# carltonyfakhry/geneticsCRE

Hardware: AMD Instinct MI355X
Metric: path_x_permutation_scores_per_sec (higher is better)
Workload: dtype u32

## Files before the change

geneticscre_amd/csrc/gcre_ie.hip:

```cpp
#include "gcre_ie_common.h"

namespace gcre {

#ifdef GCRE_IE_TIMING
#define GCRE_TM_MARK(var) __builtin_amdgcn_s_waitcnt(0); const u64 var = __builtin_amdgcn_s_memtime()
#define GCRE_TM_ADD(i, t1, t0) tm[i] += (t1) - (t0)
#else
#define GCRE_TM_MARK(var)
#define GCRE_TM_ADD(i, t1, t0)
#endif

template <int M, int L>
__global__ __launch_bounds__(64 * kIeWaves) __attribute__((amdgpu_waves_per_eu(M == 1 ? 4 : 2))) void k_null_ie(const IeArgs a) {
  static_assert(L % 4 == 0 && L >= 8 && L <= 16, "planes come in groups of 4");
  const int lane = threadIdx.x & 63;
  const int wave = __builtin_amdgcn_readfirstlane(threadIdx.x >> 6);
  const int xcd = blockIdx.x & 7;
  const i64 bi = (i64)(blockIdx.x >> 3);
  const i64 bx = a.waves_per_xcd / kIeWaves;
  const i64 cpt = (a.seg_end - a.seg_begin + kIeWaves - 1) / kIeWaves;
  const i64 chunks = cpt * a.nkt;
  const u32 lane4 = (u32)lane * 4u;
  __shared__ u32 gmax_lds[kIeWaves][32 * 64];
  u32* scr = gmax_lds[wave] + lane;
#pragma unroll
  for (int q = 0; q < 32; q++) scr[q * 64] = 0u;

  const SparseSeg GCRE_CONSTANT* segs = (const SparseSeg GCRE_CONSTANT*)a.segs;
  const u64 GCRE_CONSTANT* loff0 = (const u64 GCRE_CONSTANT*)a.loff0;
  const u32 GCRE_CONSTANT* lidx0 = (const u32 GCRE_CONSTANT*)a.lidx0;

  int cur_kt = -1;
  __amdgpu_buffer_rsrc_t mt = __builtin_amdgcn_make_buffer_rsrc((void*)a.mt, 0, 0x7fffffff, 0x00020000);
#ifdef GCRE_IE_TIMING
  u64 tm[6] = {0, 0, 0, 0, 0, 0};
  const u64 tm_begin = __builtin_amdgcn_s_memtime();
#endif

  auto flush = [&]() {
    if (cur_kt < 0) return;
    GCRE_TM_MARK(tf0);
    __syncthreads();
    const u32 slot0 = (u32)wave * 512u + (u32)lane * 8u;
    __amdgpu_buffer_rsrc_t nb = __builtin_amdgcn_make_buffer_rsrc((void*)(a.null_bits + (size_t)cur_kt * 2048), 0, 8192, 0x00020000);
    const u32x4 g0 = __builtin_amdgcn_raw_buffer_load_b128(nb, slot0 * 4u, 0, 16 );
    const u32x4 g1 = __builtin_amdgcn_raw_buffer_load_b128(nb, slot0 * 4u + 16u, 0, 16 );
    u32* out = a.null_bits + (size_t)cur_kt * 2048 + slot0;
    u32* cell = &gmax_lds[0][0] + (slot0 & 31u) * 64u + (slot0 >> 5);
    u32 own[8];
#pragma unroll
    for (int j = 0; j < 8; j++) {
      u32 m = 0u;
#pragma unroll
      for (int w = 0; w < kIeWaves; w++) {
        const u32 v = cell[w * 32 * 64 + j * 64];
        m = v > m ? v : m;
        cell[w * 32 * 64 + j * 64] = 0u;
      }
      own[j] = m;
    }
#pragma unroll
    for (int j = 0; j < 8; j++) {
      const u32 g = j < 4 ? g0[j & 3] : g1[j & 3];
      if (own[j] > g) atomicMax(out + j, own[j]);
    }
    __syncthreads();
    GCRE_TM_MARK(tf1);
    GCRE_TM_ADD(3, tf1, tf0);
#ifdef GCRE_IE_TIMING
    tm[4] += 1;
#endif
  };

  auto to_counts = [&](const u32 (&C)[L], u32 (&R)[16]) {
#pragma unroll
    for (int l = 0; l < 16; l++) R[l] = (l < L) ? C[l] : 0u;
    transpose16(R);
  };
  auto finish_m1 = [&](const u32 (&C)[L], u32 total) {
    u32 R[16];
    to_counts(C, R);
    const u32* diag_g = (const u32*)a.t32 + sp_diag_offset(total);
    u32 v[32], o[32];
#pragma unroll
    for (int j = 0; j < 16; j++) {
      v[j] = diag_g[R[j] & 0xffffu];
      v[j + 16] = diag_g[R[j] >> 16];
    }
#pragma unroll
    for (int q = 0; q < 32; q++) o[q] = scr[q * 64];
#pragma unroll
    for (int q = 0; q < 32; q++)
      if (v[q] > o[q]) scr[q * 64] = v[q];
  };

  auto finish_m2 = [&](const u32 (&Cp)[L], const u32 (&Cn)[L], u32 tp, u32 tn) {
    u32 Rp[16], Rn[16];
    to_counts(Cp, Rp);
    to_counts(Cn, Rn);
    const double* dp = a.d64 + sp_diag_offset(tp);
    const double* dn = a.d64 + sp_diag_offset(tn);
#pragma unroll
    for (int g0 = 0; g0 < 16; g0 += 4) {
      double sp[8], sn[8];
      u32 o[8];
#pragma unroll
      for (int k = 0; k < 4; k++) {
        sp[k] = dp[Rp[g0 + k] & 0xffffu];
        sn[k] = dn[Rn[g0 + k] & 0xffffu];
        sp[k + 4] = dp[Rp[g0 + k] >> 16];
        sn[k + 4] = dn[Rn[g0 + k] >> 16];
        o[k] = scr[(g0 + k) * 64];
        o[k + 4] = scr[(g0 + k + 16) * 64];
      }
#pragma unroll
      for (int k = 0; k < 8; k++) {
        float f = (float)(sp[k] + sn[k]);
        f = (f > 0.0f) ? f : 0.0f;
        const u32 v = __float_as_uint(f);
        const int q = (k < 4) ? g0 + k : g0 + k - 4 + 16;
        if (v > o[k]) scr[q * 64] = v;
      }
    }
  };

  auto load_planes = [&](u32 (&P)[L], const u32* planes, u32 unit, int groups) {
    const u32x4* src = (const u32x4*)(planes + (u64)unit * 256u) + lane;
#pragma unroll
    for (int j = 0; j < L / 4; j++) {
      u32x4 v = {0u, 0u, 0u, 0u};
      if (j < groups) v = src[j * 64];
      P[4 * j + 0] = v.x;
      P[4 * j + 1] = v.y;
      P[4 * j + 2] = v.z;
      P[4 * j + 3] = v.w;
    }
  };

  const i64 c_end = (i64)(xcd + 1) * chunks / 8;
  for (i64 c = (i64)xcd * chunks / 8 + bi; c < c_end; c += bx) {
    const int kt = (int)(c / cpt);
    if (kt != cur_kt) {
      flush();
      cur_kt = kt;
      mt = __builtin_amdgcn_make_buffer_rsrc((void*)(a.mt + (size_t)kt * a.mt_rows * 64), 0, 0x7fffffff, 0x00020000);
    }
    const i64 sidx = a.seg_begin + (c - (i64)kt * cpt) * kIeWaves + wave;
    if (sidx < a.seg_end) {
      GCRE_TM_MARK(ts0);
      const u32 row0 = segs[sidx].row0;
      const u32 first = segs[sidx].first;
      const u32 npaths = segs[sidx].n;
      const u32 qv = first + (((u32)lane < npaths) ? (u32)lane : 0u);
      u32 infov[M], lovv[M];
#pragma unroll
      for (int h = 0; h < M; h++) {
        infov[h] = a.linfo[(u64)qv * M + h];
        lovv[h] = a.lover[(u64)qv * M + h];
      }
      const u32 rzv = a.rowz[qv];
      u32 zunit[M];
#pragma unroll
      for (int h = 0; h < M; h++) {
        const u32 hz = (M == 2 && (rzv >> 31)) ? (u32)(1 - h) : (u32)h;
        zunit[h] = ((u32)kt * (u32)a.rowsz + (rzv & 0x7fffffffu) * (u32)M + hz) * (u32)a.gz;
      }
      u32 ttv[M];
#pragma unroll
      for (int h = 0; h < M; h++) ttv[h] = a.tot[(u64)qv * M + h];
      u32 lv[M][8];
#pragma unroll
      for (int h = 0; h < M; h++) {
        const u32x4* lp = (const u32x4*)(a.dlist + ((u64)qv * M + h) * 8u);
        const u32x4 e0 = lp[0], e1 = lp[1];
        lv[h][0] = e0.x; lv[h][1] = e0.y; lv[h][2] = e0.z; lv[h][3] = e0.w;
        lv[h][4] = e1.x; lv[h][5] = e1.y; lv[h][6] = e1.z; lv[h][7] = e1.w;
      }

      auto stream = [&](u32 (&P)[L], const u32 GCRE_CONSTANT* list, u64 p, u64 e) {
        u32 x[16];
        for (; p + 16 <= e; p += 16) {
          load16(x, mt, lane4, *(const u32x16 GCRE_CONSTANT*)(list + p));
          add16<L>(P, x);
        }
        for (; p < e; p += 4) {
          const u32x4 offs = *(const u32x4 GCRE_CONSTANT*)(list + p);
          u32 y4[4];
#pragma unroll
          for (int j = 0; j < 4; j++) y4[j] = __builtin_amdgcn_raw_buffer_load_b32(mt, lane4, offs[j], 0);
          add4<L>(P, y4);
        }
      };

      u32 B[M][L];
#pragma unroll
      for (int h = 0; h < M; h++) {
        const u64 r = (u64)row0 * M + h;
        if (a.planes0) {
          load_planes(B[h], a.planes0, (u32)(((u64)kt * (u64)a.rows0 + r) * (u64)a.g0), a.g0);
        } else if (a.rec_slot) {
          const u32 ra = a.rec_row0[row0], rzr = a.rec_rowz[row0], rz = rzr & 0x7fffffffu, rinfo = a.rec_linfo[r];
          const u32 hz = (M == 2 && (rzr >> 31)) ? (u32)(1 - h) : (u32)h;
          u32 ZR[L], S[L];
          load_planes(B[h], a.rec_planes_a, (u32)(((u64)kt * (u64)a.rec_rows_a + (u64)ra * M + h) * (u64)a.rec_ga), a.rec_ga);
          load_planes(ZR, a.rec_planes_z, (u32)(((u64)kt * (u64)a.rec_rows_z + (u64)rz * M + hz) * (u64)a.rec_gz), a.rec_gz);
#pragma unroll
          for (int l = 0; l < L; l++) S[l] = 0u;
          const u32 rlen = linfo_len(rinfo);
          stream(S, (const u32 GCRE_CONSTANT*)(a.rec_slot + r * 8u), 0, 8);
          if (rlen > 8u) stream(S, (const u32 GCRE_CONSTANT*)(a.rec_over + a.rec_lover[r]), 0, (u64)(rlen - 8u));
          u32 cy = 0u, bw = 0u;
#pragma unroll
          for (int l = 0; l < L; l++) {
            const u32 zl = linfo_overlap(rinfo) ? ZR[l] : S[l];
            const u32 sl_ = linfo_overlap(rinfo) ? S[l] : 0u;
            const u32 s1_ = B[h][l] ^ zl ^ cy;
            cy = maj3(B[h][l], zl, cy);
            B[h][l] = s1_ ^ sl_ ^ bw;
            bw = maj3(~s1_, sl_, bw);
          }
        } else {
#pragma unroll
          for (int l = 0; l < L; l++) B[h][l] = 0u;
          stream(B[h], lidx0, loff0[r], loff0[r + 1]);
        }
      }

      GCRE_TM_MARK(ts1);
      GCRE_TM_ADD(0, ts1, ts0);
      for (u32 t = 0; t < npaths; t++) {
        GCRE_TM_MARK(tp0);
        const u32 q = first + t;
        u32 C[M][L];
#pragma unroll
        for (int h = 0; h < M; h++) {
          const u32 r0 = rdlane(infov[h], t);
          const u32 len = linfo_len(r0);
          const bool overlap = linfo_overlap(r0);
          u32 offs[8], y[8];
#pragma unroll
          for (int j = 0; j < 8; j++) offs[j] = rdlane(lv[h][j], t);
#pragma unroll
          for (int j = 0; j < 8; j++) y[j] = __builtin_amdgcn_raw_buffer_load_b32(mt, lane4, offs[j], 0);
          u32 Z[L];
          if (overlap) {
            load_planes(Z, a.planesz, rdlane(zunit[h], t), a.gz);
          } else {
#pragma unroll
            for (int l = 0; l < L; l++) Z[l] = 0u;
          }
          u32 c0, a0, c1, a1, c2, a2, d0, b0;
          csa(c0, a0, y[0], y[1], y[2]);
          csa(c1, a1, y[3], y[4], y[5]);
          csa(c2, a2, a0, a1, y[6]);
          const u32 s0 = a2 ^ y[7], c3 = a2 & y[7];
          csa(d0, b0, c0, c1, c2);
          const u32 s1 = b0 ^ c3, d1 = b0 & c3;
          u32 S[L];
          S[0] = s0; S[1] = s1; S[2] = d0 ^ d1; S[3] = d0 & d1;
#pragma unroll
          for (int l = 4; l < L; l++) S[l] = 0u;
          if (len > 8u) stream(S, (const u32 GCRE_CONSTANT*)(a.dover + rdlane(lovv[h], t)), 0, (u64)(len - 8u));
          if (overlap) {
            u32 cy = 0u, bw = 0u;
#pragma unroll
            for (int l = 0; l < L; l++) {
              const u32 s1_ = B[h][l] ^ Z[l] ^ cy;
              cy = maj3(B[h][l], Z[l], cy);
              C[h][l] = s1_ ^ S[l] ^ bw;
              bw = maj3(~s1_, S[l], bw);
            }
          } else {
            u32 cy = 0u;
#pragma unroll
            for (int l = 0; l < L; l++) {
              C[h][l] = B[h][l] ^ S[l] ^ cy;
              cy = maj3(B[h][l], S[l], cy);
            }
          }
        }
        if (a.planes_out) {
#pragma unroll
          for (int h = 0; h < M; h++) {
            const u64 rh = ((u64)a.out_first + q) * M + h;
            u32x4* dst = (u32x4*)(a.planes_out + (((u64)cur_kt * (u64)a.rows_out + rh) * (u64)a.go) * 256u) + lane;
#pragma unroll
            for (int j = 0; j < 4; j++) {
              if (j < a.go) {
                u32x4 v = {0u, 0u, 0u, 0u};
                if (4 * j < L) v = u32x4{C[h][(4 * j) % L], C[h][(4 * j + 1) % L], C[h][(4 * j + 2) % L], C[h][(4 * j + 3) % L]};
                dst[j * 64] = v;
              }
            }
          }
        }
        GCRE_TM_MARK(tp1);
        GCRE_TM_ADD(1, tp1, tp0);
        if (q < a.score_begin || q >= a.score_end) continue;
        if constexpr (M == 1) {
          finish_m1(C[0], rdlane(ttv[0], t));
        } else {
          finish_m2(C[0], C[M - 1], rdlane(ttv[0], t), rdlane(ttv[M - 1], t));
        }
        GCRE_TM_MARK(tp2);
        GCRE_TM_ADD(2, tp2, tp1);
      }
    }
  }
  flush();
#ifdef GCRE_IE_TIMING
  tm[5] = __builtin_amdgcn_s_memtime() - tm_begin;
  if (a.timing && lane == 0)
    for (int i = 0; i < 6; i++) atomicAdd((unsigned long long*)a.timing + i, (unsigned long long)tm[i]);
  if (a.timing && lane == 0) atomicMax((unsigned long long*)a.timing + 6, (unsigned long long)tm[5]);
#endif
}


template <int L, int GZ, bool OUT, bool REC>
__global__ __launch_bounds__(64 * kIeWaves) __attribute__((amdgpu_waves_per_eu(L <= 12 ? 4 : 3))) void k_null_ie_m1(const IeArgs a) {
  constexpr int LP = (L + 3) / 4 * 4;
  static_assert(L >= 8 && L <= 16 && GZ >= 2 && 4 * GZ <= LP, "planes come in groups of 4");
  __shared__ u32 nmax_lds[kIeWaves][32 * 64];
  const int lane = threadIdx.x & 63;
  const int wave = __builtin_amdgcn_readfirstlane(threadIdx.x >> 6);
  const u32 lane4 = (u32)lane * 4u;
  u32* nm = nmax_lds[wave] + lane;
#pragma unroll
  for (int q = 0; q < 32; q++) nm[q * 64] = 0u;
  const SparseSeg GCRE_CONSTANT* segs = (const SparseSeg GCRE_CONSTANT*)a.segs;
  const char* k_planesz = (const char*)(((u64)(u32)__builtin_amdgcn_readfirstlane((int)(u32)((u64)a.planesz >> 32)) << 32) |
                                        (u64)(u32)__builtin_amdgcn_readfirstlane((int)(u32)(u64)a.planesz));

  int cur_kt = -1;
  u32 valid = 0u;
  u32 lad_base = (a.lad_mode == 0) ? 0u : (u32)(kLadderLevels - 1 + a.lad_mode) * (u32)a.ladder_stride;
  const u32 lad_keep = (u32)kLadderLevels * (u32)a.ladder_stride;
  bool dirty = false;
  u32 n_slow = 0u;
#ifdef GCRE_IE_TIMING
  u64 tm[6] = {0, 0, 0, 0, 0, 0};
  const u64 tm_begin = __builtin_amdgcn_s_memtime();
#endif
  __amdgpu_buffer_rsrc_t mt = __builtin_amdgcn_make_buffer_rsrc((void*)a.mt, 0, 0x7fffffff, 0x00020000);

  auto exchange = [&]() {
    u32* out = a.null_bits + (size_t)cur_kt * 2048 + lane * 32;
    __amdgpu_buffer_rsrc_t nb = __builtin_amdgcn_make_buffer_rsrc((void*)(a.null_bits + (size_t)cur_kt * 2048), 0, 8192, 0x00020000);
    u32x4 g4[8];
#pragma unroll
    for (int j = 0; j < 8; j++) g4[j] = __builtin_amdgcn_raw_buffer_load_b128(nb, (u32)lane * 128u + (u32)j * 16u, 0, 16 );
    u32 lo = 0xffffffffu;
#pragma unroll
    for (int q = 0; q < 32; q++) {
      const u32 g = g4[q >> 2][q & 3];
      const u32 own = nm[q * 64];
      if (dirty && own > g) atomicMax(out + q, own);
      const u32 v = own > g ? own : g;
      if ((valid >> q) & 1u) lo = v < lo ? v : lo;
    }
    dirty = false;
    u32 theta = __builtin_amdgcn_readfirstlane(wave_min_u32(lo));
    if (theta == 0xffffffffu) theta = 0u;
    int j = (int)(__uint_as_float(theta) * (float)kLadderPerUnit);
    j = j < 0 ? 0 : (j > kLadderLevels - 1 ? kLadderLevels - 1 : j);
    lad_base = (u32)j * (u32)a.ladder_stride;
  };
  auto flush_tile = [&]() {
    if (cur_kt >= 0) {
      u32* out = a.null_bits + (size_t)cur_kt * 2048 + lane * 32;
#pragma unroll 8
      for (int q = 0; q < 32; q++) {
        const u32 own = nm[q * 64];
        if (own != 0u) {
          atomicMax(out + q, own);
          nm[q * 64] = 0u;
        }
      }
    }
    dirty = false;
  };

  __shared__ u32 wq_state[kIeWaves][8];
  WorkQueue wq;
  wq.st = wq_state[wave];
  wq.init(a.queue, (u32)((a.seg_end - a.seg_begin + a.batch - 1) / a.batch), (u32)a.nkt);
  {
    wq.select(blockIdx.x & 7u);
  }
  u32 ticket = wq.take(lane);
  int since = 0, period = 1;
  for (;;) {
    const u32 work = __builtin_amdgcn_readfirstlane(ticket);
    const u32 q_n = wq.get(2);
    if (work >= q_n) {
      if (!wq.steal(lane)) break;
      ticket = wq.take(lane);
      continue;
    }
    ticket = wq.take(lane);
    const u32 item = wq.get(1) + work, nb = wq.get(3);
    const int kt = (int)(item / nb);
    const i64 s_lo = a.seg_begin + (i64)(item - (u32)kt * nb) * a.batch;
    const i64 s_hi = s_lo + a.batch < a.seg_end ? s_lo + a.batch : a.seg_end;
    if (kt != cur_kt) {
      flush_tile();
      cur_kt = kt;
      mt = __builtin_amdgcn_make_buffer_rsrc((void*)(a.mt + (size_t)kt * a.mt_rows * 64), 0, 0x7fffffff, 0x00020000);
      const int live = a.K - kt * 2048 - lane * 32;
      valid = live >= 32 ? 0xffffffffu : (live <= 0 ? 0u : ((1u << live) - 1u));
      if (a.lad_mode == 0) lad_base = 0u;
      since = 0;
      period = 1;
    }
    u32 nextv = 0u;
    bool have_next = false;
    for (i64 sidx = s_lo; sidx < s_hi; sidx++) {
      u32 row0, first, npaths;
      u32 rc_a = 0u, rc_z = 0u, rc_info = 0u, rc_lov = 0u;
      typedef u32 __attribute__((ext_vector_type(8))) u32x8;
      u32x8 rc_o = {0u, 0u, 0u, 0u, 0u, 0u, 0u, 0u};
      if (have_next) {
        row0 = rdlane(nextv, 0);
        first = rdlane(nextv, 1);
        npaths = rdlane(nextv, 2);
        if constexpr (REC) {
          rc_a = rdlane(nextv, 4);
          rc_z = rdlane(nextv, 5);
          rc_info = rdlane(nextv, 6);
          rc_lov = rdlane(nextv, 7);
#pragma unroll
          for (int j = 0; j < 8; j++) rc_o[j] = rdlane(nextv, 8 + j);
        }
      } else {
        row0 = segs[sidx].row0;
        first = segs[sidx].first;
        npaths = segs[sidx].n;
        if constexpr (REC) {
          const u32 GCRE_CONSTANT* rs = (const u32 GCRE_CONSTANT*)a.rec_segs + (u64)sidx * kRecSegWords;
          rc_a = rs[0];
          rc_z = rs[1];
          rc_info = rs[2];
          rc_lov = rs[3];
          rc_o = *(const u32x8 GCRE_CONSTANT*)(rs + 4);
        }
      }
      have_next = sidx + 1 < s_hi;
      if (have_next) {
        const u32* src = (const u32*)a.segs + (u64)(sidx + 1) * 3u + (u32)(lane < 3 ? lane : 0);
        if constexpr (REC) {
          if (lane >= 4 && lane < 16) src = a.rec_segs + (u64)(sidx + 1) * kRecSegWords + (u32)(lane - 4);
        }
        nextv = *src;
      }
      GCRE_TM_MARK(ts0);
      if (a.lad_mode == 0 && ++since >= period) {
        exchange();
        since = 0;
        period = period < kIeRefresh ? period * 2 : kIeRefresh;
      }
      GCRE_TM_MARK(ts1);
      GCRE_TM_ADD(4, ts1, ts0);

      const u32 qv = first + (((u32)lane < npaths) ? (u32)lane : 0u);
      const u32 infov = a.linfo[qv];
      const u32 lovv = a.lover[qv];
      const u32 zunit = ((u32)kt * (u32)a.rowsz + (a.rowz[qv] & 0x7fffffffu)) * (u32)a.gz;
      const u32 totv = a.tot[qv];
      const u32 lhv = a.ladder[((u64)sidx < (u64)a.score_segs ? lad_base : lad_keep) + totv];
      const u32x8 GCRE_CONSTANT* slots = (const u32x8 GCRE_CONSTANT*)(a.dlist + (u64)first * 8u);
      auto issue = [&](u32 t2, const u32x8 offs, u32 (&yy)[8], u32 (&ZZ)[4 * GZ]) {
        if constexpr (OUT) {
#pragma unroll
          for (int j = 0; j < 8; j++) yy[j] = __builtin_amdgcn_raw_buffer_load_b32(mt, lane4, offs[j], 0);
        }
        __amdgpu_buffer_rsrc_t rz = __builtin_amdgcn_make_buffer_rsrc((void*)(k_planesz + (u64)rdlane(zunit, t2) * 1024u), 0, 0x7fffffff, 0x00020000);
#pragma unroll
        for (int j = 0; j < GZ; j++) {
          const u32x4 v = __builtin_amdgcn_raw_buffer_load_b128(rz, lane4 * 4u + (u32)j * 1024u, 0, 0);
          ZZ[4 * j + 0] = v.x; ZZ[4 * j + 1] = v.y; ZZ[4 * j + 2] = v.z; ZZ[4 * j + 3] = v.w;
        }
      };
      u32 yA[8], yB[8], ZA[4 * GZ], ZB[4 * GZ];
      const u32 last = npaths - 1u;
      auto at = [&](u32 t2) -> u32 { return t2 < last ? t2 : last; };
      u32x8 oA = slots[0], oB = slots[at(1u)];
      issue(0u, oA, yA, ZA);
      u32 B[LP];
      auto load_groups = [&](u32 (&P)[LP], const u32* planes, u64 unit, int groups) {
        const u32x4* src = (const u32x4*)(planes + unit * 256u) + lane;
#pragma unroll
        for (int j = 0; j < LP / 4; j++) {
          u32x4 v = {0u, 0u, 0u, 0u};
          if (j < groups) v = src[j * 64];
          P[4 * j + 0] = v.x; P[4 * j + 1] = v.y; P[4 * j + 2] = v.z; P[4 * j + 3] = v.w;
        }
      };
      if constexpr (!REC) {
        load_groups(B, a.planes0, ((u64)kt * (u64)a.rows0 + (u64)row0) * (u64)a.g0, a.g0);
      } else {
        const u32 ra = rc_a, rz = rc_z & 0x7fffffffu, rinfo = rc_info;
        const u32x8 ro = rc_o;
        u32 yr[8];
#pragma unroll
        for (int j = 0; j < 8; j++) yr[j] = __builtin_amdgcn_raw_buffer_load_b32(mt, lane4, ro[j], 0);
        u32 ZR[LP];
        load_groups(B, a.rec_planes_a, ((u64)kt * (u64)a.rec_rows_a + (u64)ra) * (u64)a.rec_ga, a.rec_ga);
        load_groups(ZR, a.rec_planes_z, ((u64)kt * (u64)a.rec_rows_z + (u64)rz) * (u64)a.rec_gz, a.rec_gz);
        u32 S[L];
        {
          u32 S4[4];
          sum8(yr, S4);
#pragma unroll
          for (int l = 0; l < L; l++) S[l] = (l < 4) ? S4[l < 4 ? l : 0] : 0u;
        }
        const u32 rlen = linfo_len(rinfo);
        if (rlen > 8u) {
          const u32 GCRE_CONSTANT* more = (const u32 GCRE_CONSTANT*)(a.rec_over + rc_lov);
          for (u32 p = 0u; p + 8u < rlen; p += 8u) {
            const u32x8 o8 = *(const u32x8 GCRE_CONSTANT*)(more + p);
            u32 yy[8], s4[4];
#pragma unroll
            for (int j = 0; j < 8; j++) yy[j] = __builtin_amdgcn_raw_buffer_load_b32(mt, lane4, o8[j], 0);
            sum8(yy, s4);
            u32 cy = 0u;
#pragma unroll
            for (int l = 0; l < L; l++) {
              const u32 sv = S[l];
              const u32 add = (l < 4) ? s4[l < 4 ? l : 0] : 0u;
              S[l] = xor3(sv, add, cy);
              cy = majority(sv, add, cy);
            }
          }
        }
        if (linfo_overlap(rinfo)) {
          u32 cy = 0u, bw = 0u;
#pragma unroll
          for (int l = 0; l < L; l++) {
            const u32 s1_ = xor3(B[l], ZR[l], cy);
            cy = majority(B[l], ZR[l], cy);
            B[l] = xor3(s1_, S[l], bw);
            bw = borrow3(s1_, S[l], bw);
          }
        } else {
          u32 cy = 0u;
#pragma unroll
          for (int l = 0; l < L; l++) {
            const u32 bl = B[l];
            B[l] = xor3(bl, S[l], cy);
            cy = majority(bl, S[l], cy);
          }
        }
      }

      GCRE_TM_MARK(ts2);
      GCRE_TM_ADD(0, ts2, ts1);
      auto compute = [&](u32 t, const u32 (&y)[8], const u32 (&Z)[4 * GZ]) {
        GCRE_TM_MARK(tp0);
        const u32 r0 = rdlane(infov, t);
        const u32 len = linfo_len(r0);
        const bool overlap = linfo_overlap(r0);
        u32 C[L];
        u32 S4[4];
        sum8(y, S4);
        if (len <= 8u && overlap) {
          u32 T[4 * GZ];
          u32 bw = 0u;
#pragma unroll
          for (int l = 0; l < 4 * GZ; l++) {
            if (l < 4) {
              T[l] = xor3(Z[l], S4[l < 4 ? l : 0], bw);
              bw = borrow3(Z[l], S4[l < 4 ? l : 0], bw);
            } else {
              T[l] = Z[l] ^ bw;
              bw = bw & ~Z[l];
            }
          }
          u32 cy = 0u;
#pragma unroll
          for (int l = 0; l < L; l++) {
            if (l < 4 * GZ) {
              C[l] = xor3(B[l], T[l < 4 * GZ ? l : 0], cy);
              cy = majority(B[l], T[l < 4 * GZ ? l : 0], cy);
            } else {
              C[l] = B[l] ^ cy;
              cy = B[l] & cy;
            }
          }
        } else if (len <= 8u) {
          u32 cy = 0u;
#pragma unroll
          for (int l = 0; l < L; l++) {
            if (l < 4) {
              C[l] = xor3(B[l], S4[l < 4 ? l : 0], cy);
              cy = majority(B[l], S4[l < 4 ? l : 0], cy);
            } else {
              C[l] = B[l] ^ cy;
              cy = B[l] & cy;
            }
          }
        } else {
          u32 S[L];
#pragma unroll
          for (int l = 0; l < L; l++) S[l] = (l < 4) ? S4[l < 4 ? l : 0] : 0u;
          const u32 GCRE_CONSTANT* more = (const u32 GCRE_CONSTANT*)(a.dover + rdlane(lovv, t));
          for (u32 p = 0u; p + 8u < len; p += 8u) {
            const u32x8 o8 = *(const u32x8 GCRE_CONSTANT*)(more + p);
            u32 yy[8], s4[4];
#pragma unroll
            for (int j = 0; j < 8; j++) yy[j] = __builtin_amdgcn_raw_buffer_load_b32(mt, lane4, o8[j], 0);
            sum8(yy, s4);
            u32 cy = 0u;
#pragma unroll
            for (int l = 0; l < L; l++) {
              const u32 sv = S[l];
              if (l < 4) {
                S[l] = xor3(sv, s4[l < 4 ? l : 0], cy);
                cy = majority(sv, s4[l < 4 ? l : 0], cy);
              } else {
                S[l] = sv ^ cy;
                cy = sv & cy;
              }
            }
          }
          if (overlap) {
            u32 cy = 0u, bw = 0u;
#pragma unroll
            for (int l = 0; l < L; l++) {
              const u32 zl = (l < 4 * GZ) ? Z[l < 4 * GZ ? l : 0] : 0u;
              const u32 s1_ = xor3(B[l], zl, cy);
              cy = majority(B[l], zl, cy);
              C[l] = xor3(s1_, S[l], bw);
              bw = borrow3(s1_, S[l], bw);
            }
          } else {
            u32 cy = 0u;
#pragma unroll
            for (int l = 0; l < L; l++) {
              C[l] = xor3(B[l], S[l], cy);
              cy = majority(B[l], S[l], cy);
            }
          }
        }
        if constexpr (OUT) {
          const u64 rh = (u64)a.out_first + first + t;
          u32x4* dst = (u32x4*)(a.planes_out + (((u64)kt * (u64)a.rows_out + rh) * (u64)a.go) * 256u) + lane;
#pragma unroll
          for (int j = 0; j < 4; j++) {
            if (j < a.go) {
              u32x4 v = {0u, 0u, 0u, 0u};
              if (4 * j < L) v = u32x4{C[(4 * j) % L], (4 * j + 1 < L) ? C[(4 * j + 1) % L] : 0u, (4 * j + 2 < L) ? C[(4 * j + 2) % L] : 0u,
                                       (4 * j + 3 < L) ? C[(4 * j + 3) % L] : 0u};
              dst[j * 64] = v;
            }
          }
        }
        const u32 lh = rdlane(lhv, t);
        const u32 lo = lh & 0xffffu, hi = lh >> 16;
        u32 blo = 0u, bhi = 0u;
#pragma unroll
        for (int l = 0; l < L; l++) {
          const u32 kl = (u32)__builtin_amdgcn_sbfe((int)lo, l, 1);
          const u32 kh = (u32)__builtin_amdgcn_sbfe((int)hi, l, 1);
          blo = borrow3(C[l], kl, blo);
          bhi = borrow3(kh, C[l], bhi);
        }
        u32 m = (blo | bhi) & valid;
        GCRE_TM_MARK(tp2);
        GCRE_TM_ADD(2, tp2, tp0);
        if (__builtin_amdgcn_ballot_w64(m != 0u) == 0ull) return;
        n_slow++;
        const u32* diag_g = (const u32*)a.t32 + sp_diag_offset(rdlane(totv, t));
        while (m != 0u) {
          u32 bb[4], vv[4];
#pragma unroll
          for (int k = 0; k < 4; k++) {
            bb[k] = m ? (u32)__builtin_ctz(m) : bb[k ? k - 1 : 0];
            m &= m - 1u;
            u32 cnt = 0u;
#pragma unroll
            for (int l = 0; l < L; l++) cnt |= ((C[l] >> bb[k]) & 1u) << l;
            vv[k] = diag_g[cnt];
          }
#pragma unroll
          for (int k = 0; k < 4; k++)
            __hip_atomic_fetch_max(nm + bb[k] * 64, vv[k], __ATOMIC_RELAXED, __HIP_MEMORY_SCOPE_WAVEFRONT);
        }
        dirty = true;
        GCRE_TM_MARK(tp3);
        GCRE_TM_ADD(3, tp3, tp2);
      };

      auto compute_f = [&](u32 t, const u32 (&Z)[4 * GZ]) {
        const u32 r0 = rdlane(infov, t);
        const u32 len = linfo_len(r0);
        const bool overlap = linfo_overlap(r0);
        const u32 ov = len - linfo_pad(r0);
        const u32 lh = rdlane(lhv, t);
        const u32 lo = lh & 0xffffu, hi = lh >> 16;
        u32 W[L];
        u32 mu = valid;
        if (overlap) {
          u32 cy = 0u;
#pragma unroll
          for (int l = 0; l < L; l++) {
            if (l < 4 * GZ) {
              W[l] = xor3(B[l], Z[l < 4 * GZ ? l : 0], cy);
              cy = majority(B[l], Z[l < 4 * GZ ? l : 0], cy);
            } else {
              W[l] = B[l] ^ cy;
              cy = B[l] & cy;
            }
          }
          u32 lo2 = lo ? lo + ov : 0u;
          lo2 = lo2 > 0xffffu ? 0xffffu : lo2;
          u32 blo = 0u, bhi = 0u;
#pragma unroll
          for (int l = 0; l < L; l++) {
            const u32 kl = (u32)__builtin_amdgcn_sbfe((int)lo2, l, 1);
            const u32 kh = (u32)__builtin_amdgcn_sbfe((int)hi, l, 1);
            blo = borrow3(W[l], kl, blo);
            bhi = borrow3(kh, W[l], bhi);
          }
          if ((lo2 >> L) != 0u) blo = 0xffffffffu;
          mu = (blo | bhi | cy) & valid;
        } else {
#pragma unroll
          for (int l = 0; l < L; l++) W[l] = B[l];
        }
        if (__builtin_amdgcn_ballot_w64(mu != 0u) == 0ull) return;
#ifdef GCRE_IE_TIMING
        tm[1] += 1;
        tm[3] += (u64)__popcll(__builtin_amdgcn_ballot_w64(mu != 0u));
#endif
        u32 slow = 0u;
        const u32x8 o = slots[t];
        if (mu != 0u) {
          u32 y[8], S4[4];
#pragma unroll
          for (int j = 0; j < 8; j++) y[j] = __builtin_amdgcn_raw_buffer_load_b32(mt, lane4, o[j], 0);
          sum8(y, S4);
          u32 S[L];
#pragma unroll
          for (int l = 0; l < L; l++) S[l] = (l < 4) ? S4[l < 4 ? l : 0] : 0u;
          if (len > 8u) {
            const u32 GCRE_CONSTANT* more = (const u32 GCRE_CONSTANT*)(a.dover + rdlane(lovv, t));
            for (u32 p = 0u; p + 8u < len; p += 8u) {
              const u32x8 o8 = *(const u32x8 GCRE_CONSTANT*)(more + p);
              u32 yy[8], s4[4];
#pragma unroll
              for (int j = 0; j < 8; j++) yy[j] = __builtin_amdgcn_raw_buffer_load_b32(mt, lane4, o8[j], 0);
              sum8(yy, s4);
              u32 cy = 0u;
#pragma unroll
              for (int l = 0; l < L; l++) {
                const u32 sv = S[l];
                if (l < 4) {
                  S[l] = xor3(sv, s4[l < 4 ? l : 0], cy);
                  cy = majority(sv, s4[l < 4 ? l : 0], cy);
                } else {
                  S[l] = sv ^ cy;
                  cy = sv & cy;
                }
              }
            }
          }
          u32 C[L];
          if (overlap) {
            u32 bw = 0u;
#pragma unroll
            for (int l = 0; l < L; l++) {
              C[l] = xor3(W[l], S[l], bw);
              bw = borrow3(W[l], S[l], bw);
            }
          } else {
            u32 cy = 0u;
#pragma unroll
            for (int l = 0; l < L; l++) {
              C[l] = xor3(W[l], S[l], cy);
              cy = majority(W[l], S[l], cy);
            }
          }
          u32 blo = 0u, bhi = 0u;
#pragma unroll
          for (int l = 0; l < L; l++) {
            const u32 kl = (u32)__builtin_amdgcn_sbfe((int)lo, l, 1);
            const u32 kh = (u32)__builtin_amdgcn_sbfe((int)hi, l, 1);
            blo = borrow3(C[l], kl, blo);
            bhi = borrow3(kh, C[l], bhi);
          }
          u32 m = (blo | bhi) & mu;
          if (m != 0u) {
            slow = 1u;
            const u32* diag_g = (const u32*)a.t32 + sp_diag_offset(rdlane(totv, t));
            while (m != 0u) {
              u32 bb[4], vv[4];
#pragma unroll
              for (int k = 0; k < 4; k++) {
                bb[k] = m ? (u32)__builtin_ctz(m) : bb[k ? k - 1 : 0];
                m &= m - 1u;
                u32 cnt = 0u;
#pragma unroll
                for (int l = 0; l < L; l++) cnt |= ((C[l] >> bb[k]) & 1u) << l;
                vv[k] = diag_g[cnt];
              }
#pragma unroll
              for (int k = 0; k < 4; k++)
                __hip_atomic_fetch_max(nm + bb[k] * 64, vv[k], __ATOMIC_RELAXED, __HIP_MEMORY_SCOPE_WAVEFRONT);
            }
          }
        }
        if (__builtin_amdgcn_ballot_w64(slow != 0u) != 0ull) {
          n_slow++;
          dirty = true;
        }
      };

      if constexpr (OUT) {
        for (u32 t = 0; t < npaths; t += 2) {
          issue(at(t + 1), oB, yB, ZB);
          oA = slots[at(t + 2)];
          compute(t, yA, ZA);
          if (t + 1 < npaths) {
            issue(at(t + 2), oA, yA, ZA);
            oB = slots[at(t + 3)];
            compute(t + 1, yB, ZB);
          }
        }
      } else {
        u32 ZC[4 * GZ];
        issue(at(1u), oB, yB, ZB);
        for (u32 t = 0; t < npaths; t += 3) {
          issue(at(t + 2), oA, yA, ZC);
          compute_f(t, ZA);
          if (t + 1 < npaths) {
            issue(at(t + 3), oA, yA, ZA);
            compute_f(t + 1, ZB);
          }
          if (t + 2 < npaths) {
            issue(at(t + 4), oA, yA, ZB);
            compute_f(t + 2, ZC);
          }
        }
      }
    }
  }
  flush_tile();
#ifdef GCRE_IE_TIMING
  tm[5] = __builtin_amdgcn_s_memtime() - tm_begin;
  if (a.timing && lane == 0)
    for (int i = 0; i < 6; i++) atomicAdd((unsigned long long*)a.timing + i, (unsigned long long)tm[i]);
  if (a.timing && lane == 0) atomicMax((unsigned long long*)a.timing + 6, (unsigned long long)tm[5]);
#endif
  if (a.stats && lane == 0 && n_slow) atomicAdd(a.stats, n_slow);
}

#define GCRE_IE_M2(EXPR)                    \
  if (planes <= 8) { EXPR(2, 8); }          \
  else if (planes <= 12) { EXPR(2, 12); }   \
  else { EXPR(2, 16); }

#define GCRE_IE_M1_OR(EXPR, LL, GG)                                                  \
  if (out) { if (rec) { EXPR(LL, GG, true, true); } else { EXPR(LL, GG, true, false); } }   \
  else { if (rec) { EXPR(LL, GG, false, true); } else { EXPR(LL, GG, false, false); } }

#define GCRE_IE_M1(EXPR)                                                     \
  if (planes <= 8) { GCRE_IE_M1_OR(EXPR, 8, 2) }                             \
  else if (planes <= 10) {                                                   \
    if (gz <= 2) { GCRE_IE_M1_OR(EXPR, 10, 2) } else { GCRE_IE_M1_OR(EXPR, 10, 3) }        \
  } else if (planes <= 12) {                                                 \
    if (gz <= 2) { GCRE_IE_M1_OR(EXPR, 12, 2) } else { GCRE_IE_M1_OR(EXPR, 12, 3) }        \
  } else {                                                                   \
    if (gz <= 2) { GCRE_IE_M1_OR(EXPR, 16, 2) }                              \
    else if (gz == 3) { GCRE_IE_M1_OR(EXPR, 16, 3) }                         \
    else { GCRE_IE_M1_OR(EXPR, 16, 4) }                                      \
  }

#define GCRE_IE_GEN(EXPR)                                          \
  if (method == 1) {                                               \
    if (planes <= 8) { EXPR(1, 8); }                               \
    else if (planes <= 12) { EXPR(1, 12); }                        \
    else { EXPR(1, 16); }                                          \
  } else {                                                         \
    GCRE_IE_M2(EXPR)                                               \
  }

__global__ __launch_bounds__(256) void k_fill_rec_segs(const SparseSeg* segs, i64 nsegs, const u32* r_row0, const u32* r_rowz,
                                                       const u32* r_linfo, const u32* r_lover, const u32* r_slot, const u32* r_tot,
                                                       u32* out) {
  const i64 t = (i64)blockIdx.x * blockDim.x + threadIdx.x;
  const i64 sidx = t >> 2;
  const int part = (int)(t & 3);
  if (sidx >= nsegs) return;
  const u32 row0 = segs[sidx].row0;
  u32* o = out + sidx * kRecSegWords;
  if (part == 0) {
    o[0] = r_row0[row0];
    o[1] = r_rowz[row0];
  } else if (part == 1) {
    u32 info = r_linfo[row0];
    u32 need = 3u;
    if (r_tot) {
      const u32 t = r_tot[row0];
      need = t < 16u ? 0u : (t < 256u ? 1u : (t < 4096u ? 2u : 3u));
    }
    o[2] = linfo_with_groups(info, need);
    o[3] = r_lover[row0];
  } else {
    const u32x4 v = *(const u32x4*)(r_slot + (u64)row0 * 8u + (part - 2) * 4);
    *(u32x4*)(o + 4 + (part - 2) * 4) = v;
  }
}

hipError_t launch_fill_rec_segs(const SparseSeg* segs, int64_t nsegs, const uint32_t* r_row0, const uint32_t* r_rowz,
                                const uint32_t* r_linfo, const uint32_t* r_lover, const uint32_t* r_slot, const uint32_t* r_tot,
                                uint32_t* out, hipStream_t stream) {
  if (nsegs == 0) return hipSuccess;
  const i64 blocks = (nsegs * 4 + 255) / 256;
  hipLaunchKernelGGL(k_fill_rec_segs, dim3((unsigned)blocks), dim3(256), 0, stream, segs, nsegs, r_row0, r_rowz, r_linfo, r_lover,
                     r_slot, r_tot, out);
  return hipGetLastError();
}

hipError_t launch_null_ie(const IeArgs& a, int method, int planes, bool general, hipStream_t stream) {
  const dim3 grid((unsigned)(8 * a.waves_per_xcd / kIeWaves));
  const dim3 block(64 * kIeWaves);
  if (method == 1 && !general) {
    const int gz = a.gz;
    const bool out = a.planes_out != nullptr;
    const bool rec = a.rec_slot != nullptr;
#define GCRE_LAUNCH(LL, GG, OO, RR) hipLaunchKernelGGL((k_null_ie_m1<LL, GG, OO, RR>), grid, block, 0, stream, a)
    GCRE_IE_M1(GCRE_LAUNCH)
#undef GCRE_LAUNCH
  } else if (method == 2 && !general) {
    return launch_null_ie_m2(a, planes, stream);
  } else {
    if (a.waves_per_xcd < kIeWaves || a.waves_per_xcd % kIeWaves != 0) return hipErrorInvalidValue;
#define GCRE_LAUNCH(MM, LL) hipLaunchKernelGGL((k_null_ie<MM, LL>), grid, block, 0, stream, a)
    GCRE_IE_GEN(GCRE_LAUNCH)
#undef GCRE_LAUNCH
  }
  return hipGetLastError();
}

int ie_max_waves_per_cu(int method, int planes, int gz, bool out, bool rec) {
  int blocks = 0;
  hipError_t e = hipSuccess;
  if (method == 1) {
#define GCRE_OCC(LL, GG, OO, RR) e = hipOccupancyMaxActiveBlocksPerMultiprocessor(&blocks, k_null_ie_m1<LL, GG, OO, RR>, 64 * kIeWaves, 0)
    GCRE_IE_M1(GCRE_OCC)
#undef GCRE_OCC
  } else {
    return ie2_max_waves_per_cu(planes, gz, out, rec);
  }
  if (e != hipSuccess || blocks < 1) blocks = 1;
  return blocks * kIeWaves;
}

template <int L>
__global__ __launch_bounds__(256) void k_build_planes(const u32* mt_all, u32 mt_rows, int nkt, const u64* loff,
                                                      const u32* lidx, i64 nrowhalves, int groups, u32* planes) {
  const int lane = threadIdx.x & 63;
  const i64 wave = (i64)blockIdx.x * 4 + __builtin_amdgcn_readfirstlane(threadIdx.x >> 6);
  const i64 nwaves = (i64)gridDim.x * 4;
  const u32 lane4 = (u32)lane * 4u;
  const u64 GCRE_CONSTANT* off = (const u64 GCRE_CONSTANT*)loff;
  const u32 GCRE_CONSTANT* list = (const u32 GCRE_CONSTANT*)lidx;
  const i64 items = nrowhalves * nkt;
  for (i64 it = wave; it < items; it += nwaves) {
    const i64 w = it / nrowhalves;
    const i64 rr = it - w * nrowhalves;
    __amdgpu_buffer_rsrc_t mt = __builtin_amdgcn_make_buffer_rsrc((void*)(mt_all + (size_t)w * mt_rows * 64), 0, 0x7fffffff, 0x00020000);
    u32 P[L];
#pragma unroll
    for (int l = 0; l < L; l++) P[l] = 0u;
    u64 p = off[rr];
    const u64 e = off[rr + 1];
    u32 x[16];
    for (; p + 16 <= e; p += 16) {
      load16(x, mt, lane4, *(const u32x16 GCRE_CONSTANT*)(list + p));
      add16<L>(P, x);
    }
    for (; p < e; p += 4) {
      const u32x4 offs = *(const u32x4 GCRE_CONSTANT*)(list + p);
      u32 y[4];
#pragma unroll
      for (int j = 0; j < 4; j++) y[j] = __builtin_amdgcn_raw_buffer_load_b32(mt, lane4, offs[j], 0);
      add4<L>(P, y);
    }
    u32x4* dst = (u32x4*)(planes + (((u64)w * (u64)nrowhalves + (u64)rr) * (u64)groups) * 256u) + lane;
#pragma unroll
    for (int j = 0; j < L / 4; j++)
      if (j < groups) dst[j * 64] = u32x4{P[4 * j], P[4 * j + 1], P[4 * j + 2], P[4 * j + 3]};
  }
}

hipError_t launch_build_planes(const uint32_t* mt, uint32_t mt_rows, int nkt, const uint64_t* loff, const uint32_t* lidx,
                               int64_t nrowhalves, int groups, uint32_t* planes, hipStream_t stream) {
  const i64 items = nrowhalves * nkt;
  if (items == 0) return hipSuccess;
  const i64 blocks = (items + 3) / 4;
  const dim3 grid((unsigned)(blocks < 256 * 8 ? blocks : 256 * 8)), block(256);
  if (groups <= 2) hipLaunchKernelGGL(k_build_planes<8>, grid, block, 0, stream, mt, mt_rows, nkt, loff, lidx, nrowhalves, groups, planes);
  else if (groups == 3) hipLaunchKernelGGL(k_build_planes<12>, grid, block, 0, stream, mt, mt_rows, nkt, loff, lidx, nrowhalves, groups, planes);
  else hipLaunchKernelGGL(k_build_planes<16>, grid, block, 0, stream, mt, mt_rows, nkt, loff, lidx, nrowhalves, groups, planes);
  return hipGetLastError();
}

__global__ __launch_bounds__(64) void k_build_ladder(const u32* t32, int TD, u32* ladder) {
  __shared__ int left[kLadderLevels + 2], right[kLadderLevels + 2];
  const int t = blockIdx.x;
  const int lane = threadIdx.x;
  if (t >= TD) return;
  const u32* d = t32 + sp_diag_offset((u32)t);
  for (int k = lane; k < kLadderLevels + 2; k += 64) {
    left[k] = -1;
    right[k] = t + 1;
  }
  u64 mine = ~(u64)0;
  for (int c = lane; c <= t; c += 64) {
    const u64 key = ((u64)d[c] << 32) | (u32)c;
    mine = key < mine ? key : mine;
  }
#pragma unroll
  for (int o = 32; o > 0; o >>= 1) {
    const u64 other = ((u64)(u32)__shfl_xor((int)(mine >> 32), o, 64) << 32) | (u32)__shfl_xor((int)(u32)mine, o, 64);
    mine = other < mine ? other : mine;
  }
  const u32 best = (u32)(mine >> 32);
  const int c0 = (int)(u32)mine;
  __syncthreads();
  auto blocked_below = [](u32 bits) -> int {
    const float v = __uint_as_float(bits);
    if (!(v > 0.0f)) return 0;
    const float x = v * (float)kLadderPerUnit;
    if (x >= (float)kLadderLevels) return kLadderLevels;
    const int j = (int)x;
    return ((float)j < x) ? j + 1 : j;
  };
  for (int c = lane; c <= t; c += 64) {
    if (c == c0) continue;
    const int J = blocked_below(d[c]);
    if (J == 0) continue;
    if (c < c0) atomicMax(&left[J], c);
    else atomicMin(&right[J], c);
  }
  __syncthreads();
  if (lane == 0) {
    int l = -1, r = t + 1;
    for (int k = kLadderLevels; k >= 0; k--) {
      l = left[k] > l ? left[k] : l;
      r = right[k] < r ? right[k] : r;
      left[k] = l;
      right[k] = r;
    }
  }
  __syncthreads();
  const int Jbest = blocked_below(best);
  for (int j = lane; j < kLadderLevels; j += 64) {
    u32 e = 1u;
    if (Jbest <= j) e = ((u32)(right[j + 1] - 1) << 16) | (u32)(left[j + 1] + 1);
    ladder[(size_t)j * TD + t] = e;
  }
  if (lane == 0) {
    ladder[(size_t)kLadderLevels * TD + t] = 0xffff0000u;
    ladder[(size_t)(kLadderLevels + 1) * TD + t] = 1u;
  }
}

hipError_t launch_build_ladder(const float* t32, int TD, uint32_t* ladder, hipStream_t stream) {
  hipLaunchKernelGGL(k_build_ladder, dim3((unsigned)TD), dim3(64), 0, stream, (const u32*)t32, TD, ladder);
  return hipGetLastError();
}

__global__ __launch_bounds__(64) void k_build_ladder2(const double* dmax, int TD, u32* ladder) {
  __shared__ int left[kLadder2Levels + 2], right[kLadder2Levels + 2];
  const int t = blockIdx.x;
  const int lane = threadIdx.x;
  if (t >= TD) return;
  const double* d = dmax + sp_diag_offset((u32)t);
  for (int k = lane; k < kLadder2Levels + 2; k += 64) {
    left[k] = -1;
    right[k] = t + 1;
  }
  double bestv = __builtin_inf();
  int bestc = 0x7fffffff;
  for (int c = lane; c <= t; c += 64) {
    const double v = d[c];
    if (v < bestv || (v == bestv && c < bestc) || (bestc == 0x7fffffff)) {
      if (!(v != v)) { bestv = v; bestc = c; }
      else if (bestc == 0x7fffffff) { bestv = __builtin_inf(); bestc = c; }
    }
  }
#pragma unroll
  for (int o = 32; o > 0; o >>= 1) {
    const double ov = __shfl_xor(bestv, o, 64);
    const int oc = __shfl_xor(bestc, o, 64);
    if (ov < bestv || (ov == bestv && oc < bestc)) { bestv = ov; bestc = oc; }
  }
  const int c0 = bestc;
  __syncthreads();
  auto blocked_below = [](double v) -> int {
    if (v != v) return kLadder2Levels;
    if (!(v > 0.0)) return 0;
    const double x = v * (double)(2 * kLadderPerUnit);
    if (x >= (double)kLadder2Levels) return kLadder2Levels;
    const int j = (int)x;
    return ((double)j < x) ? j + 1 : j;
  };
  for (int c = lane; c <= t; c += 64) {
    if (c == c0) continue;
    const int J = blocked_below(d[c]);
    if (J == 0) continue;
    if (c < c0) atomicMax(&left[J], c);
    else atomicMin(&right[J], c);
  }
  __syncthreads();
  if (lane == 0) {
    int l = -1, r = t + 1;
    for (int k = kLadder2Levels; k >= 0; k--) {
      l = left[k] > l ? left[k] : l;
      r = right[k] < r ? right[k] : r;
      left[k] = l;
      right[k] = r;
    }
  }
  __syncthreads();
  const int Jbest = blocked_below(d[c0]);
  for (int j = lane; j < kLadder2Levels; j += 64) {
    u32 e = 1u;
    if (Jbest <= j) e = ((u32)(right[j + 1] - 1) << 16) | (u32)(left[j + 1] + 1);
    ladder[(size_t)j * TD + t] = e;
  }
  if (lane == 0) {
    ladder[(size_t)kLadder2Levels * TD + t] = 0xffff0000u;
    ladder[(size_t)(kLadder2Levels + 1) * TD + t] = 1u;
  }
}

hipError_t launch_build_ladder2(const double* dmax, int TD, uint32_t* ladder, hipStream_t stream) {
  hipLaunchKernelGGL(k_build_ladder2, dim3((unsigned)TD), dim3(64), 0, stream, dmax, TD, ladder);
  return hipGetLastError();
}

}
```

geneticscre_amd/csrc/gcre_ie2.hip:

```cpp
#include "gcre_ie_common.h"

#ifndef GCRE_M2_STEPS
#define GCRE_M2_STEPS 2
#endif
#ifndef GCRE_M2_YW_WIDE
#define GCRE_M2_YW_WIDE 4
#endif
#ifndef GCRE_M2_WAVES16
#define GCRE_M2_WAVES16 3
#endif
#ifndef GCRE_M2_MODES
#define GCRE_M2_MODES 3
#endif

namespace gcre {

template <int L, int GZ, bool OUT, bool REC>
__global__ __launch_bounds__(64 * kIeWaves) __attribute__((amdgpu_waves_per_eu(L <= 10 ? 4 : (L <= 12 ? 3 : GCRE_M2_WAVES16)))) void k_null_ie_m2(const IeArgs a) {
  constexpr int NS = GCRE_M2_STEPS;
  static_assert(NS == 2 || NS == 3, "two or three steps");
  constexpr int LP = (L + 3) / 4 * 4;
  constexpr int YW = L <= 10 ? 4 : GCRE_M2_YW_WIDE;
  constexpr int LZ = 4 * GZ;
  static_assert(LZ <= LP, "added rows have no more planes than joined paths");
  static_assert(L >= 8 && L <= 16, "8 to 16 counter planes");
  typedef u32 __attribute__((ext_vector_type(8))) u32x8;
  typedef u32 __attribute__((ext_vector_type(YW))) SlotV;
  __shared__ u32 nmax_lds[kIeWaves][32 * 64];
  constexpr u32 kLqCap = 128u;
  __shared__ u32 lq_lds[kIeWaves][3][kLqCap];
  const int lane = threadIdx.x & 63;
  const int wave = __builtin_amdgcn_readfirstlane(threadIdx.x >> 6);
  const u32 lane4 = (u32)lane * 4u;
  u32* nm = nmax_lds[wave] + lane;
#pragma unroll
  for (int q = 0; q < 32; q++) nm[q * 64] = 0u;
  const SparseSeg GCRE_CONSTANT* segs = (const SparseSeg GCRE_CONSTANT*)a.segs;
  u32 (*lq)[kLqCap] = lq_lds[wave];
  u32 lq_n = 0u;
  bool dirty = false;
  auto lq_drain = [&]() {
    for (u32 base = 0u; base < lq_n; base += 64u) {
      const u32 i = base + (u32)lane;
      if (i < lq_n) {
        const double f64 = a.d64[lq[0][i]] + a.d64[lq[1][i]];
        float f = (float)f64;
        f = (f > 0.0f) ? f : 0.0f;
        __hip_atomic_fetch_max(nmax_lds[wave] + lq[2][i], __float_as_uint(f), __ATOMIC_RELAXED, __HIP_MEMORY_SCOPE_WAVEFRONT);
      }
    }
    if (lq_n != 0u) dirty = true;
    lq_n = 0u;
  };
  const char* k_planesz = (const char*)(((u64)(u32)__builtin_amdgcn_readfirstlane((int)(u32)((u64)a.planesz >> 32)) << 32) |
                                        (u64)(u32)__builtin_amdgcn_readfirstlane((int)(u32)(u64)a.planesz));

  int cur_kt = -1;
  u32 valid = 0u;
  u32 lad[NS];
#pragma unroll
  for (int s = 0; s < NS; s++) lad[s] = (a.lad_mode == 0) ? 0u : (u32)(kLadder2Levels - 1 + a.lad_mode) * (u32)a.ladder_stride;
  const u32 lad_keep = (u32)kLadder2Levels * (u32)a.ladder_stride;
  u32 lad_top = lad[0];
  bool top_ok = a.lad_mode != 0 || a.g00_rows == 0u;
  u32 n_slow = 0u;
#ifdef GCRE_IE_TIMING
  u64 tm[8] = {0, 0, 0, 0, 0, 0, 0, 0};
#define GCRE_TM_COUNT(i, n) tm[i] += (u64)(n)
#else
#define GCRE_TM_COUNT(i, n)
#endif
  __amdgpu_buffer_rsrc_t mt = __builtin_amdgcn_make_buffer_rsrc((void*)a.mt, 0, 0x7fffffff, 0x00020000);

  auto exchange = [&]() {
    lq_drain();
    u32* out = a.null_bits + (size_t)cur_kt * 2048 + lane * 32;
    __amdgpu_buffer_rsrc_t nb = __builtin_amdgcn_make_buffer_rsrc((void*)(a.null_bits + (size_t)cur_kt * 2048), 0, 8192, 0x00020000);
    u32x4 g4[8];
#pragma unroll
    for (int j = 0; j < 8; j++) g4[j] = __builtin_amdgcn_raw_buffer_load_b128(nb, (u32)lane * 128u + (u32)j * 16u, 0, 16 );
    u32 lo = 0xffffffffu;
#pragma unroll
    for (int q = 0; q < 32; q++) {
      const u32 g = g4[q >> 2][q & 3];
      const u32 own = nm[q * 64];
      if (dirty && own > g) atomicMax(out + q, own);
      const u32 v = own > g ? own : g;
      if ((valid >> q) & 1u) lo = v < lo ? v : lo;
    }
    dirty = false;
    u32 theta = __builtin_amdgcn_readfirstlane(wave_min_u32(lo));
    if (theta == 0xffffffffu) theta = 0u;
    int j = (int)(__uint_as_float(theta) * (float)kLadderPerUnit);
    j = j < 0 ? 0 : (j > kLadderLevels - 1 ? kLadderLevels - 1 : j);
    int r[NS];
    if constexpr (NS == 2) {
      r[0] = (2 * j) / 3;
      r[1] = 2 * j - r[0];
    } else {
      r[0] = j / 2;
      r[1] = j;
      r[2] = 2 * j - r[0];
    }
#pragma unroll
    for (int s = 0; s < NS; s++) {
      const int rs = r[s] > kLadder2Levels - 1 ? kLadder2Levels - 1 : r[s];
      lad[s] = (u32)rs * (u32)a.ladder_stride;
    }
    const int rt = 2 * j - (int)a.g00_rows;
    top_ok = a.g00_rows != 0xffffffffu && rt >= 0;
    lad_top = (u32)(rt < 0 ? 0 : (rt > kLadder2Levels - 1 ? kLadder2Levels - 1 : rt)) * (u32)a.ladder_stride;
  };
  auto flush_tile = [&]() {
    lq_drain();
    if (cur_kt >= 0) {
      u32* out = a.null_bits + (size_t)cur_kt * 2048 + lane * 32;
#pragma unroll 8
      for (int q = 0; q < 32; q++) {
        const u32 own = nm[q * 64];
        if (own != 0u) {
          atomicMax(out + q, own);
          nm[q * 64] = 0u;
        }
      }
    }
    dirty = false;
  };
  auto load_groups = [&](u32 (&P)[LP], const u32* planes, u64 unit, int groups) {
    const u32x4* src = (const u32x4*)(planes + unit * 256u) + lane;
#pragma unroll
    for (int j = 0; j < LP / 4; j++) {
      u32x4 v = {0u, 0u, 0u, 0u};
      if (j < groups) v = src[j * 64];
      P[4 * j + 0] = v.x; P[4 * j + 1] = v.y; P[4 * j + 2] = v.z; P[4 * j + 3] = v.w;
    }
  };
  auto outside = [&](const auto& C, u32 lh) -> u32 {
    const u32 lo = lh & 0xffffu, hi = lh >> 16;
    u32 blo = 0u, bhi = 0u;
#pragma unroll
    for (int l = 0; l < L; l++) {
      const u32 kl = (u32)__builtin_amdgcn_sbfe((int)lo, l, 1);
      const u32 kh = (u32)__builtin_amdgcn_sbfe((int)hi, l, 1);
      blo = borrow3(C[l], kl, blo);
      bhi = borrow3(kh, C[l], bhi);
    }
    return blo | bhi;
  };
  auto sum4 = [&](const u32 (&y)[4], u32 (&S)[4]) {
    const u32 a0 = xor3(y[0], y[1], y[2]), c0 = majority(y[0], y[1], y[2]);
    S[0] = a0 ^ y[3];
    const u32 c1 = a0 & y[3];
    S[1] = c0 ^ c1;
    S[2] = c0 & c1;
    S[3] = 0u;
  };
  auto sum_more = [&](u32 (&S)[L], u32 len, const u32 GCRE_CONSTANT* over, const u32 GCRE_CONSTANT* lover_at) {
    const u32 GCRE_CONSTANT* more = over + *lover_at;
    for (u32 p = 0u; p + 8u < len; p += 8u) {
      const u32x8 o8 = *(const u32x8 GCRE_CONSTANT*)(more + p);
      u32 yy[8], s4[4];
#pragma unroll
      for (int j = 0; j < 8; j++) yy[j] = __builtin_amdgcn_raw_buffer_load_b32(mt, lane4, o8[j], 0);
      sum8(yy, s4);
      u32 cy = 0u;
#pragma unroll
      for (int l = 0; l < L; l++) {
        const u32 sv = S[l];
        if (l < 4) {
          S[l] = xor3(sv, s4[l < 4 ? l : 0], cy);
          cy = majority(sv, s4[l < 4 ? l : 0], cy);
        } else {
          S[l] = sv ^ cy;
          cy = sv & cy;
        }
      }
    }
  };
  auto add_half = [&](u32 (&C)[L], const auto& Bx, const u32 (&y)[YW], const u32 (&Z)[LZ], u32 info, const u32 GCRE_CONSTANT* slot_at,
                      const u32 GCRE_CONSTANT* lover_at) {
    const u32 len = linfo_len(info);
    const bool overlap = linfo_overlap(info);
    const u32 real = len - linfo_pad(info);
    u32 S4[4];
    {
      const u32 y03[4] = {y[0], y[1], y[2], y[3]};
      sum4(y03, S4);
    }
    if (real > 4u) {
      GCRE_TM_COUNT(4, 1);
      u32 y2[4], s2[4];
      if constexpr (YW == 8) {
#pragma unroll
        for (int j = 0; j < 4; j++) y2[j] = y[(4 + j) % YW];
      } else {
        const u32x4 o = *(const u32x4 GCRE_CONSTANT*)(slot_at + 4);
#pragma unroll
        for (int j = 0; j < 4; j++) y2[j] = __builtin_amdgcn_raw_buffer_load_b32(mt, lane4, o[j], 0);
      }
      sum4(y2, s2);
      const u32 t0 = S4[0] ^ s2[0], c0 = S4[0] & s2[0];
      const u32 t1 = xor3(S4[1], s2[1], c0), c1 = majority(S4[1], s2[1], c0);
      const u32 t2 = xor3(S4[2], s2[2], c1), c2 = majority(S4[2], s2[2], c1);
      S4[0] = t0; S4[1] = t1; S4[2] = t2; S4[3] = c2;
    }
    if (len <= 8u) {
      if (overlap) {
        u32 T[LZ];
        u32 bw = 0u;
#pragma unroll
        for (int l = 0; l < LZ; l++) {
          if (l < 4) {
            T[l] = xor3(Z[l], S4[l < 4 ? l : 0], bw);
            bw = borrow3(Z[l], S4[l < 4 ? l : 0], bw);
          } else {
            T[l] = Z[l] ^ bw;
            bw = bw & ~Z[l];
          }
        }
        u32 cy = 0u;
#pragma unroll
        for (int l = 0; l < L; l++) {
          if (l < LZ) {
            C[l] = xor3(Bx[l], T[l < LZ ? l : 0], cy);
            cy = majority(Bx[l], T[l < LZ ? l : 0], cy);
          } else {
            C[l] = Bx[l] ^ cy;
            cy = Bx[l] & cy;
          }
        }
      } else {
        u32 cy = 0u;
#pragma unroll
        for (int l = 0; l < L; l++) {
          if (l < 4) {
            C[l] = xor3(Bx[l], S4[l < 4 ? l : 0], cy);
            cy = majority(Bx[l], S4[l < 4 ? l : 0], cy);
          } else {
            C[l] = Bx[l] ^ cy;
            cy = Bx[l] & cy;
          }
        }
      }
      return;
    }
    GCRE_TM_COUNT(6, 1);
    u32 S[L];
#pragma unroll
    for (int l = 0; l < L; l++) S[l] = (l < 4) ? S4[l < 4 ? l : 0] : 0u;
    sum_more(S, len, (const u32 GCRE_CONSTANT*)a.dover, lover_at);
    if (overlap) {
      u32 cy = 0u, bw = 0u;
#pragma unroll
      for (int l = 0; l < L; l++) {
        const u32 zl = (l < LZ) ? Z[l < LZ ? l : 0] : 0u;
        const u32 s1_ = xor3(Bx[l], zl, cy);
        cy = majority(Bx[l], zl, cy);
        C[l] = xor3(s1_, S[l], bw);
        bw = borrow3(s1_, S[l], bw);
      }
    } else {
      u32 cy = 0u;
#pragma unroll
      for (int l = 0; l < L; l++) {
        C[l] = xor3(Bx[l], S[l], cy);
        cy = majority(Bx[l], S[l], cy);
      }
    }
  };
  auto issue = [&](u32 info, u32 zu, const SlotV offs, u32 (&yy)[YW], u32 (&ZZ)[LZ]) {
    const u32 real = linfo_true_len(info);
    if (YW == 8 && real > 4u) {
#pragma unroll
      for (int j = 0; j < 8; j++) yy[j % YW] = __builtin_amdgcn_raw_buffer_load_b32(mt, lane4, offs[j % YW], 0);
    } else if (real > 0u) {
#ifdef GCRE_M2_NOROWS
#pragma unroll
      for (int j = 0; j < 4; j++) yy[j] = offs[j];
#else
#pragma unroll
      for (int j = 0; j < 4; j++) yy[j] = __builtin_amdgcn_raw_buffer_load_b32(mt, lane4, offs[j], 0);
#endif
    } else {
#pragma unroll
      for (int j = 0; j < 4; j++) yy[j] = 0u;
    }
    if (linfo_overlap(info)) {
      __amdgpu_buffer_rsrc_t rz = __builtin_amdgcn_make_buffer_rsrc((void*)(k_planesz + (u64)zu * 1024u), 0, 0x7fffffff, 0x00020000);
#pragma unroll
      for (int j = 0; j < GZ; j++) {
        u32x4 v = {0u, 0u, 0u, 0u};
#ifdef GCRE_M2_NOZLOAD
        v = u32x4{zu, zu + (u32)j, lane4, 0u};
#else
        if (j < 2 || j < a.gz) v = __builtin_amdgcn_raw_buffer_load_b128(rz, lane4 * 4u + (u32)j * 1024u, 0, 0);
#endif
        ZZ[4 * j + 0] = v.x; ZZ[4 * j + 1] = v.y; ZZ[4 * j + 2] = v.z; ZZ[4 * j + 3] = v.w;
      }
    }
  };
  auto enqueue = [&](u32 m, const auto& Ca, const auto& Cb, u32 da, u32 db, bool b_zero) {
    while (__builtin_amdgcn_ballot_w64(m != 0u) != 0ull) {
      if (lq_n + 64u > kLqCap) lq_drain();
      const bool has = m != 0u;
      const u32 bb = has ? (u32)__builtin_ctz(m) : 0u;
      m &= m - 1u;
      u32 ca = 0u, cb = 0u;
#pragma unroll
      for (int l = L - 1; l >= 0; l--) ca = (ca << 1) | __builtin_amdgcn_ubfe(Ca[l], bb, 1u);
      if (!b_zero) {
#pragma unroll
        for (int l = L - 1; l >= 0; l--) cb = (cb << 1) | __builtin_amdgcn_ubfe(Cb[l], bb, 1u);
      }
      const u64 hm = __builtin_amdgcn_ballot_w64(has);
      GCRE_TM_COUNT(5, __builtin_popcountll(hm));
      const u32 pos = lq_n + __builtin_amdgcn_mbcnt_hi((u32)(hm >> 32), __builtin_amdgcn_mbcnt_lo((u32)hm, 0u));
      if (has) {
        lq[0][pos] = da + ca;
        lq[1][pos] = db + cb;
        lq[2][pos] = bb * 64u + (u32)lane;
      }
      lq_n += (u32)__builtin_popcountll(hm);
    }
  };

  __shared__ u32 wq_state[kIeWaves][8];
  WorkQueue wq;
  wq.st = wq_state[wave];
  wq.init(a.queue, (u32)((a.seg_end - a.seg_begin + a.batch - 1) / a.batch), (u32)a.nkt);
  wq.select(blockIdx.x & 7u);
  u32 ticket = wq.take(lane);
  int since = 0, period = 1;
  for (;;) {
    const u32 work = __builtin_amdgcn_readfirstlane(ticket);
    const u32 q_n = wq.get(2);
    if (work >= q_n) {
      if (!wq.steal(lane)) break;
      ticket = wq.take(lane);
      continue;
    }
    ticket = wq.take(lane);
    const u32 item = wq.get(1) + work, nb = wq.get(3);
    const int kt = (int)(item / nb);
    const i64 s_lo = a.seg_begin + (i64)(item - (u32)kt * nb) * a.batch;
    const i64 s_hi = s_lo + a.batch < a.seg_end ? s_lo + a.batch : a.seg_end;
    if (kt != cur_kt) {
      flush_tile();
      cur_kt = kt;
      mt = __builtin_amdgcn_make_buffer_rsrc((void*)(a.mt + (size_t)kt * a.mt_rows * 64), 0, 0x7fffffff, 0x00020000);
      const int live = a.K - kt * 2048 - lane * 32;
      valid = live >= 32 ? 0xffffffffu : (live <= 0 ? 0u : ((1u << live) - 1u));
      if (a.lad_mode == 0) {
#pragma unroll
        for (int s = 0; s < NS; s++) lad[s] = 0u;
        lad_top = 0u;
        top_ok = a.g00_rows == 0u;
      }
      since = 0;
      period = 1;
    }
    for (i64 sidx = s_lo; sidx < s_hi; sidx++) {
      const u32 row0 = segs[sidx].row0;
      const u32 first = segs[sidx].first;
      const u32 npaths = segs[sidx].n;
      if (a.lad_mode == 0 && ++since >= period) {
        exchange();
        since = 0;
        period = period < kIeRefresh ? period * 2 : kIeRefresh;
      }
      const bool inl = (u32)lane < npaths;
      const u32 qv = first + (inl ? (u32)lane : 0u);
      const u32 rzv = a.rowz[qv];
      const bool mine = (u64)sidx < (u64)a.score_segs;
      const bool seg_top_ok = top_ok;
      const u32 GCRE_CONSTANT* k_lover = (const u32 GCRE_CONSTANT*)a.lover + (u64)first * 2u;
      const u32 GCRE_CONSTANT* k_tot = (const u32 GCRE_CONSTANT*)a.tot + (u64)first * 2u;
      const u32 GCRE_CONSTANT* k_slot = (const u32 GCRE_CONSTANT*)a.dlist + (u64)first * 16u;
      u32 infoc, zunitc, ladc[NS], ladt, ladu[NS], totu;
      u64 pm0, pm1, pm2;
      {
        const u32 i0 = a.linfo[(u64)qv * 2], i1 = a.linfo[(u64)qv * 2 + 1];
        const u32 t0_ = a.tot[(u64)qv * 2], t1_ = a.tot[(u64)qv * 2 + 1];
        const bool e0 = !linfo_overlap(i0) && (i0 & kLinfoLenMask) == linfo_pad(i0);
        const bool e1 = !linfo_overlap(i1) && (i1 & kLinfoLenMask) == linfo_pad(i1);
        pm0 = __builtin_amdgcn_ballot_w64(inl && e1);
        pm1 = __builtin_amdgcn_ballot_w64(inl && e0 && !e1);
        pm2 = __builtin_amdgcn_ballot_w64(inl && !e0 && !e1);
        const bool c1 = e0 && !e1;
        infoc = c1 ? i1 : i0;
        const u32 hz = ((rzv >> 31) != 0u) != c1 ? 1u : 0u;
        zunitc = ((u32)kt * (u32)a.rowsz + (rzv & 0x7fffffffu) * 2u + hz) * (u32)a.gz;
        const u32 tc = c1 ? t1_ : t0_;
        totu = c1 ? t0_ : t1_;
#pragma unroll
        for (int s = 0; s < NS; s++) {
          ladc[s] = a.ladder[(mine ? lad[s] : lad_keep) + tc];
          ladu[s] = a.ladder[(mine ? lad[NS - 1 - s] : lad_keep) + totu];
        }
        ladt = a.ladder[(mine ? lad_top : lad_keep) + tc];
      }

      u32 B[2][LP];
      if constexpr (!REC) {
#pragma unroll
        for (int h = 0; h < 2; h++)
          load_groups(B[h], a.planes0, ((u64)kt * (u64)a.rows0 + (u64)row0 * 2 + h) * (u64)a.g0, a.g0);
      } else {
        const u32 GCRE_CONSTANT* r_row0 = (const u32 GCRE_CONSTANT*)a.rec_row0;
        const u32 GCRE_CONSTANT* r_rowz = (const u32 GCRE_CONSTANT*)a.rec_rowz;
        const u32 GCRE_CONSTANT* r_linfo = (const u32 GCRE_CONSTANT*)a.rec_linfo;
        const u32 GCRE_CONSTANT* r_lover = (const u32 GCRE_CONSTANT*)a.rec_lover;
        const u32 ra = r_row0[row0], rzr = r_rowz[row0];
        const u32 ri0 = r_linfo[(u64)row0 * 2], ri1 = r_linfo[(u64)row0 * 2 + 1];
#pragma unroll
        for (int h = 0; h < 2; h++)
          load_groups(B[h], a.rec_planes_a, ((u64)kt * (u64)a.rec_rows_a + (u64)ra * 2 + h) * (u64)a.rec_ga, a.rec_ga);
#pragma unroll
        for (int h = 0; h < 2; h++) {
          const u32 rinfo = h ? ri1 : ri0;
          const u32 rlen = linfo_len(rinfo);
          if (!linfo_overlap(rinfo) && rlen == linfo_pad(rinfo)) continue;
          const u32x8 ro = *(const u32x8 GCRE_CONSTANT*)(a.rec_slot + ((u64)row0 * 2 + h) * 8u);
          u32 yr[8];
#pragma unroll
          for (int j = 0; j < 8; j++) yr[j] = __builtin_amdgcn_raw_buffer_load_b32(mt, lane4, ro[j], 0);
          u32 ZR[LP];
          if (linfo_overlap(rinfo)) {
            const u32 hz = (rzr >> 31) ? (u32)(1 - h) : (u32)h;
            load_groups(ZR, a.rec_planes_z, ((u64)kt * (u64)a.rec_rows_z + (u64)(rzr & 0x7fffffffu) * 2 + hz) * (u64)a.rec_gz, a.rec_gz);
          }
          u32 S[L];
          {
            u32 S4[4];
            sum8(yr, S4);
#pragma unroll
            for (int l = 0; l < L; l++) S[l] = (l < 4) ? S4[l < 4 ? l : 0] : 0u;
          }
          if (rlen > 8u) sum_more(S, rlen, (const u32 GCRE_CONSTANT*)a.rec_over, r_lover + (u64)row0 * 2 + h);
          if (linfo_overlap(rinfo)) {
            u32 cy = 0u, bw = 0u;
#pragma unroll
            for (int l = 0; l < L; l++) {
              const u32 s1_ = xor3(B[h][l], ZR[l], cy);
              cy = majority(B[h][l], ZR[l], cy);
              B[h][l] = xor3(s1_, S[l], bw);
              bw = borrow3(s1_, S[l], bw);
            }
          } else {
            u32 cy = 0u;
#pragma unroll
            for (int l = 0; l < L; l++) {
              const u32 bl = B[h][l];
              B[h][l] = xor3(bl, S[l], cy);
              cy = majority(bl, S[l], cy);
            }
          }
        }
      }
      auto write_out = [&](u32 h, u32 t, const auto& C) {
        if constexpr (OUT) {
          const u64 rh = ((u64)a.out_first + first + t) * 2 + h;
          u32x4* dst = (u32x4*)(a.planes_out + (((u64)kt * (u64)a.rows_out + rh) * (u64)a.go) * 256u) + lane;
#pragma unroll
          for (int j = 0; j < 4; j++) {
            if (j < a.go) {
              u32x4 v = {0u, 0u, 0u, 0u};
              if (4 * j < L) v = u32x4{C[(4 * j) % L], (4 * j + 1 < L) ? C[(4 * j + 1) % L] : 0u,
                                       (4 * j + 2 < L) ? C[(4 * j + 2) % L] : 0u, (4 * j + 3 < L) ? C[(4 * j + 3) % L] : 0u};
              dst[j * 64] = v;
            }
          }
        }
      };
      u32 yA[YW], yB[YW], ZA[LZ], ZB[LZ];
#pragma unroll
      for (int l = 0; l < LZ; l++) ZA[l] = ZB[l] = 0u;

      if (pm2 != 0ull) {
        u32 info2[2], zunit2[2], lad2[NS][2];
#pragma unroll
        for (int h = 0; h < 2; h++) {
          info2[h] = a.linfo[(u64)qv * 2 + h];
          const u32 hz = (rzv >> 31) ? (u32)(1 - h) : (u32)h;
          zunit2[h] = ((u32)kt * (u32)a.rowsz + (rzv & 0x7fffffffu) * 2u + hz) * (u32)a.gz;
          const u32 th = a.tot[(u64)qv * 2 + h];
#pragma unroll
          for (int s = 0; s < NS; s++) lad2[s][h] = a.ladder[(mine ? lad[s] : lad_keep) + th];
        }
        u64 rem = pm2;
        u32 t = (u32)__builtin_ctzll(rem);
        rem &= rem - 1ull;
        SlotV oA = *(const SlotV GCRE_CONSTANT*)(k_slot + t * 16u), oB = *(const SlotV GCRE_CONSTANT*)(k_slot + t * 16u + 8u);
        issue(rdlane(info2[0], t), rdlane(zunit2[0], t), oA, yA, ZA);
        for (;;) {
          issue(rdlane(info2[1], t), rdlane(zunit2[1], t), oB, yB, ZB);
          const bool more = rem != 0ull;
          const u32 tn = more ? (u32)__builtin_ctzll(rem) : t;
          rem &= rem - 1ull;
          oA = *(const SlotV GCRE_CONSTANT*)(k_slot + tn * 16u);
          u32 C0[L], C1[L];
          add_half(C0, B[0], yA, ZA, rdlane(info2[0], t), k_slot + t * 16u, k_lover + t * 2u);
          write_out(0u, t, C0);
          issue(rdlane(info2[0], tn), rdlane(zunit2[0], tn), oA, yA, ZA);
          oB = *(const SlotV GCRE_CONSTANT*)(k_slot + tn * 16u + 8u);
          add_half(C1, B[1], yB, ZB, rdlane(info2[1], t), k_slot + t * 16u + 8u, k_lover + t * 2u + 1u);
          write_out(1u, t, C1);
          u32 m = valid;
#pragma unroll
          for (int s = 0; s < NS; s++) m &= outside(C0, rdlane(lad2[s][0], t)) | outside(C1, rdlane(lad2[NS - 1 - s][1], t));
          GCRE_TM_COUNT(3, 1);
          if (__builtin_amdgcn_ballot_w64(m != 0u) != 0ull) {
            n_slow++;
            enqueue(m, C0, C1, sp_diag_offset(k_tot[t * 2u]), sp_diag_offset(k_tot[t * 2u + 1u]), false);
          }
          if (!more) break;
          t = tn;
        }
      }

      const u32 t00 = pm0 ? (u32)__builtin_ctzll(pm0) : 0u, t01 = pm1 ? (u32)__builtin_ctzll(pm1) : 0u;
      const u32 totU0 = rdlane(totu, t00), totU1 = rdlane(totu, t01);
      const bool empty0 = (GCRE_M2_MODES & 1) && pm0 != 0ull && totU0 == 0u && seg_top_ok;
      const bool empty1 = (GCRE_M2_MODES & 1) && pm1 != 0ull && totU1 == 0u && seg_top_ok;
      u32 U[NS], U1[NS];
#pragma unroll
      for (int s = 0; s < NS; s++) U[s] = U1[s] = 0u;
      bool single0 = true, single1 = true;
      if (pm0 != 0ull && !empty0) {
#pragma unroll
        for (int s = 0; s < NS; s++) U[s] = outside(B[1], rdlane(ladu[s], t00));
        single0 = (GCRE_M2_MODES & 2) && __builtin_amdgcn_ballot_w64((U[NS - 1] & valid) != 0u) == 0ull;
      }
      if (pm1 != 0ull && !empty1) {
#pragma unroll
        for (int s = 0; s < NS; s++) U1[s] = outside(B[0], rdlane(ladu[s], t01));
        single1 = (GCRE_M2_MODES & 2) && __builtin_amdgcn_ballot_w64((U1[NS - 1] & valid) != 0u) == 0ull;
      }
#pragma nounroll
      for (u32 hc = 0u; hc < 2u; hc++) {
        const u64 pm = hc ? pm1 : pm0;
        if (pm == 0ull) continue;
        if (hc) {
#pragma unroll
          for (int l = 0; l < L; l++) { const u32 x = B[0][l]; B[0][l] = B[1][l]; B[1][l] = x; }
#pragma unroll
          for (int s = 0; s < NS; s++) U[s] = U1[s];
        }
        const bool u_empty = hc ? empty1 : empty0;
        const bool single = hc ? single1 : single0;
        const u32 dU = sp_diag_offset(hc ? totU1 : totU0);
        const u32 ladw = u_empty ? ladt : ladc[NS - 1];
        auto compute = [&](u32 t, const u32 (&y)[YW], const u32 (&Z)[LZ]) {
          u32 C[L];
          add_half(C, B[0], y, Z, rdlane(infoc, t), k_slot + t * 16u + hc * 8u, k_lover + t * 2u + hc);
          write_out(hc, t, C);
          write_out(1u - hc, t, B[1]);
          GCRE_TM_COUNT(u_empty ? 0 : (single ? 1 : 2), 1);
          u32 m = outside(C, rdlane(ladw, t));
          if (!single) {
            asm volatile("" ::: "memory");
            m |= U[NS - 1];
#pragma unroll
            for (int s = 0; s < NS - 1; s++) m &= outside(C, rdlane(ladc[s], t)) | U[s];
          }
          m &= valid;
          if (__builtin_amdgcn_ballot_w64(m != 0u) == 0ull) return;
          n_slow++;
#ifdef GCRE_M2_NOLOOKUP
          return;
#endif
          enqueue(m, C, B[1], sp_diag_offset(k_tot[t * 2u + hc]), dU, u_empty);
        };
        u64 rem = pm;
        u32 tA = (u32)__builtin_ctzll(rem);
        rem &= rem - 1ull;
        bool hasB = rem != 0ull;
        u32 tB = hasB ? (u32)__builtin_ctzll(rem) : tA;
        rem &= rem - 1ull;
        SlotV oA = *(const SlotV GCRE_CONSTANT*)(k_slot + tA * 16u + hc * 8u), oB = *(const SlotV GCRE_CONSTANT*)(k_slot + tB * 16u + hc * 8u);
        issue(rdlane(infoc, tA), rdlane(zunitc, tA), oA, yA, ZA);
        for (;;) {
          issue(rdlane(infoc, tB), rdlane(zunitc, tB), oB, yB, ZB);
          const bool hasC = rem != 0ull;
          const u32 tC = hasC ? (u32)__builtin_ctzll(rem) : tB;
          rem &= rem - 1ull;
          oA = *(const SlotV GCRE_CONSTANT*)(k_slot + tC * 16u + hc * 8u);
          compute(tA, yA, ZA);
          if (!hasB) break;
          issue(rdlane(infoc, tC), rdlane(zunitc, tC), oA, yA, ZA);
          const bool hasD = rem != 0ull;
          const u32 tD = hasD ? (u32)__builtin_ctzll(rem) : tC;
          rem &= rem - 1ull;
          oB = *(const SlotV GCRE_CONSTANT*)(k_slot + tD * 16u + hc * 8u);
          compute(tB, yB, ZB);
          if (!hasC) break;
          tA = tC;
          tB = tD;
          hasB = hasD;
        }
      }
    }
  }
  flush_tile();
#ifdef GCRE_IE_TIMING
  if (a.timing && lane == 0)
    for (int i = 0; i < 7; i++) atomicAdd((unsigned long long*)a.timing + i, (unsigned long long)tm[i]);
#endif
  if (a.stats && lane == 0 && n_slow) atomicAdd(a.stats, n_slow);
}

#define GCRE_IE_M2P(EXPR)                                                                  \
  if (planes <= 8) { EXPR(8, 2); }                                                         \
  else if (planes <= 10) { if (a.gz <= 2) { EXPR(10, 2); } else { EXPR(10, 3); } }         \
  else if (planes <= 12) { EXPR(12, 3); }                                                  \
  else { EXPR(16, 4); }

#define GCRE_IE_M2_OR(EXPR, LL, GG)                                                            \
  if (out) { if (rec) { EXPR(LL, GG, true, true); } else { EXPR(LL, GG, true, false); } }       \
  else { if (rec) { EXPR(LL, GG, false, true); } else { EXPR(LL, GG, false, false); } }

hipError_t launch_null_ie_m2(const IeArgs& a, int planes, hipStream_t stream) {
  const dim3 grid((unsigned)(8 * a.waves_per_xcd / kIeWaves));
  const dim3 block(64 * kIeWaves);
  const bool out = a.planes_out != nullptr;
  const bool rec = a.rec_slot != nullptr;
#define GCRE_LAUNCH2X(LL, GG, OO, RR) hipLaunchKernelGGL((k_null_ie_m2<LL, GG, OO, RR>), grid, block, 0, stream, a)
#define GCRE_LAUNCH2(LL, GG) GCRE_IE_M2_OR(GCRE_LAUNCH2X, LL, GG)
  GCRE_IE_M2P(GCRE_LAUNCH2)
#undef GCRE_LAUNCH2
#undef GCRE_LAUNCH2X
  return hipGetLastError();
}

int ie2_max_waves_per_cu(int planes, int gz, bool out, bool rec) {
  int blocks = 0;
  hipError_t e = hipSuccess;
  struct { int gz; } a{gz};
#define GCRE_OCC2X(LL, GG, OO, RR) e = hipOccupancyMaxActiveBlocksPerMultiprocessor(&blocks, k_null_ie_m2<LL, GG, OO, RR>, 64 * kIeWaves, 0)
#define GCRE_OCC2(LL, GG) GCRE_IE_M2_OR(GCRE_OCC2X, LL, GG)
  GCRE_IE_M2P(GCRE_OCC2)
#undef GCRE_OCC2
#undef GCRE_OCC2X
  if (e != hipSuccess || blocks < 1) blocks = 1;
  return blocks * kIeWaves;
}

int ie2_steps() { return GCRE_M2_STEPS; }

}
```

geneticscre_amd/csrc/gcre_ie_common.h:

```cpp
#pragma once
#include "gcre_bitslice.h"
#include "gcre_kernels.h"

namespace gcre {

constexpr int kIeWaves = 4;
constexpr int kIeQueueStride = 16;
constexpr int kIeRefresh = 32;

__device__ __forceinline__ u32 maj3(u32 a, u32 b, u32 c) { return (a & b) | ((a ^ b) & c); }

__device__ __forceinline__ u32 wave_min_u32(u32 v) {
#pragma unroll
  for (int o = 32; o > 0; o >>= 1) {
    const u32 t = (u32)__shfl_xor((int)v, o, 64);
    v = t < v ? t : v;
  }
  return v;
}

__device__ __forceinline__ u32 rdlane(u32 v, u32 t) { return (u32)__builtin_amdgcn_readlane((int)v, (int)t); }

__device__ __forceinline__ u32 wave_max_u32(u32 v) {
#pragma unroll
  for (int o = 32; o > 0; o >>= 1) {
    const u32 t = (u32)__shfl_xor((int)v, o, 64);
    v = t > v ? t : v;
  }
  return v;
}

struct WorkQueue {
  volatile u32* st;
  __device__ __forceinline__ u32 get(int i) const { return (u32)__builtin_amdgcn_readfirstlane(st[i]); }
  __device__ __forceinline__ u32* counters() const { return (u32*)(((u64)get(7) << 32) | (u64)get(6)); }
  __device__ __forceinline__ void init(u32* counters, u32 nbatch, u32 nkt) {
    st[3] = nbatch;
    st[4] = nbatch * nkt;
    st[6] = (u32)(u64)counters;
    st[7] = (u32)((u64)counters >> 32);
  }
  __device__ __forceinline__ u32 first_of(u32 j, u32 total) const { return (u32)(((u64)total * j) >> 3); }
  __device__ __forceinline__ void select(u32 j) {
    const u32 total = get(4);
    const u32 lo = first_of(j, total);
    st[0] = j;
    st[1] = lo;
    st[2] = first_of(j + 1, total) - lo;
  }
  __device__ __forceinline__ u32 take(int lane) const {
    u32 t = 0u;
    if (lane == 0) t = atomicAdd(counters() + get(0) * kIeQueueStride, 1u);
    return (u32)__builtin_amdgcn_readfirstlane((int)t);
  }
  __device__ __forceinline__ bool steal(int lane) {
    const u32 total = get(4);
    u32 left = 0u;
    if (lane < 8) {
      const u32 taken = __hip_atomic_load(counters() + lane * kIeQueueStride, __ATOMIC_RELAXED, __HIP_MEMORY_SCOPE_AGENT);
      const u32 all = first_of((u32)lane + 1u, total) - first_of((u32)lane, total);
      left = taken < all ? all - taken : 0u;
    }
    const u32 m = __builtin_amdgcn_readfirstlane(wave_max_u32(left));
    if (m == 0u) return false;
    select((u32)(__ffsll((long long)__ballot(left == m)) - 1));
    return true;
  }
};

__device__ __forceinline__ u32 xor3(u32 a, u32 b, u32 c) { return __builtin_amdgcn_bitop3_b32(a, b, c, 0x96); }
__device__ __forceinline__ u32 majority(u32 a, u32 b, u32 c) { return __builtin_amdgcn_bitop3_b32(a, b, c, 0xE8); }
__device__ __forceinline__ u32 borrow3(u32 a, u32 b, u32 c) { return __builtin_amdgcn_bitop3_b32(a, b, c, 0x8E); }

__device__ __forceinline__ void sum8(const u32 (&r)[8], u32 (&s)[4]) {
  const u32 a0 = xor3(r[0], r[1], r[2]), c0 = majority(r[0], r[1], r[2]);
  const u32 a1 = xor3(r[3], r[4], r[5]), c1 = majority(r[3], r[4], r[5]);
  const u32 a2 = xor3(a0, a1, r[6]), c2 = majority(a0, a1, r[6]);
  s[0] = a2 ^ r[7];
  const u32 c3 = a2 & r[7];
  const u32 b0 = xor3(c0, c1, c2), d0 = majority(c0, c1, c2);
  s[1] = b0 ^ c3;
  const u32 d1 = b0 & c3;
  s[2] = d0 ^ d1;
  s[3] = d0 & d1;
}

}
```

geneticscre_amd/csrc/gcre_ieq.hip:

```cpp
#include "gcre_ie_common.h"

#include <type_traits>

namespace gcre {

#ifndef GCRE_REFINE_MAX
#define GCRE_REFINE_MAX 2
#endif
#ifndef GCRE_QSEGS
#define GCRE_QSEGS 2
#endif
#ifndef GCRE_QWAVES
#define GCRE_QWAVES 4
#endif
constexpr int kQSegs = GCRE_QSEGS;

#ifdef GCRE_IE_TIMING
#define GCRE_QT(var) const u64 var = __builtin_amdgcn_s_memtime()
#define GCRE_QT_ADD(i, t1, t0) tm[i] += (t1) - (t0)
#else
#define GCRE_QT(var)
#define GCRE_QT_ADD(i, t1, t0)
#endif

template <int N, class F>
__device__ __forceinline__ void with_count(u32 count, F&& f) {
  if constexpr (N > 1) {
    if (count != (u32)N) return with_count<N - 1>(count, f);
  }
  f(std::integral_constant<int, N>{});
}

template <int L, int GZ, bool REC, bool WIDE>
__global__ __launch_bounds__(64 * kIeWaves) __attribute__((amdgpu_waves_per_eu(GCRE_QWAVES))) void k_null_ie_q(const IeArgs a) {
  constexpr int LP = (L + 3) / 4 * 4;
  constexpr int LZ = 4 * GZ;
  static_assert(L >= 8 && L <= 16 && GZ >= 2 && LZ <= LP, "planes come in groups of 4");
  typedef u32 __attribute__((ext_vector_type(8))) u32x8;
  __shared__ u32 nmax_lds[kIeWaves][32 * 64];
  __shared__ u32 wq_state[kIeWaves][8];
  constexpr u32 kLqCap = 128u;
  __shared__ u32 lq_lds[kIeWaves][2][kLqCap];
  const int lane = threadIdx.x & 63;
  const int wave = __builtin_amdgcn_readfirstlane(threadIdx.x >> 6);
  const u32 lane4 = (u32)lane * 4u;
  u32* nm = nmax_lds[wave] + lane;
#pragma unroll
  for (int q = 0; q < 32; q++) nm[q * 64] = 0u;
  u32 (*lq)[kLqCap] = lq_lds[wave];
  u32 lq_n = 0u;
  constexpr u32 kFqCap = 64u;
  __shared__ u32 fq_lds[kIeWaves][2][kFqCap];
  u32 (*fq)[kFqCap] = fq_lds[wave];
  u32 fq_n = 0u;
  auto lq_drain = [&]() {
    for (u32 base = 0u; base < lq_n; base += 64u) {
      const u32 i = base + (u32)lane;
      if (i < lq_n)
        __hip_atomic_fetch_max(nmax_lds[wave] + lq[1][i], ((const u32*)a.t32)[lq[0][i]], __ATOMIC_RELAXED, __HIP_MEMORY_SCOPE_WAVEFRONT);
    }
    lq_n = 0u;
  };
  auto uni = [](u32 v) -> u32 { return (u32)__builtin_amdgcn_readfirstlane((int)v); };
  auto uni_ptr = [&](const void* p) -> const char* { return (const char*)(((u64)uni((u32)((u64)p >> 32)) << 32) | (u64)uni((u32)(u64)p)); };
  const u32 k_quad_begin = uni((u32)a.quad_begin), k_quad_end = uni((u32)a.quad_end), k_batch = uni((u32)a.batch);
  const u32 k_nkt = uni((u32)a.nkt), k_K = uni((u32)a.K), k_mt_rows = uni(a.mt_rows), k_lstride = uni((u32)a.ladder_stride);
  const u32 k_lad_mode = uni((u32)a.lad_mode), k_score_segs = uni(a.score_segs);
  const char* k_mt = uni_ptr(a.mt);
  const char* k_planesz = uni_ptr(a.planesz);
  const u32 k_ztile = uni(a.z_tile_units);

  const u32 k_road = (k_lad_mode == 0u) ? (uni(a.flagq) != 0u ? 2u : 1u) : 0u;

  int cur_kt = -1;
  u32 valid = 0u;
  u32 lad_base = (k_lad_mode == 0u) ? 0u : ((u32)kLadderLevels - 1u + k_lad_mode) * k_lstride;
  const u32 lad_keep = (u32)kLadderLevels * k_lstride;
  u32 n_slow = 0u;
#ifdef GCRE_IE_TIMING
  u64 tm[11] = {0, 0, 0, 0, 0, 0, 0, 0, 0, 0, 0};
  u32 n_flagged = 0u;
  const u64 tm_begin = __builtin_amdgcn_s_memtime();
#endif
  __amdgpu_buffer_rsrc_t mt = __builtin_amdgcn_make_buffer_rsrc((void*)k_mt, 0, 0x7fffffff, 0x00020000);
  __amdgpu_buffer_rsrc_t zt = __builtin_amdgcn_make_buffer_rsrc((void*)k_planesz, 0, 0x7fffffff, 0x00020000);

  auto fq_drain = [&]() {
    GCRE_QT(td0);
    if ((u32)lane < fq_n) {
      const u32 q = fq[0][lane], w = fq[1][lane];
      const u32 bb = (w >> 17) & 31u, at = (w >> 22) * 4u;
      const u32x4* e = (const u32x4*)(a.dlist + (u64)q * 8u);
      const u32x4 e0 = e[0], e1 = e[1];
      const u32 tot = a.tot[q];
      u32 y[8];
#pragma unroll
      for (int j = 0; j < 4; j++) {
        y[j] = __builtin_amdgcn_raw_buffer_load_b32(mt, e0[j] + at, 0, 0);
        y[4 + j] = __builtin_amdgcn_raw_buffer_load_b32(mt, e1[j] + at, 0, 0);
      }
      u32 S = 0u;
#pragma unroll
      for (int j = 0; j < 8; j++) S += (y[j] >> bb) & 1u;
      const u32 cell = sp_diag_offset(tot) + (w & 0x1ffffu) - S;
      __hip_atomic_fetch_max(nmax_lds[wave] + bb * 64u + (w >> 22), ((const u32*)a.t32)[cell], __ATOMIC_RELAXED, __HIP_MEMORY_SCOPE_WAVEFRONT);
    }
    fq_n = 0u;
    GCRE_QT(td1);
    GCRE_QT_ADD(9, td1, td0);
  };

  auto merge_global = [&](bool want_theta) {
    u32* out = a.null_bits + (size_t)cur_kt * 2048 + lane * 32;
    __amdgpu_buffer_rsrc_t nb = __builtin_amdgcn_make_buffer_rsrc((void*)(a.null_bits + (size_t)cur_kt * 2048), 0, 8192, 0x00020000);
    u32x4 g4[8];
#pragma unroll
    for (int j = 0; j < 8; j++) g4[j] = __builtin_amdgcn_raw_buffer_load_b128(nb, (u32)lane * 128u + (u32)j * 16u, 0, 16 );
    u32 lo = 0xffffffffu;
#pragma unroll
    for (int q = 0; q < 32; q++) {
      const u32 g = g4[q >> 2][q & 3];
      const u32 own = nm[q * 64];
      if (own > g) atomicMax(out + q, own);
      const u32 v = own > g ? own : g;
      nm[q * 64] = want_theta ? v : 0u;
      if ((valid >> q) & 1u) lo = v < lo ? v : lo;
    }
    return lo;
  };
  auto exchange = [&]() {
    fq_drain();
    lq_drain();
    u32 theta = __builtin_amdgcn_readfirstlane(wave_min_u32(merge_global(true)));
    if (theta == 0xffffffffu) theta = 0u;
    int j = (int)(__uint_as_float(theta) * (float)kLadderPerUnit);
    j = j < 0 ? 0 : (j > kLadderLevels - 1 ? kLadderLevels - 1 : j);
    lad_base = (u32)j * k_lstride;
  };
  auto flush_tile = [&]() {
    fq_drain();
    lq_drain();
    if (cur_kt >= 0) (void)merge_global(false);
  };

  WorkQueue wq;
  wq.st = wq_state[wave];
  wq.init(a.queue, (k_quad_end - k_quad_begin + k_batch - 1u) / k_batch, k_nkt);
  wq.select(blockIdx.x & 7u);
  u32 ticket = wq.take(lane);
  int since = 0, period = 1;
  for (;;) {
    const u32 work = __builtin_amdgcn_readfirstlane(ticket);
    const u32 q_n = wq.get(2);
    if (work >= q_n) {
      if (!wq.steal(lane)) break;
      ticket = wq.take(lane);
      continue;
    }
    ticket = wq.take(lane);
    const u32 item = wq.get(1) + work, nbt = wq.get(3);
    const int kt = __builtin_amdgcn_readfirstlane((int)(item / nbt));
    const u32 q_lo = uni(k_quad_begin + (item - (u32)kt * nbt) * k_batch);
    const u32 q_hi = uni(q_lo + k_batch < k_quad_end ? q_lo + k_batch : k_quad_end);
    if (kt != cur_kt) {
      flush_tile();
      cur_kt = kt;
      mt = __builtin_amdgcn_make_buffer_rsrc((void*)(k_mt + (size_t)kt * k_mt_rows * 256u), 0, 0x7fffffff, 0x00020000);
      if constexpr (!WIDE) zt = __builtin_amdgcn_make_buffer_rsrc((void*)(k_planesz + (u64)kt * (u64)k_ztile * 1024u), 0, 0x7fffffff, 0x00020000);
      const int live = (int)k_K - kt * 2048 - lane * 32;
      valid = live >= 32 ? 0xffffffffu : (live <= 0 ? 0u : ((1u << live) - 1u));
      if (k_lad_mode == 0u) lad_base = 0u;
      since = 0;
      period = 1;
    }
    auto load_hdr = [&](u32 qe_, u32 (&h)[kQSegs]) {
      const u32 cnt_ = (qe_ >> 30) + 1u, s0_ = qe_ & 0x3fffffffu;
#pragma unroll
      for (int g = 0; g < kQSegs; g++) {
        h[g] = 0u;
        if ((u32)g < cnt_) {
          const u32* src = (const u32*)a.segs + (u64)(s0_ + (u32)g) * 3u + (u32)(lane < 3 ? lane : 0);
          if constexpr (REC) {
            if (lane >= 4 && lane < 16) src = a.rec_segs + (u64)(s0_ + (u32)g) * kRecSegWords + (u32)(lane - 4);
          }
          h[g] = *src;
        }
      }
    };
    u32 hdr_n[kQSegs] = {};
    u32 qe_n = 0u;
    bool have_next = false;
    for (u32 qi = q_lo; qi < q_hi; qi++) {
      GCRE_QT(t0);
      u32 hdr[kQSegs];
      u32 qe;
      if (have_next) {
        qe = qe_n;
#pragma unroll
        for (int g = 0; g < kQSegs; g++) hdr[g] = hdr_n[g];
      } else {
        qe = uni(((const u32 GCRE_CONSTANT*)a.quads)[qi]);
        load_hdr(qe, hdr);
      }
      have_next = qi + 1u < q_hi;
      if (have_next) qe_n = uni(((const u32 GCRE_CONSTANT*)a.quads)[qi + 1u]);
      const u32 qcnt = (qe >> 30) + 1u;
      const u32 s0 = qe & 0x3fffffffu;
      const u32 npaths = rdlane(hdr[0], 2);
      GCRE_QT(te0);
      if (k_lad_mode == 0u && ++since >= period) {
        exchange();
        since = 0;
        period = period < kIeRefresh ? period * 2 : kIeRefresh;
      }
      GCRE_QT(te1);
      GCRE_QT_ADD(5, te1, te0);
      const u32 lad_row = (s0 < k_score_segs) ? lad_base : lad_keep;

      u32 infov[kQSegs], lhv[kQSegs], lfv[kQSegs], firstg[kQSegs];
      u32 B[kQSegs][L];
      u32 zunit = 0u;
      auto load_groups = [&](auto& P, const u32* planes, u64 unit, int groups) {
        constexpr int NP = (int)(sizeof(P) / sizeof(u32));
        __amdgpu_buffer_rsrc_t rp = __builtin_amdgcn_make_buffer_rsrc((void*)(uni_ptr(planes) + unit * 1024u), 0, 0x7fffffff, 0x00020000);
#pragma unroll
        for (int j = 0; j < LP / 4; j++) {
          u32x4 v = {0u, 0u, 0u, 0u};
          if (j < groups) v = __builtin_amdgcn_raw_buffer_load_b128(rp, lane4 * 4u + (u32)j * 1024u, 0, 0);
#pragma unroll
          for (int i = 0; i < 4; i++)
            if (4 * j + i < NP) P[4 * j + i] = v[i];
        }
      };
      u32 totv[kQSegs];
      u32 yr[REC ? kQSegs : 1][8];
      u32 rinfo_g[kQSegs] = {}, rlov_g[kQSegs] = {}, rz_g[kQSegs] = {};
#pragma unroll
      for (int g = 0; g < kQSegs; g++) {
        totv[g] = 0u;
        if ((u32)g < qcnt) {
          const u32 first = rdlane(hdr[g], 1);
          firstg[g] = first;
          const u32 qv = first + (((u32)lane < npaths) ? (u32)lane : 0u);
          infov[g] = a.linfo[qv];
          totv[g] = a.tot[qv];
          if (g == 0) {
            if constexpr (WIDE) zunit = ((u32)kt * (u32)a.rowsz + (a.rowz[qv] & 0x7fffffffu)) * (u32)a.gz;
            else zunit = ((a.rowz[qv] & 0x7fffffffu) * (u32)a.gz) << 10;
          }
        }
      }
#pragma unroll
      for (int g = 0; g < kQSegs; g++) {
        if ((u32)g < qcnt) {
          const u32 row0 = rdlane(hdr[g], 0);
          if constexpr (!REC) {
            load_groups(B[g], a.planes0, ((u64)kt * (u64)a.rows0 + (u64)row0) * (u64)a.g0, a.g0);
          } else {
            const u32 ra = rdlane(hdr[g], 4);
            rz_g[g] = rdlane(hdr[g], 5) & 0x7fffffffu;
            rinfo_g[g] = rdlane(hdr[g], 6);
            rlov_g[g] = rdlane(hdr[g], 7);
            u32 ro[8];
#pragma unroll
            for (int j = 0; j < 8; j++) ro[j] = rdlane(hdr[g], 8 + j);
            const u32 rtrue = linfo_true_len(rinfo_g[g]);
#pragma unroll
            for (int j = 0; j < 8; j++) {
              yr[REC ? g : 0][j] = 0u;
              if ((u32)j < rtrue) yr[REC ? g : 0][j] = __builtin_amdgcn_raw_buffer_load_b32(mt, lane4, ro[j], 0);
            }
            const int ga_need = (int)linfo_groups(rinfo_g[g]) + 1;
            load_groups(B[g], a.rec_planes_a, ((u64)kt * (u64)a.rec_rows_a + (u64)ra) * (u64)a.rec_ga, ga_need < a.rec_ga ? ga_need : a.rec_ga);
          }
        }
      }
      if (have_next) load_hdr(qe_n, hdr_n);
      GCRE_QT(t1);
      GCRE_QT_ADD(0, t1, t0);
      if constexpr (REC) {
        u32 ZR[LP];
        load_groups(ZR, a.rec_planes_z, ((u64)kt * (u64)a.rec_rows_z + (u64)rz_g[0]) * (u64)a.rec_gz, a.rec_gz);
#pragma unroll
        for (int g = 0; g < kQSegs; g++) {
          if ((u32)g < qcnt) {
            if (rz_g[g] != rz_g[0]) load_groups(ZR, a.rec_planes_z, ((u64)kt * (u64)a.rec_rows_z + (u64)rz_g[g]) * (u64)a.rec_gz, a.rec_gz);
            const u32 rinfo = rinfo_g[g];
            const u32 rlen = linfo_len(rinfo);
            u32 S[L];
            {
              u32 S4[4];
              sum8(yr[REC ? g : 0], S4);
#pragma unroll
              for (int l = 0; l < L; l++) S[l] = (l < 4) ? S4[l < 4 ? l : 0] : 0u;
            }
            if (rlen > 8u) {
              const u32 GCRE_CONSTANT* more = (const u32 GCRE_CONSTANT*)(a.rec_over + rlov_g[g]);
              for (u32 p = 0u; p + 8u < rlen; p += 8u) {
                const u32x8 o8 = *(const u32x8 GCRE_CONSTANT*)(more + p);
                u32 yy[8], s4[4];
#pragma unroll
                for (int j = 0; j < 8; j++) yy[j] = __builtin_amdgcn_raw_buffer_load_b32(mt, lane4, uni(o8[j]), 0);
                sum8(yy, s4);
                u32 cy = 0u;
#pragma unroll
                for (int l = 0; l < L; l++) {
                  const u32 sv = S[l];
                  const u32 add = (l < 4) ? s4[l < 4 ? l : 0] : 0u;
                  S[l] = xor3(sv, add, cy);
                  cy = majority(sv, add, cy);
                }
              }
            }
            if (linfo_overlap(rinfo)) {
              u32 cy = 0u, bw = 0u;
#pragma unroll
              for (int l = 0; l < L; l++) {
                const u32 s1_ = xor3(B[g][l], ZR[l], cy);
                cy = majority(B[g][l], ZR[l], cy);
                B[g][l] = xor3(s1_, S[l], bw);
                bw = borrow3(s1_, S[l], bw);
              }
            } else {
              u32 cy = 0u;
#pragma unroll
              for (int l = 0; l < L; l++) {
                const u32 bl = B[g][l];
                B[g][l] = xor3(bl, S[l], cy);
                cy = majority(bl, S[l], cy);
              }
            }
            if (rz_g[g] != rz_g[0]) load_groups(ZR, a.rec_planes_z, ((u64)kt * (u64)a.rec_rows_z + (u64)rz_g[0]) * (u64)a.rec_gz, a.rec_gz);
          }
        }
      }
      GCRE_QT(t2);
      GCRE_QT_ADD(1, t2, t1);
#pragma unroll
      for (int g = 0; g < kQSegs; g++) {
        if ((u32)g < qcnt) {
          const u32 lh = a.ladder[lad_row + totv[g]];
          const u32 r0 = infov[g];
          const u32 ov = linfo_true_len(r0);
          const u32 lo = lh & 0xffffu;
          const u32 lo2 = lo ? lo + ov : 0u;
          lhv[g] = lh;
          lfv[g] = (!linfo_overlap(r0) || (lo2 >> L) != 0u) ? 1u : ((lh & 0xffff0000u) | lo2);
        }
      }

      GCRE_QT(t3);
      GCRE_QT_ADD(2, t3, t2);
      const u32x8 GCRE_CONSTANT* slots = (const u32x8 GCRE_CONSTANT*)a.dlist;
      auto issue_at = [&](u32 zu, u32 (&ZZ)[LZ]) {
        __amdgpu_buffer_rsrc_t rz = zt;
        u32 so = 0u;
        if constexpr (WIDE) rz = __builtin_amdgcn_make_buffer_rsrc((void*)(k_planesz + (u64)zu * 1024u), 0, 0x7fffffff, 0x00020000);
        else so = zu;
#pragma unroll
        for (int j = 0; j < GZ; j++) {
          const u32x4 v = __builtin_amdgcn_raw_buffer_load_b128(rz, lane4 * 4u + (u32)j * 1024u, so, 0);
          ZZ[4 * j + 0] = v.x; ZZ[4 * j + 1] = v.y; ZZ[4 * j + 2] = v.z; ZZ[4 * j + 3] = v.w;
        }
      };
      auto issue = [&](u32 t2, u32 (&ZZ)[LZ]) { issue_at(rdlane(zunit, t2), ZZ); };

      u64 todo[kQSegs] = {};
      auto filter_f = [&](int g, u32 t, const u32 (&Bg)[L], const u32 (&Z)[LZ]) {
        const u32 lf = rdlane(lfv[g], t);
        u32 cy = 0u, blo = 0u, bhi = 0u;
#pragma unroll
        for (int l = 0; l < L; l++) {
          u32 w;
          if (l < LZ) {
            w = xor3(Bg[l], Z[l < LZ ? l : 0], cy);
            cy = majority(Bg[l], Z[l < LZ ? l : 0], cy);
          } else {
            w = Bg[l] ^ cy;
            cy = Bg[l] & cy;
          }
          const u32 kl = (u32)__builtin_amdgcn_sbfe((int)lf, l, 1);
          const u32 kh = (u32)__builtin_amdgcn_sbfe((int)lf, 16 + l, 1);
          blo = borrow3(w, kl, blo);
          bhi = borrow3(kh, w, bhi);
        }
        u32 fm = (blo | bhi | cy) & valid;
        if (__builtin_amdgcn_ballot_w64(fm != 0u) == 0ull) return;
        const u32 info = rdlane(infov[g], t);
        if (k_road != 0u && (info & 1u) != 0u && __builtin_amdgcn_ballot_w64(__builtin_popcount(fm) > GCRE_REFINE_MAX) == 0ull) {
          GCRE_QT(ts0);
#ifdef GCRE_IE_TIMING
          tm[10] += 1;
          n_flagged += (u32)__builtin_popcount(fm);
#endif
          u32 Wp[L];
          u32 c2 = 0u;
          auto sum_w = [&]() {
#pragma unroll
            for (int l = 0; l < L; l++) {
              if (l < LZ) {
                Wp[l] = xor3(Bg[l], Z[l < LZ ? l : 0], c2);
                c2 = majority(Bg[l], Z[l < LZ ? l : 0], c2);
              } else {
                Wp[l] = Bg[l] ^ c2;
                c2 = Bg[l] & c2;
              }
            }
          };
          if (k_road == 2u && linfo_len(info) <= 8u) {
            u32 total = 0u;
            {
              u32 f = fm;
              asm volatile("" : "+v"(f));
#pragma unroll
              for (int r = 0; r < GCRE_REFINE_MAX; r++) {
                total += (u32)__builtin_popcountll(__builtin_amdgcn_ballot_w64(f != 0u));
                f &= f - 1u;
              }
            }
            if (total <= kFqCap) {
              if (fq_n + total > kFqCap) fq_drain();
              sum_w();
              const u32 q = firstg[g] + t;
              while (__builtin_amdgcn_ballot_w64(fm != 0u) != 0ull) {
                const bool has = fm != 0u;
                const u32 bb = has ? (u32)__builtin_ctz(fm) : 0u;
                fm &= fm - 1u;
                u32 cnt = ((c2 >> bb) & 1u) << L;
#pragma unroll
                for (int l = 0; l < L; l++) cnt |= ((Wp[l] >> bb) & 1u) << l;
                const u64 hm = __builtin_amdgcn_ballot_w64(has);
                const u32 pos = fq_n + __builtin_amdgcn_mbcnt_hi((u32)(hm >> 32), __builtin_amdgcn_mbcnt_lo((u32)hm, 0u));
                if (has) {
                  fq[0][pos] = q;
                  fq[1][pos] = cnt | (bb << 17) | ((u32)lane << 22);
                }
                fq_n += (u32)__builtin_popcountll(hm);
              }
              n_slow++;
              GCRE_QT(ts1);
              GCRE_QT_ADD(8, ts1, ts0);
              return;
            }
          }
          const u32 ov = linfo_true_len(info);
          const u32* lad_t = a.ladder + rdlane(totv[g], t);
          sum_w();
          bool unsafe = false;
          while (__builtin_amdgcn_ballot_w64(fm != 0u) != 0ull) {
            const bool has = fm != 0u;
            const u32 bb = has ? (u32)__builtin_ctz(fm) : 0u;
            fm &= fm - 1u;
            u32 cnt = ((c2 >> bb) & 1u) << L;
#pragma unroll
            for (int l = 0; l < L; l++) cnt |= ((Wp[l] >> bb) & 1u) << l;
            if (has) {
              int j = (int)(__uint_as_float(nm[bb * 64]) * (float)kLadderPerUnit);
              j = j < 0 ? 0 : (j > kLadderLevels - 1 ? kLadderLevels - 1 : j);
              const u32 lh = lad_t[(u32)j * k_lstride];
              const u32 lo = lh & 0xffffu, hi = lh >> 16;
              if (cnt > hi || (lo != 0u && cnt < lo + ov)) unsafe = true;
            }
          }
          GCRE_QT(ts1);
          GCRE_QT_ADD(8, ts1, ts0);
          if (__builtin_amdgcn_ballot_w64(unsafe) == 0ull) return;
        }
        todo[g] |= 1ull << t;
      };

      if (lad_row != lad_keep && npaths != 0u) {
        with_count<kQSegs>(qcnt, [&](auto ns) {
          u32 ZA[LZ], ZB[LZ];
          auto position = [&](u32 t, const u32 (&Z)[LZ]) {
#pragma unroll
            for (int g = 0; g < decltype(ns)::value; g++) filter_f(g, t, B[g], Z);
          };
          issue(0u, ZA);
          u32 zu = rdlane(zunit, 1u);
          u32 t = 0u;
          for (; t + 2u < npaths; t += 2u) {
            issue_at(zu, ZB);
            zu = rdlane(zunit, t + 2u);
            position(t, ZA);
            issue_at(zu, ZA);
            zu = rdlane(zunit, t + 3u);
            position(t + 1u, ZB);
          }
          if (t + 1u < npaths) {
            issue_at(zu, ZB);
            position(t, ZA);
            position(t + 1u, ZB);
          } else {
            position(t, ZA);
          }
        });
      }

      GCRE_QT(t4);
      GCRE_QT_ADD(3, t4, t3);
      struct Item { u32 t, info, lov, tot, lh; u32x8 o; };
      auto item_meta = [&](int g, u32 t) -> Item {
        Item it;
        const u64 q = (u64)firstg[g] + t;
        it.t = t;
        it.info = rdlane(infov[g], t);
        it.lh = rdlane(lhv[g], t);
        it.lov = (u32)q;
        it.tot = rdlane(totv[g], t);
        it.o = slots[q];
        return it;
      };
      auto item_issue = [&](const Item& it, u32 (&yy)[8], u32 (&ZZ)[LZ]) {
        const u32 ov = linfo_true_len(it.info);
#pragma unroll
        for (int j = 0; j < 8; j++) {
          yy[j] = 0u;
          if ((u32)j < ov) yy[j] = __builtin_amdgcn_raw_buffer_load_b32(mt, lane4, it.o[j], 0);
        }
        if (linfo_overlap(it.info)) issue(it.t, ZZ);
      };
      auto exact_f = [&](const Item& it, const u32 (&Bg)[L], const u32 (&y)[8], const u32 (&Z)[LZ]) {
        const u32 len = linfo_len(it.info);
        const bool overlap = linfo_overlap(it.info);
        const u32 lo = it.lh & 0xffffu, hi = it.lh >> 16;
        u32 S4[4];
        sum8(y, S4);
        u32 S[L];
#pragma unroll
        for (int l = 0; l < L; l++) S[l] = (l < 4) ? S4[l < 4 ? l : 0] : 0u;
        if (len > 8u) {
          const u32 GCRE_CONSTANT* more = (const u32 GCRE_CONSTANT*)(a.dover + ((const u32 GCRE_CONSTANT*)a.lover)[it.lov]);
          for (u32 p = 0u; p + 8u < len; p += 8u) {
            const u32x8 o8 = *(const u32x8 GCRE_CONSTANT*)(more + p);
            u32 yy[8], s4[4];
#pragma unroll
            for (int j = 0; j < 8; j++) yy[j] = __builtin_amdgcn_raw_buffer_load_b32(mt, lane4, o8[j], 0);
            sum8(yy, s4);
            u32 cy = 0u;
#pragma unroll
            for (int l = 0; l < L; l++) {
              const u32 sv = S[l];
              if (l < 4) {
                S[l] = xor3(sv, s4[l < 4 ? l : 0], cy);
                cy = majority(sv, s4[l < 4 ? l : 0], cy);
              } else {
                S[l] = sv ^ cy;
                cy = sv & cy;
              }
            }
          }
        }
        u32 C[L];
        if (overlap) {
          u32 cy = 0u, bw = 0u;
#pragma unroll
          for (int l = 0; l < L; l++) {
            const u32 zl = (l < LZ) ? Z[l < LZ ? l : 0] : 0u;
            const u32 w = xor3(Bg[l], zl, cy);
            cy = majority(Bg[l], zl, cy);
            C[l] = xor3(w, S[l], bw);
            bw = borrow3(w, S[l], bw);
          }
        } else {
          u32 cy = 0u;
#pragma unroll
          for (int l = 0; l < L; l++) {
            C[l] = xor3(Bg[l], S[l], cy);
            cy = majority(Bg[l], S[l], cy);
          }
        }
        u32 blo = 0u, bhi = 0u;
#pragma unroll
        for (int l = 0; l < L; l++) {
          const u32 kl = (u32)__builtin_amdgcn_sbfe((int)lo, l, 1);
          const u32 kh = (u32)__builtin_amdgcn_sbfe((int)hi, l, 1);
          blo = borrow3(C[l], kl, blo);
          bhi = borrow3(kh, C[l], bhi);
        }
        u32 m = (blo | bhi) & valid;
        if (__builtin_amdgcn_ballot_w64(m != 0u) == 0ull) return;
        n_slow++;
        const u32 diag = sp_diag_offset(it.tot);
        while (__builtin_amdgcn_ballot_w64(m != 0u) != 0ull) {
          if (lq_n + 64u > kLqCap) lq_drain();
          const bool has = m != 0u;
          const u32 bb = has ? (u32)__builtin_ctz(m) : 0u;
          m &= m - 1u;
          u32 cnt = 0u;
#pragma unroll
          for (int l = 0; l < L; l++) cnt |= ((C[l] >> bb) & 1u) << l;
          const u64 hm = __builtin_amdgcn_ballot_w64(has);
          const u32 pos = lq_n + __builtin_amdgcn_mbcnt_hi((u32)(hm >> 32), __builtin_amdgcn_mbcnt_lo((u32)hm, 0u));
          if (has) {
            lq[0][pos] = diag + cnt;
            lq[1][pos] = bb * 64u + (u32)lane;
          }
          lq_n += (u32)__builtin_popcountll(hm);
        }
      };
#pragma unroll
      for (int g = 0; g < kQSegs; g++) {
        if ((u32)g < qcnt && todo[g] != 0ull) {
          u64 m = todo[g];
          u32 yA[8], yB[8], ZA[LZ], ZB[LZ];
#pragma unroll
          for (int l = 0; l < LZ; l++) ZA[l] = ZB[l] = 0u;
          auto pop = [&]() -> u32 {
            const u32 t = (u32)__builtin_ctzll(m);
            m &= m - 1ull;
            return t;
          };
          Item cur = item_meta(g, pop()), nxt = cur, aft = cur;
          bool has_n = m != 0ull, has_a = false;
          if (has_n) nxt = item_meta(g, pop());
          item_issue(cur, yA, ZA);
          for (;;) {
            if (has_n) item_issue(nxt, yB, ZB);
            has_a = m != 0ull;
            if (has_a) aft = item_meta(g, pop());
            exact_f(cur, B[g], yA, ZA);
            if (!has_n) break;
            cur = nxt; nxt = aft; has_n = has_a;
            if (has_n) item_issue(nxt, yA, ZA);
            has_a = m != 0ull;
            if (has_a) aft = item_meta(g, pop());
            exact_f(cur, B[g], yB, ZB);
            if (!has_n) break;
            cur = nxt; nxt = aft; has_n = has_a;
          }
        }
      }
      GCRE_QT(t5);
      GCRE_QT_ADD(4, t5, t4);
#ifdef GCRE_IE_TIMING
      tm[7] += 1;
#endif
    }
  }
  flush_tile();
#ifdef GCRE_IE_TIMING
  tm[6] = __builtin_amdgcn_s_memtime() - tm_begin;
  if (a.timing && lane == 0)
    for (int i = 0; i < 11; i++) atomicAdd((unsigned long long*)a.timing + i, (unsigned long long)tm[i]);
  if (a.timing && n_flagged) atomicAdd((unsigned long long*)a.timing + 11, (unsigned long long)n_flagged);
#endif
  if (a.stats && lane == 0 && n_slow) atomicAdd(a.stats, n_slow);
}

#define GCRE_IEQ_W(EXPR, LL, GG, RR) if (wide) { EXPR(LL, GG, RR, true); } else { EXPR(LL, GG, RR, false); }
#define GCRE_IEQ_R(EXPR, LL, GG) if (rec) { GCRE_IEQ_W(EXPR, LL, GG, true) } else { GCRE_IEQ_W(EXPR, LL, GG, false) }

#ifdef GCRE_IEQ_ONLY
#define GCRE_IEQ(EXPR) { (void)gz; (void)planes; GCRE_IEQ_R(EXPR, 10, 2) }
#else
#define GCRE_IEQ(EXPR)                                                     \
  if (planes <= 8) { GCRE_IEQ_R(EXPR, 8, 2) }                              \
  else if (planes <= 10) {                                                 \
    if (gz <= 2) { GCRE_IEQ_R(EXPR, 10, 2) } else { GCRE_IEQ_R(EXPR, 10, 3) }        \
  } else if (planes <= 11) {                                               \
    if (gz <= 2) { GCRE_IEQ_R(EXPR, 11, 2) } else { GCRE_IEQ_R(EXPR, 11, 3) }        \
  } else if (planes <= 12) {                                               \
    if (gz <= 2) { GCRE_IEQ_R(EXPR, 12, 2) } else { GCRE_IEQ_R(EXPR, 12, 3) }        \
  } else {                                                                 \
    if (gz <= 2) { GCRE_IEQ_R(EXPR, 16, 2) }                               \
    else if (gz == 3) { GCRE_IEQ_R(EXPR, 16, 3) }                          \
    else { GCRE_IEQ_R(EXPR, 16, 4) }                                       \
  }
#endif

hipError_t launch_null_ie_quad(const IeArgs& a, int planes, hipStream_t stream) {
  const dim3 grid((unsigned)(8 * a.waves_per_xcd / kIeWaves));
  const dim3 block(64 * kIeWaves);
  const int gz = a.gz;
  const bool rec = a.rec_slot != nullptr, wide = a.z_wide != 0u;
#define GCRE_LAUNCHQ(LL, GG, RR, WW) hipLaunchKernelGGL((k_null_ie_q<LL, GG, RR, WW>), grid, block, 0, stream, a)
  GCRE_IEQ(GCRE_LAUNCHQ)
#undef GCRE_LAUNCHQ
  return hipGetLastError();
}

int ieq_quad_segs() { return kQSegs; }

int ieq_max_waves_per_cu(int planes, int gz, bool rec, bool wide) {
  int blocks = 0;
  hipError_t e = hipSuccess;
#define GCRE_OCCQ(LL, GG, RR, WW) e = hipOccupancyMaxActiveBlocksPerMultiprocessor(&blocks, k_null_ie_q<LL, GG, RR, WW>, 64 * kIeWaves, 0)
  GCRE_IEQ(GCRE_OCCQ)
#undef GCRE_OCCQ
  if (e != hipSuccess || blocks < 1) blocks = 1;
  return blocks * kIeWaves;
}

}
```

Measured before the change: 9796 billion.

## Read kernel arguments through a constant pointer rematerialized per loop iteration

```diff
diff --git a/geneticscre_amd/csrc/gcre_ie.hip b/geneticscre_amd/csrc/gcre_ie.hip
--- a/geneticscre_amd/csrc/gcre_ie.hip
+++ b/geneticscre_amd/csrc/gcre_ie.hip
@@ -11,27 +11,24 @@
 #endif
 
 template <int M, int L>
-__global__ __launch_bounds__(64 * kIeWaves) __attribute__((amdgpu_waves_per_eu(M == 1 ? 4 : 2))) void k_null_ie(const IeArgs a) {
+__global__ __launch_bounds__(64 * kIeWaves) __attribute__((amdgpu_waves_per_eu(M == 1 ? 4 : 2))) void k_null_ie(const IeArgs ) {
+  const IeArgs GCRE_CONSTANT* ap = ie_args();
   static_assert(L % 4 == 0 && L >= 8 && L <= 16, "planes come in groups of 4");
   const int lane = threadIdx.x & 63;
   const int wave = __builtin_amdgcn_readfirstlane(threadIdx.x >> 6);
   const int xcd = blockIdx.x & 7;
   const i64 bi = (i64)(blockIdx.x >> 3);
-  const i64 bx = a.waves_per_xcd / kIeWaves;
-  const i64 cpt = (a.seg_end - a.seg_begin + kIeWaves - 1) / kIeWaves;
-  const i64 chunks = cpt * a.nkt;
+  const i64 bx = ap->waves_per_xcd / kIeWaves;
+  const i64 cpt = (ap->seg_end - ap->seg_begin + kIeWaves - 1) / kIeWaves;
+  const i64 chunks = cpt * ap->nkt;
   const u32 lane4 = (u32)lane * 4u;
   __shared__ u32 gmax_lds[kIeWaves][32 * 64];
   u32* scr = gmax_lds[wave] + lane;
 #pragma unroll
   for (int q = 0; q < 32; q++) scr[q * 64] = 0u;
 
-  const SparseSeg GCRE_CONSTANT* segs = (const SparseSeg GCRE_CONSTANT*)a.segs;
-  const u64 GCRE_CONSTANT* loff0 = (const u64 GCRE_CONSTANT*)a.loff0;
-  const u32 GCRE_CONSTANT* lidx0 = (const u32 GCRE_CONSTANT*)a.lidx0;
-
   int cur_kt = -1;
-  __amdgpu_buffer_rsrc_t mt = __builtin_amdgcn_make_buffer_rsrc((void*)a.mt, 0, 0x7fffffff, 0x00020000);
+  __amdgpu_buffer_rsrc_t mt = __builtin_amdgcn_make_buffer_rsrc((void*)ap->mt, 0, 0x7fffffff, 0x00020000);
 #ifdef GCRE_IE_TIMING
   u64 tm[6] = {0, 0, 0, 0, 0, 0};
   const u64 tm_begin = __builtin_amdgcn_s_memtime();
@@ -42,10 +39,10 @@
     GCRE_TM_MARK(tf0);
     __syncthreads();
     const u32 slot0 = (u32)wave * 512u + (u32)lane * 8u;
-    __amdgpu_buffer_rsrc_t nb = __builtin_amdgcn_make_buffer_rsrc((void*)(a.null_bits + (size_t)cur_kt * 2048), 0, 8192, 0x00020000);
+    __amdgpu_buffer_rsrc_t nb = __builtin_amdgcn_make_buffer_rsrc((void*)(ap->null_bits + (size_t)cur_kt * 2048), 0, 8192, 0x00020000);
     const u32x4 g0 = __builtin_amdgcn_raw_buffer_load_b128(nb, slot0 * 4u, 0, 16 );
     const u32x4 g1 = __builtin_amdgcn_raw_buffer_load_b128(nb, slot0 * 4u + 16u, 0, 16 );
-    u32* out = a.null_bits + (size_t)cur_kt * 2048 + slot0;
+    u32* out = ap->null_bits + (size_t)cur_kt * 2048 + slot0;
     u32* cell = &gmax_lds[0][0] + (slot0 & 31u) * 64u + (slot0 >> 5);
     u32 own[8];
 #pragma unroll
@@ -80,7 +77,7 @@
   auto finish_m1 = [&](const u32 (&C)[L], u32 total) {
     u32 R[16];
     to_counts(C, R);
-    const u32* diag_g = (const u32*)a.t32 + sp_diag_offset(total);
+    const u32* diag_g = (const u32*)ap->t32 + sp_diag_offset(total);
     u32 v[32], o[32];
 #pragma unroll
     for (int j = 0; j < 16; j++) {
@@ -98,8 +95,8 @@
     u32 Rp[16], Rn[16];
     to_counts(Cp, Rp);
     to_counts(Cn, Rn);
-    const double* dp = a.d64 + sp_diag_offset(tp);
-    const double* dn = a.d64 + sp_diag_offset(tn);
+    const double* dp = ap->d64 + sp_diag_offset(tp);
+    const double* dn = ap->d64 + sp_diag_offset(tn);
 #pragma unroll
     for (int g0 = 0; g0 < 16; g0 += 4) {
       double sp[8], sn[8];
@@ -139,15 +136,17 @@
 
   const i64 c_end = (i64)(xcd + 1) * chunks / 8;
   for (i64 c = (i64)xcd * chunks / 8 + bi; c < c_end; c += bx) {
+    ie_args_again(ap);
     const int kt = (int)(c / cpt);
     if (kt != cur_kt) {
       flush();
       cur_kt = kt;
-      mt = __builtin_amdgcn_make_buffer_rsrc((void*)(a.mt + (size_t)kt * a.mt_rows * 64), 0, 0x7fffffff, 0x00020000);
-    }
-    const i64 sidx = a.seg_begin + (c - (i64)kt * cpt) * kIeWaves + wave;
-    if (sidx < a.seg_end) {
+      mt = __builtin_amdgcn_make_buffer_rsrc((void*)(ap->mt + (size_t)kt * ap->mt_rows * 64), 0, 0x7fffffff, 0x00020000);
+    }
+    const i64 sidx = ap->seg_begin + (c - (i64)kt * cpt) * kIeWaves + wave;
+    if (sidx < ap->seg_end) {
       GCRE_TM_MARK(ts0);
+      const SparseSeg GCRE_CONSTANT* segs = (const SparseSeg GCRE_CONSTANT*)ap->segs;
       const u32 row0 = segs[sidx].row0;
       const u32 first = segs[sidx].first;
       const u32 npaths = segs[sidx].n;
@@ -155,23 +154,23 @@
       u32 infov[M], lovv[M];
 #pragma unroll
       for (int h = 0; h < M; h++) {
-        infov[h] = a.linfo[(u64)qv * M + h];
-        lovv[h] = a.lover[(u64)qv * M + h];
-      }
-      const u32 rzv = a.rowz[qv];
+        infov[h] = ap->linfo[(u64)qv * M + h];
+        lovv[h] = ap->lover[(u64)qv * M + h];
+      }
+      const u32 rzv = ap->rowz[qv];
       u32 zunit[M];
 #pragma unroll
       for (int h = 0; h < M; h++) {
         const u32 hz = (M == 2 && (rzv >> 31)) ? (u32)(1 - h) : (u32)h;
-        zunit[h] = ((u32)kt * (u32)a.rowsz + (rzv & 0x7fffffffu) * (u32)M + hz) * (u32)a.gz;
+        zunit[h] = ((u32)kt * (u32)ap->rowsz + (rzv & 0x7fffffffu) * (u32)M + hz) * (u32)ap->gz;
       }
       u32 ttv[M];
 #pragma unroll
-      for (int h = 0; h < M; h++) ttv[h] = a.tot[(u64)qv * M + h];
+      for (int h = 0; h < M; h++) ttv[h] = ap->tot[(u64)qv * M + h];
       u32 lv[M][8];
 #pragma unroll
       for (int h = 0; h < M; h++) {
-        const u32x4* lp = (const u32x4*)(a.dlist + ((u64)qv * M + h) * 8u);
+        const u32x4* lp = (const u32x4*)(ap->dlist + ((u64)qv * M + h) * 8u);
         const u32x4 e0 = lp[0], e1 = lp[1];
         lv[h][0] = e0.x; lv[h][1] = e0.y; lv[h][2] = e0.z; lv[h][3] = e0.w;
         lv[h][4] = e1.x; lv[h][5] = e1.y; lv[h][6] = e1.z; lv[h][7] = e1.w;
@@ -196,19 +195,19 @@
 #pragma unroll
       for (int h = 0; h < M; h++) {
         const u64 r = (u64)row0 * M + h;
-        if (a.planes0) {
-          load_planes(B[h], a.planes0, (u32)(((u64)kt * (u64)a.rows0 + r) * (u64)a.g0), a.g0);
-        } else if (a.rec_slot) {
-          const u32 ra = a.rec_row0[row0], rzr = a.rec_rowz[row0], rz = rzr & 0x7fffffffu, rinfo = a.rec_linfo[r];
+        if (ap->planes0) {
+          load_planes(B[h], ap->planes0, (u32)(((u64)kt * (u64)ap->rows0 + r) * (u64)ap->g0), ap->g0);
+        } else if (ap->rec_slot) {
+          const u32 ra = ap->rec_row0[row0], rzr = ap->rec_rowz[row0], rz = rzr & 0x7fffffffu, rinfo = ap->rec_linfo[r];
           const u32 hz = (M == 2 && (rzr >> 31)) ? (u32)(1 - h) : (u32)h;
           u32 ZR[L], S[L];
-          load_planes(B[h], a.rec_planes_a, (u32)(((u64)kt * (u64)a.rec_rows_a + (u64)ra * M + h) * (u64)a.rec_ga), a.rec_ga);
-          load_planes(ZR, a.rec_planes_z, (u32)(((u64)kt * (u64)a.rec_rows_z + (u64)rz * M + hz) * (u64)a.rec_gz), a.rec_gz);
+          load_planes(B[h], ap->rec_planes_a, (u32)(((u64)kt * (u64)ap->rec_rows_a + (u64)ra * M + h) * (u64)ap->rec_ga), ap->rec_ga);
+          load_planes(ZR, ap->rec_planes_z, (u32)(((u64)kt * (u64)ap->rec_rows_z + (u64)rz * M + hz) * (u64)ap->rec_gz), ap->rec_gz);
 #pragma unroll
           for (int l = 0; l < L; l++) S[l] = 0u;
           const u32 rlen = linfo_len(rinfo);
-          stream(S, (const u32 GCRE_CONSTANT*)(a.rec_slot + r * 8u), 0, 8);
-          if (rlen > 8u) stream(S, (const u32 GCRE_CONSTANT*)(a.rec_over + a.rec_lover[r]), 0, (u64)(rlen - 8u));
+          stream(S, (const u32 GCRE_CONSTANT*)(ap->rec_slot + r * 8u), 0, 8);
+          if (rlen > 8u) stream(S, (const u32 GCRE_CONSTANT*)(ap->rec_over + ap->rec_lover[r]), 0, (u64)(rlen - 8u));
           u32 cy = 0u, bw = 0u;
 #pragma unroll
           for (int l = 0; l < L; l++) {
@@ -222,7 +221,8 @@
         } else {
 #pragma unroll
           for (int l = 0; l < L; l++) B[h][l] = 0u;
-          stream(B[h], lidx0, loff0[r], loff0[r + 1]);
+          const u64 GCRE_CONSTANT* loff0 = (const u64 GCRE_CONSTANT*)ap->loff0;
+          stream(B[h], (const u32 GCRE_CONSTANT*)ap->lidx0, loff0[r], loff0[r + 1]);
         }
       }
 
@@ -244,7 +244,7 @@
           for (int j = 0; j < 8; j++) y[j] = __builtin_amdgcn_raw_buffer_load_b32(mt, lane4, offs[j], 0);
           u32 Z[L];
           if (overlap) {
-            load_planes(Z, a.planesz, rdlane(zunit[h], t), a.gz);
+            load_planes(Z, ap->planesz, rdlane(zunit[h], t), ap->gz);
           } else {
 #pragma unroll
             for (int l = 0; l < L; l++) Z[l] = 0u;
@@ -260,7 +260,7 @@
           S[0] = s0; S[1] = s1; S[2] = d0 ^ d1; S[3] = d0 & d1;
 #pragma unroll
           for (int l = 4; l < L; l++) S[l] = 0u;
-          if (len > 8u) stream(S, (const u32 GCRE_CONSTANT*)(a.dover + rdlane(lovv[h], t)), 0, (u64)(len - 8u));
+          if (len > 8u) stream(S, (const u32 GCRE_CONSTANT*)(ap->dover + rdlane(lovv[h], t)), 0, (u64)(len - 8u));
           if (overlap) {
             u32 cy = 0u, bw = 0u;
 #pragma unroll
@@ -279,14 +279,14 @@
             }
           }
         }
-        if (a.planes_out) {
+        if (ap->planes_out) {
 #pragma unroll
           for (int h = 0; h < M; h++) {
-            const u64 rh = ((u64)a.out_first + q) * M + h;
-            u32x4* dst = (u32x4*)(a.planes_out + (((u64)cur_kt * (u64)a.rows_out + rh) * (u64)a.go) * 256u) + lane;
+            const u64 rh = ((u64)ap->out_first + q) * M + h;
+            u32x4* dst = (u32x4*)(ap->planes_out + (((u64)cur_kt * (u64)ap->rows_out + rh) * (u64)ap->go) * 256u) + lane;
 #pragma unroll
             for (int j = 0; j < 4; j++) {
-              if (j < a.go) {
+              if (j < ap->go) {
                 u32x4 v = {0u, 0u, 0u, 0u};
                 if (4 * j < L) v = u32x4{C[h][(4 * j) % L], C[h][(4 * j + 1) % L], C[h][(4 * j + 2) % L], C[h][(4 * j + 3) % L]};
                 dst[j * 64] = v;
@@ -296,7 +296,7 @@
         }
         GCRE_TM_MARK(tp1);
         GCRE_TM_ADD(1, tp1, tp0);
-        if (q < a.score_begin || q >= a.score_end) continue;
+        if (q < ap->score_begin || q >= ap->score_end) continue;
         if constexpr (M == 1) {
           finish_m1(C[0], rdlane(ttv[0], t));
         } else {
@@ -310,15 +310,16 @@
   flush();
 #ifdef GCRE_IE_TIMING
   tm[5] = __builtin_amdgcn_s_memtime() - tm_begin;
-  if (a.timing && lane == 0)
-    for (int i = 0; i < 6; i++) atomicAdd((unsigned long long*)a.timing + i, (unsigned long long)tm[i]);
-  if (a.timing && lane == 0) atomicMax((unsigned long long*)a.timing + 6, (unsigned long long)tm[5]);
+  if (ap->timing && lane == 0)
+    for (int i = 0; i < 6; i++) atomicAdd((unsigned long long*)ap->timing + i, (unsigned long long)tm[i]);
+  if (ap->timing && lane == 0) atomicMax((unsigned long long*)ap->timing + 6, (unsigned long long)tm[5]);
 #endif
 }
 
 
 template <int L, int GZ, bool OUT, bool REC>
-__global__ __launch_bounds__(64 * kIeWaves) __attribute__((amdgpu_waves_per_eu(L <= 12 ? 4 : 3))) void k_null_ie_m1(const IeArgs a) {
+__global__ __launch_bounds__(64 * kIeWaves) __attribute__((amdgpu_waves_per_eu(L <= 12 ? 4 : 3))) void k_null_ie_m1(const IeArgs ) {
+  const IeArgs GCRE_CONSTANT* ap = ie_args();
   constexpr int LP = (L + 3) / 4 * 4;
   static_assert(L >= 8 && L <= 16 && GZ >= 2 && 4 * GZ <= LP, "planes come in groups of 4");
   __shared__ u32 nmax_lds[kIeWaves][32 * 64];
@@ -328,47 +329,44 @@
   u32* nm = nmax_lds[wave] + lane;
 #pragma unroll
   for (int q = 0; q < 32; q++) nm[q * 64] = 0u;
-  const SparseSeg GCRE_CONSTANT* segs = (const SparseSeg GCRE_CONSTANT*)a.segs;
-  const char* k_planesz = (const char*)(((u64)(u32)__builtin_amdgcn_readfirstlane((int)(u32)((u64)a.planesz >> 32)) << 32) |
-                                        (u64)(u32)__builtin_amdgcn_readfirstlane((int)(u32)(u64)a.planesz));
-
   int cur_kt = -1;
   u32 valid = 0u;
-  u32 lad_base = (a.lad_mode == 0) ? 0u : (u32)(kLadderLevels - 1 + a.lad_mode) * (u32)a.ladder_stride;
-  const u32 lad_keep = (u32)kLadderLevels * (u32)a.ladder_stride;
+  u32 lad_base = (ap->lad_mode == 0) ? 0u : (u32)(kLadderLevels - 1 + ap->lad_mode) * (u32)ap->ladder_stride;
   bool dirty = false;
   u32 n_slow = 0u;
 #ifdef GCRE_IE_TIMING
   u64 tm[6] = {0, 0, 0, 0, 0, 0};
   const u64 tm_begin = __builtin_amdgcn_s_memtime();
 #endif
-  __amdgpu_buffer_rsrc_t mt = __builtin_amdgcn_make_buffer_rsrc((void*)a.mt, 0, 0x7fffffff, 0x00020000);
+  __amdgpu_buffer_rsrc_t mt = __builtin_amdgcn_make_buffer_rsrc((void*)ap->mt, 0, 0x7fffffff, 0x00020000);
 
   auto exchange = [&]() {
-    u32* out = a.null_bits + (size_t)cur_kt * 2048 + lane * 32;
-    __amdgpu_buffer_rsrc_t nb = __builtin_amdgcn_make_buffer_rsrc((void*)(a.null_bits + (size_t)cur_kt * 2048), 0, 8192, 0x00020000);
+    u32* out = ap->null_bits + (size_t)cur_kt * 2048 + lane * 32;
+    __amdgpu_buffer_rsrc_t nb = __builtin_amdgcn_make_buffer_rsrc((void*)(ap->null_bits + (size_t)cur_kt * 2048), 0, 8192, 0x00020000);
     u32x4 g4[8];
 #pragma unroll
     for (int j = 0; j < 8; j++) g4[j] = __builtin_amdgcn_raw_buffer_load_b128(nb, (u32)lane * 128u + (u32)j * 16u, 0, 16 );
     u32 lo = 0xffffffffu;
+    u32 live = valid;
+    asm volatile("" : "+v"(live));
 #pragma unroll
     for (int q = 0; q < 32; q++) {
       const u32 g = g4[q >> 2][q & 3];
       const u32 own = nm[q * 64];
       if (dirty && own > g) atomicMax(out + q, own);
       const u32 v = own > g ? own : g;
-      if ((valid >> q) & 1u) lo = v < lo ? v : lo;
+      if ((live >> q) & 1u) lo = v < lo ? v : lo;
     }
     dirty = false;
     u32 theta = __builtin_amdgcn_readfirstlane(wave_min_u32(lo));
     if (theta == 0xffffffffu) theta = 0u;
     int j = (int)(__uint_as_float(theta) * (float)kLadderPerUnit);
     j = j < 0 ? 0 : (j > kLadderLevels - 1 ? kLadderLevels - 1 : j);
-    lad_base = (u32)j * (u32)a.ladder_stride;
+    lad_base = (u32)j * (u32)ap->ladder_stride;
   };
   auto flush_tile = [&]() {
     if (cur_kt >= 0) {
-      u32* out = a.null_bits + (size_t)cur_kt * 2048 + lane * 32;
+      u32* out = ap->null_bits + (size_t)cur_kt * 2048 + lane * 32;
 #pragma unroll 8
       for (int q = 0; q < 32; q++) {
         const u32 own = nm[q * 64];
@@ -384,13 +382,14 @@
   __shared__ u32 wq_state[kIeWaves][8];
   WorkQueue wq;
   wq.st = wq_state[wave];
-  wq.init(a.queue, (u32)((a.seg_end - a.seg_begin + a.batch - 1) / a.batch), (u32)a.nkt);
+  wq.init(ap->queue, (u32)((ap->seg_end - ap->seg_begin + ap->batch - 1) / ap->batch), (u32)ap->nkt);
   {
     wq.select(blockIdx.x & 7u);
   }
   u32 ticket = wq.take(lane);
   int since = 0, period = 1;
   for (;;) {
+    ie_args_again(ap);
     const u32 work = __builtin_amdgcn_readfirstlane(ticket);
     const u32 q_n = wq.get(2);
     if (work >= q_n) {
@@ -401,21 +400,22 @@
     ticket = wq.take(lane);
     const u32 item = wq.get(1) + work, nb = wq.get(3);
     const int kt = (int)(item / nb);
-    const i64 s_lo = a.seg_begin + (i64)(item - (u32)kt * nb) * a.batch;
-    const i64 s_hi = s_lo + a.batch < a.seg_end ? s_lo + a.batch : a.seg_end;
+    const i64 s_lo = ap->seg_begin + (i64)(item - (u32)kt * nb) * ap->batch;
+    const i64 s_hi = s_lo + ap->batch < ap->seg_end ? s_lo + ap->batch : ap->seg_end;
     if (kt != cur_kt) {
       flush_tile();
       cur_kt = kt;
-      mt = __builtin_amdgcn_make_buffer_rsrc((void*)(a.mt + (size_t)kt * a.mt_rows * 64), 0, 0x7fffffff, 0x00020000);
-      const int live = a.K - kt * 2048 - lane * 32;
+      mt = __builtin_amdgcn_make_buffer_rsrc((void*)(ap->mt + (size_t)kt * ap->mt_rows * 64), 0, 0x7fffffff, 0x00020000);
+      const int live = ap->K - kt * 2048 - lane * 32;
       valid = live >= 32 ? 0xffffffffu : (live <= 0 ? 0u : ((1u << live) - 1u));
-      if (a.lad_mode == 0) lad_base = 0u;
+      if (ap->lad_mode == 0) lad_base = 0u;
       since = 0;
       period = 1;
     }
     u32 nextv = 0u;
     bool have_next = false;
     for (i64 sidx = s_lo; sidx < s_hi; sidx++) {
+      ie_args_again(ap);
       u32 row0, first, npaths;
       u32 rc_a = 0u, rc_z = 0u, rc_info = 0u, rc_lov = 0u;
       typedef u32 __attribute__((ext_vector_type(8))) u32x8;
@@ -433,11 +433,12 @@
           for (int j = 0; j < 8; j++) rc_o[j] = rdlane(nextv, 8 + j);
         }
       } else {
+        const SparseSeg GCRE_CONSTANT* segs = (const SparseSeg GCRE_CONSTANT*)ap->segs;
         row0 = segs[sidx].row0;
         first = segs[sidx].first;
         npaths = segs[sidx].n;
         if constexpr (REC) {
-          const u32 GCRE_CONSTANT* rs = (const u32 GCRE_CONSTANT*)a.rec_segs + (u64)sidx * kRecSegWords;
+          const u32 GCRE_CONSTANT* rs = (const u32 GCRE_CONSTANT*)ap->rec_segs + (u64)sidx * kRecSegWords;
           rc_a = rs[0];
           rc_z = rs[1];
           rc_info = rs[2];
@@ -447,14 +448,14 @@
       }
       have_next = sidx + 1 < s_hi;
       if (have_next) {
-        const u32* src = (const u32*)a.segs + (u64)(sidx + 1) * 3u + (u32)(lane < 3 ? lane : 0);
+        const u32* src = (const u32*)ap->segs + (u64)(sidx + 1) * 3u + (u32)(lane < 3 ? lane : 0);
         if constexpr (REC) {
-          if (lane >= 4 && lane < 16) src = a.rec_segs + (u64)(sidx + 1) * kRecSegWords + (u32)(lane - 4);
+          if (lane >= 4 && lane < 16) src = ap->rec_segs + (u64)(sidx + 1) * kRecSegWords + (u32)(lane - 4);
         }
         nextv = *src;
       }
       GCRE_TM_MARK(ts0);
-      if (a.lad_mode == 0 && ++since >= period) {
+      if (ap->lad_mode == 0 && ++since >= period) {
         exchange();
         since = 0;
         period = period < kIeRefresh ? period * 2 : kIeRefresh;
@@ -463,18 +464,18 @@
       GCRE_TM_ADD(4, ts1, ts0);
 
       const u32 qv = first + (((u32)lane < npaths) ? (u32)lane : 0u);
-      const u32 infov = a.linfo[qv];
-      const u32 lovv = a.lover[qv];
-      const u32 zunit = ((u32)kt * (u32)a.rowsz + (a.rowz[qv] & 0x7fffffffu)) * (u32)a.gz;
-      const u32 totv = a.tot[qv];
-      const u32 lhv = a.ladder[((u64)sidx < (u64)a.score_segs ? lad_base : lad_keep) + totv];
-      const u32x8 GCRE_CONSTANT* slots = (const u32x8 GCRE_CONSTANT*)(a.dlist + (u64)first * 8u);
+      const u32 infov = ap->linfo[qv];
+      const u32 lovv = ap->lover[qv];
+      const u32 zunit = ((u32)kt * (u32)ap->rowsz + (ap->rowz[qv] & 0x7fffffffu)) * (u32)ap->gz;
+      const u32 totv = ap->tot[qv];
+      const u32 lhv = ap->ladder[((u64)sidx < (u64)ap->score_segs ? lad_base : (u32)kLadderLevels * (u32)ap->ladder_stride) + totv];
+      const u32x8 GCRE_CONSTANT* slots = (const u32x8 GCRE_CONSTANT*)(ap->dlist + (u64)first * 8u);
       auto issue = [&](u32 t2, const u32x8 offs, u32 (&yy)[8], u32 (&ZZ)[4 * GZ]) {
         if constexpr (OUT) {
 #pragma unroll
           for (int j = 0; j < 8; j++) yy[j] = __builtin_amdgcn_raw_buffer_load_b32(mt, lane4, offs[j], 0);
         }
-        __amdgpu_buffer_rsrc_t rz = __builtin_amdgcn_make_buffer_rsrc((void*)(k_planesz + (u64)rdlane(zunit, t2) * 1024u), 0, 0x7fffffff, 0x00020000);
+        __amdgpu_buffer_rsrc_t rz = __builtin_amdgcn_make_buffer_rsrc((void*)((const char*)ap->planesz + (u64)rdlane(zunit, t2) * 1024u), 0, 0x7fffffff, 0x00020000);
 #pragma unroll
         for (int j = 0; j < GZ; j++) {
           const u32x4 v = __builtin_amdgcn_raw_buffer_load_b128(rz, lane4 * 4u + (u32)j * 1024u, 0, 0);
@@ -497,7 +498,7 @@
         }
       };
       if constexpr (!REC) {
-        load_groups(B, a.planes0, ((u64)kt * (u64)a.rows0 + (u64)row0) * (u64)a.g0, a.g0);
+        load_groups(B, ap->planes0, ((u64)kt * (u64)ap->rows0 + (u64)row0) * (u64)ap->g0, ap->g0);
       } else {
         const u32 ra = rc_a, rz = rc_z & 0x7fffffffu, rinfo = rc_info;
         const u32x8 ro = rc_o;
@@ -505,8 +506,8 @@
 #pragma unroll
         for (int j = 0; j < 8; j++) yr[j] = __builtin_amdgcn_raw_buffer_load_b32(mt, lane4, ro[j], 0);
         u32 ZR[LP];
-        load_groups(B, a.rec_planes_a, ((u64)kt * (u64)a.rec_rows_a + (u64)ra) * (u64)a.rec_ga, a.rec_ga);
-        load_groups(ZR, a.rec_planes_z, ((u64)kt * (u64)a.rec_rows_z + (u64)rz) * (u64)a.rec_gz, a.rec_gz);
+        load_groups(B, ap->rec_planes_a, ((u64)kt * (u64)ap->rec_rows_a + (u64)ra) * (u64)ap->rec_ga, ap->rec_ga);
+        load_groups(ZR, ap->rec_planes_z, ((u64)kt * (u64)ap->rec_rows_z + (u64)rz) * (u64)ap->rec_gz, ap->rec_gz);
         u32 S[L];
         {
           u32 S4[4];
@@ -516,7 +517,7 @@
         }
         const u32 rlen = linfo_len(rinfo);
         if (rlen > 8u) {
-          const u32 GCRE_CONSTANT* more = (const u32 GCRE_CONSTANT*)(a.rec_over + rc_lov);
+          const u32 GCRE_CONSTANT* more = (const u32 GCRE_CONSTANT*)(ap->rec_over + rc_lov);
           for (u32 p = 0u; p + 8u < rlen; p += 8u) {
             const u32x8 o8 = *(const u32x8 GCRE_CONSTANT*)(more + p);
             u32 yy[8], s4[4];
@@ -603,7 +604,7 @@
           u32 S[L];
 #pragma unroll
           for (int l = 0; l < L; l++) S[l] = (l < 4) ? S4[l < 4 ? l : 0] : 0u;
-          const u32 GCRE_CONSTANT* more = (const u32 GCRE_CONSTANT*)(a.dover + rdlane(lovv, t));
+          const u32 GCRE_CONSTANT* more = (const u32 GCRE_CONSTANT*)(ap->dover + rdlane(lovv, t));
           for (u32 p = 0u; p + 8u < len; p += 8u) {
             const u32x8 o8 = *(const u32x8 GCRE_CONSTANT*)(more + p);
             u32 yy[8], s4[4];
@@ -643,11 +644,11 @@
           }
         }
         if constexpr (OUT) {
-          const u64 rh = (u64)a.out_first + first + t;
-          u32x4* dst = (u32x4*)(a.planes_out + (((u64)kt * (u64)a.rows_out + rh) * (u64)a.go) * 256u) + lane;
+          const u64 rh = (u64)ap->out_first + first + t;
+          u32x4* dst = (u32x4*)(ap->planes_out + (((u64)kt * (u64)ap->rows_out + rh) * (u64)ap->go) * 256u) + lane;
 #pragma unroll
           for (int j = 0; j < 4; j++) {
-            if (j < a.go) {
+            if (j < ap->go) {
               u32x4 v = {0u, 0u, 0u, 0u};
               if (4 * j < L) v = u32x4{C[(4 * j) % L], (4 * j + 1 < L) ? C[(4 * j + 1) % L] : 0u, (4 * j + 2 < L) ? C[(4 * j + 2) % L] : 0u,
                                        (4 * j + 3 < L) ? C[(4 * j + 3) % L] : 0u};
@@ -670,7 +671,7 @@
         GCRE_TM_ADD(2, tp2, tp0);
         if (__builtin_amdgcn_ballot_w64(m != 0u) == 0ull) return;
         n_slow++;
-        const u32* diag_g = (const u32*)a.t32 + sp_diag_offset(rdlane(totv, t));
+        const u32* diag_g = (const u32*)ap->t32 + sp_diag_offset(rdlane(totv, t));
         while (m != 0u) {
           u32 bb[4], vv[4];
 #pragma unroll
@@ -744,7 +745,7 @@
 #pragma unroll
           for (int l = 0; l < L; l++) S[l] = (l < 4) ? S4[l < 4 ? l : 0] : 0u;
           if (len > 8u) {
-            const u32 GCRE_CONSTANT* more = (const u32 GCRE_CONSTANT*)(a.dover + rdlane(lovv, t));
+            const u32 GCRE_CONSTANT* more = (const u32 GCRE_CONSTANT*)(ap->dover + rdlane(lovv, t));
             for (u32 p = 0u; p + 8u < len; p += 8u) {
               const u32x8 o8 = *(const u32x8 GCRE_CONSTANT*)(more + p);
               u32 yy[8], s4[4];
@@ -792,7 +793,7 @@
           u32 m = (blo | bhi) & mu;
           if (m != 0u) {
             slow = 1u;
-            const u32* diag_g = (const u32*)a.t32 + sp_diag_offset(rdlane(totv, t));
+            const u32* diag_g = (const u32*)ap->t32 + sp_diag_offset(rdlane(totv, t));
             while (m != 0u) {
               u32 bb[4], vv[4];
 #pragma unroll
@@ -848,11 +849,11 @@
   flush_tile();
 #ifdef GCRE_IE_TIMING
   tm[5] = __builtin_amdgcn_s_memtime() - tm_begin;
-  if (a.timing && lane == 0)
-    for (int i = 0; i < 6; i++) atomicAdd((unsigned long long*)a.timing + i, (unsigned long long)tm[i]);
-  if (a.timing && lane == 0) atomicMax((unsigned long long*)a.timing + 6, (unsigned long long)tm[5]);
+  if (ap->timing && lane == 0)
+    for (int i = 0; i < 6; i++) atomicAdd((unsigned long long*)ap->timing + i, (unsigned long long)tm[i]);
+  if (ap->timing && lane == 0) atomicMax((unsigned long long*)ap->timing + 6, (unsigned long long)tm[5]);
 #endif
-  if (a.stats && lane == 0 && n_slow) atomicAdd(a.stats, n_slow);
+  if (ap->stats && lane == 0 && n_slow) atomicAdd(ap->stats, n_slow);
 }
 
 #define GCRE_IE_M2(EXPR)                    \
diff --git a/geneticscre_amd/csrc/gcre_ie2.hip b/geneticscre_amd/csrc/gcre_ie2.hip
--- a/geneticscre_amd/csrc/gcre_ie2.hip
+++ b/geneticscre_amd/csrc/gcre_ie2.hip
@@ -16,7 +16,8 @@
 namespace gcre {
 
 template <int L, int GZ, bool OUT, bool REC>
-__global__ __launch_bounds__(64 * kIeWaves) __attribute__((amdgpu_waves_per_eu(L <= 10 ? 4 : (L <= 12 ? 3 : GCRE_M2_WAVES16)))) void k_null_ie_m2(const IeArgs a) {
+__global__ __launch_bounds__(64 * kIeWaves) __attribute__((amdgpu_waves_per_eu(L <= 10 ? 4 : (L <= 12 ? 3 : GCRE_M2_WAVES16)))) void k_null_ie_m2(const IeArgs ) {
+  const IeArgs GCRE_CONSTANT* ap = ie_args();
   constexpr int NS = GCRE_M2_STEPS;
   static_assert(NS == 2 || NS == 3, "two or three steps");
   constexpr int LP = (L + 3) / 4 * 4;
@@ -35,7 +36,6 @@
   u32* nm = nmax_lds[wave] + lane;
 #pragma unroll
   for (int q = 0; q < 32; q++) nm[q * 64] = 0u;
-  const SparseSeg GCRE_CONSTANT* segs = (const SparseSeg GCRE_CONSTANT*)a.segs;
   u32 (*lq)[kLqCap] = lq_lds[wave];
   u32 lq_n = 0u;
   bool dirty = false;
@@ -43,7 +43,7 @@
     for (u32 base = 0u; base < lq_n; base += 64u) {
       const u32 i = base + (u32)lane;
       if (i < lq_n) {
-        const double f64 = a.d64[lq[0][i]] + a.d64[lq[1][i]];
+        const double f64 = ap->d64[lq[0][i]] + ap->d64[lq[1][i]];
         float f = (float)f64;
         f = (f > 0.0f) ? f : 0.0f;
         __hip_atomic_fetch_max(nmax_lds[wave] + lq[2][i], __float_as_uint(f), __ATOMIC_RELAXED, __HIP_MEMORY_SCOPE_WAVEFRONT);
@@ -52,17 +52,13 @@
     if (lq_n != 0u) dirty = true;
     lq_n = 0u;
   };
-  const char* k_planesz = (const char*)(((u64)(u32)__builtin_amdgcn_readfirstlane((int)(u32)((u64)a.planesz >> 32)) << 32) |
-                                        (u64)(u32)__builtin_amdgcn_readfirstlane((int)(u32)(u64)a.planesz));
-
   int cur_kt = -1;
   u32 valid = 0u;
   u32 lad[NS];
 #pragma unroll
-  for (int s = 0; s < NS; s++) lad[s] = (a.lad_mode == 0) ? 0u : (u32)(kLadder2Levels - 1 + a.lad_mode) * (u32)a.ladder_stride;
-  const u32 lad_keep = (u32)kLadder2Levels * (u32)a.ladder_stride;
+  for (int s = 0; s < NS; s++) lad[s] = (ap->lad_mode == 0) ? 0u : (u32)(kLadder2Levels - 1 + ap->lad_mode) * (u32)ap->ladder_stride;
   u32 lad_top = lad[0];
-  bool top_ok = a.lad_mode != 0 || a.g00_rows == 0u;
+  bool top_ok = ap->lad_mode != 0 || ap->g00_rows == 0u;
   u32 n_slow = 0u;
 #ifdef GCRE_IE_TIMING
   u64 tm[8] = {0, 0, 0, 0, 0, 0, 0, 0};
@@ -70,23 +66,25 @@
 #else
 #define GCRE_TM_COUNT(i, n)
 #endif
-  __amdgpu_buffer_rsrc_t mt = __builtin_amdgcn_make_buffer_rsrc((void*)a.mt, 0, 0x7fffffff, 0x00020000);
+  __amdgpu_buffer_rsrc_t mt = __builtin_amdgcn_make_buffer_rsrc((void*)ap->mt, 0, 0x7fffffff, 0x00020000);
 
   auto exchange = [&]() {
     lq_drain();
-    u32* out = a.null_bits + (size_t)cur_kt * 2048 + lane * 32;
-    __amdgpu_buffer_rsrc_t nb = __builtin_amdgcn_make_buffer_rsrc((void*)(a.null_bits + (size_t)cur_kt * 2048), 0, 8192, 0x00020000);
+    u32* out = ap->null_bits + (size_t)cur_kt * 2048 + lane * 32;
+    __amdgpu_buffer_rsrc_t nb = __builtin_amdgcn_make_buffer_rsrc((void*)(ap->null_bits + (size_t)cur_kt * 2048), 0, 8192, 0x00020000);
     u32x4 g4[8];
 #pragma unroll
     for (int j = 0; j < 8; j++) g4[j] = __builtin_amdgcn_raw_buffer_load_b128(nb, (u32)lane * 128u + (u32)j * 16u, 0, 16 );
     u32 lo = 0xffffffffu;
+    u32 live = valid;
+    asm volatile("" : "+v"(live));
 #pragma unroll
     for (int q = 0; q < 32; q++) {
       const u32 g = g4[q >> 2][q & 3];
       const u32 own = nm[q * 64];
       if (dirty && own > g) atomicMax(out + q, own);
       const u32 v = own > g ? own : g;
-      if ((valid >> q) & 1u) lo = v < lo ? v : lo;
+      if ((live >> q) & 1u) lo = v < lo ? v : lo;
     }
     dirty = false;
     u32 theta = __builtin_amdgcn_readfirstlane(wave_min_u32(lo));
@@ -105,16 +103,16 @@
 #pragma unroll
     for (int s = 0; s < NS; s++) {
       const int rs = r[s] > kLadder2Levels - 1 ? kLadder2Levels - 1 : r[s];
-      lad[s] = (u32)rs * (u32)a.ladder_stride;
-    }
-    const int rt = 2 * j - (int)a.g00_rows;
-    top_ok = a.g00_rows != 0xffffffffu && rt >= 0;
-    lad_top = (u32)(rt < 0 ? 0 : (rt > kLadder2Levels - 1 ? kLadder2Levels - 1 : rt)) * (u32)a.ladder_stride;
+      lad[s] = (u32)rs * (u32)ap->ladder_stride;
+    }
+    const int rt = 2 * j - (int)ap->g00_rows;
+    top_ok = ap->g00_rows != 0xffffffffu && rt >= 0;
+    lad_top = (u32)(rt < 0 ? 0 : (rt > kLadder2Levels - 1 ? kLadder2Levels - 1 : rt)) * (u32)ap->ladder_stride;
   };
   auto flush_tile = [&]() {
     lq_drain();
     if (cur_kt >= 0) {
-      u32* out = a.null_bits + (size_t)cur_kt * 2048 + lane * 32;
+      u32* out = ap->null_bits + (size_t)cur_kt * 2048 + lane * 32;
 #pragma unroll 8
       for (int q = 0; q < 32; q++) {
         const u32 own = nm[q * 64];
@@ -248,7 +246,7 @@
     u32 S[L];
 #pragma unroll
     for (int l = 0; l < L; l++) S[l] = (l < 4) ? S4[l < 4 ? l : 0] : 0u;
-    sum_more(S, len, (const u32 GCRE_CONSTANT*)a.dover, lover_at);
+    sum_more(S, len, (const u32 GCRE_CONSTANT*)ap->dover, lover_at);
     if (overlap) {
       u32 cy = 0u, bw = 0u;
 #pragma unroll
@@ -286,14 +284,14 @@
       for (int j = 0; j < 4; j++) yy[j] = 0u;
     }
     if (linfo_overlap(info)) {
-      __amdgpu_buffer_rsrc_t rz = __builtin_amdgcn_make_buffer_rsrc((void*)(k_planesz + (u64)zu * 1024u), 0, 0x7fffffff, 0x00020000);
+      __amdgpu_buffer_rsrc_t rz = __builtin_amdgcn_make_buffer_rsrc((void*)((const char*)ap->planesz + (u64)zu * 1024u), 0, 0x7fffffff, 0x00020000);
 #pragma unroll
       for (int j = 0; j < GZ; j++) {
         u32x4 v = {0u, 0u, 0u, 0u};
 #ifdef GCRE_M2_NOZLOAD
         v = u32x4{zu, zu + (u32)j, lane4, 0u};
 #else
-        if (j < 2 || j < a.gz) v = __builtin_amdgcn_raw_buffer_load_b128(rz, lane4 * 4u + (u32)j * 1024u, 0, 0);
+        if (j < 2 || j < ap->gz) v = __builtin_amdgcn_raw_buffer_load_b128(rz, lane4 * 4u + (u32)j * 1024u, 0, 0);
 #endif
         ZZ[4 * j + 0] = v.x; ZZ[4 * j + 1] = v.y; ZZ[4 * j + 2] = v.z; ZZ[4 * j + 3] = v.w;
       }
@@ -327,11 +325,12 @@
   __shared__ u32 wq_state[kIeWaves][8];
   WorkQueue wq;
   wq.st = wq_state[wave];
-  wq.init(a.queue, (u32)((a.seg_end - a.seg_begin + a.batch - 1) / a.batch), (u32)a.nkt);
+  wq.init(ap->queue, (u32)((ap->seg_end - ap->seg_begin + ap->batch - 1) / ap->batch), (u32)ap->nkt);
   wq.select(blockIdx.x & 7u);
   u32 ticket = wq.take(lane);
   int since = 0, period = 1;
   for (;;) {
+    ie_args_again(ap);
     const u32 work = __builtin_amdgcn_readfirstlane(ticket);
     const u32 q_n = wq.get(2);
     if (work >= q_n) {
@@ -342,45 +341,48 @@
     ticket = wq.take(lane);
     const u32 item = wq.get(1) + work, nb = wq.get(3);
     const int kt = (int)(item / nb);
-    const i64 s_lo = a.seg_begin + (i64)(item - (u32)kt * nb) * a.batch;
-    const i64 s_hi = s_lo + a.batch < a.seg_end ? s_lo + a.batch : a.seg_end;
+    const i64 s_lo = ap->seg_begin + (i64)(item - (u32)kt * nb) * ap->batch;
+    const i64 s_hi = s_lo + ap->batch < ap->seg_end ? s_lo + ap->batch : ap->seg_end;
     if (kt != cur_kt) {
       flush_tile();
       cur_kt = kt;
-      mt = __builtin_amdgcn_make_buffer_rsrc((void*)(a.mt + (size_t)kt * a.mt_rows * 64), 0, 0x7fffffff, 0x00020000);
-      const int live = a.K - kt * 2048 - lane * 32;
+      mt = __builtin_amdgcn_make_buffer_rsrc((void*)(ap->mt + (size_t)kt * ap->mt_rows * 64), 0, 0x7fffffff, 0x00020000);
+      const int live = ap->K - kt * 2048 - lane * 32;
       valid = live >= 32 ? 0xffffffffu : (live <= 0 ? 0u : ((1u << live) - 1u));
-      if (a.lad_mode == 0) {
+      if (ap->lad_mode == 0) {
 #pragma unroll
         for (int s = 0; s < NS; s++) lad[s] = 0u;
         lad_top = 0u;
-        top_ok = a.g00_rows == 0u;
+        top_ok = ap->g00_rows == 0u;
       }
       since = 0;
       period = 1;
     }
     for (i64 sidx = s_lo; sidx < s_hi; sidx++) {
+      ie_args_again(ap);
+      const SparseSeg GCRE_CONSTANT* segs = (const SparseSeg GCRE_CONSTANT*)ap->segs;
       const u32 row0 = segs[sidx].row0;
       const u32 first = segs[sidx].first;
       const u32 npaths = segs[sidx].n;
-      if (a.lad_mode == 0 && ++since >= period) {
+      if (ap->lad_mode == 0 && ++since >= period) {
         exchange();
         since = 0;
         period = period < kIeRefresh ? period * 2 : kIeRefresh;
       }
       const bool inl = (u32)lane < npaths;
       const u32 qv = first + (inl ? (u32)lane : 0u);
-      const u32 rzv = a.rowz[qv];
-      const bool mine = (u64)sidx < (u64)a.score_segs;
+      const u32 rzv = ap->rowz[qv];
+      const bool mine = (u64)sidx < (u64)ap->score_segs;
+      const u32 lad_keep = (u32)kLadder2Levels * (u32)ap->ladder_stride;
       const bool seg_top_ok = top_ok;
-      const u32 GCRE_CONSTANT* k_lover = (const u32 GCRE_CONSTANT*)a.lover + (u64)first * 2u;
-      const u32 GCRE_CONSTANT* k_tot = (const u32 GCRE_CONSTANT*)a.tot + (u64)first * 2u;
-      const u32 GCRE_CONSTANT* k_slot = (const u32 GCRE_CONSTANT*)a.dlist + (u64)first * 16u;
+      const u32 GCRE_CONSTANT* k_lover = (const u32 GCRE_CONSTANT*)ap->lover + (u64)first * 2u;
+      const u32 GCRE_CONSTANT* k_tot = (const u32 GCRE_CONSTANT*)ap->tot + (u64)first * 2u;
+      const u32 GCRE_CONSTANT* k_slot = (const u32 GCRE_CONSTANT*)ap->dlist + (u64)first * 16u;
       u32 infoc, zunitc, ladc[NS], ladt, ladu[NS], totu;
       u64 pm0, pm1, pm2;
       {
-        const u32 i0 = a.linfo[(u64)qv * 2], i1 = a.linfo[(u64)qv * 2 + 1];
-        const u32 t0_ = a.tot[(u64)qv * 2], t1_ = a.tot[(u64)qv * 2 + 1];
+        const u32 i0 = ap->linfo[(u64)qv * 2], i1 = ap->linfo[(u64)qv * 2 + 1];
+        const u32 t0_ = ap->tot[(u64)qv * 2], t1_ = ap->tot[(u64)qv * 2 + 1];
         const bool e0 = !linfo_overlap(i0) && (i0 & kLinfoLenMask) == linfo_pad(i0);
         const bool e1 = !linfo_overlap(i1) && (i1 & kLinfoLenMask) == linfo_pad(i1);
         pm0 = __builtin_amdgcn_ballot_w64(inl && e1);
@@ -389,45 +391,45 @@
         const bool c1 = e0 && !e1;
         infoc = c1 ? i1 : i0;
         const u32 hz = ((rzv >> 31) != 0u) != c1 ? 1u : 0u;
-        zunitc = ((u32)kt * (u32)a.rowsz + (rzv & 0x7fffffffu) * 2u + hz) * (u32)a.gz;
+        zunitc = ((u32)kt * (u32)ap->rowsz + (rzv & 0x7fffffffu) * 2u + hz) * (u32)ap->gz;
         const u32 tc = c1 ? t1_ : t0_;
         totu = c1 ? t0_ : t1_;
 #pragma unroll
         for (int s = 0; s < NS; s++) {
-          ladc[s] = a.ladder[(mine ? lad[s] : lad_keep) + tc];
-          ladu[s] = a.ladder[(mine ? lad[NS - 1 - s] : lad_keep) + totu];
-        }
-        ladt = a.ladder[(mine ? lad_top : lad_keep) + tc];
+          ladc[s] = ap->ladder[(mine ? lad[s] : lad_keep) + tc];
+          ladu[s] = ap->ladder[(mine ? lad[NS - 1 - s] : lad_keep) + totu];
+        }
+        ladt = ap->ladder[(mine ? lad_top : lad_keep) + tc];
       }
 
       u32 B[2][LP];
       if constexpr (!REC) {
 #pragma unroll
         for (int h = 0; h < 2; h++)
-          load_groups(B[h], a.planes0, ((u64)kt * (u64)a.rows0 + (u64)row0 * 2 + h) * (u64)a.g0, a.g0);
+          load_groups(B[h], ap->planes0, ((u64)kt * (u64)ap->rows0 + (u64)row0 * 2 + h) * (u64)ap->g0, ap->g0);
       } else {
-        const u32 GCRE_CONSTANT* r_row0 = (const u32 GCRE_CONSTANT*)a.rec_row0;
-        const u32 GCRE_CONSTANT* r_rowz = (const u32 GCRE_CONSTANT*)a.rec_rowz;
-        const u32 GCRE_CONSTANT* r_linfo = (const u32 GCRE_CONSTANT*)a.rec_linfo;
-        const u32 GCRE_CONSTANT* r_lover = (const u32 GCRE_CONSTANT*)a.rec_lover;
+        const u32 GCRE_CONSTANT* r_row0 = (const u32 GCRE_CONSTANT*)ap->rec_row0;
+        const u32 GCRE_CONSTANT* r_rowz = (const u32 GCRE_CONSTANT*)ap->rec_rowz;
+        const u32 GCRE_CONSTANT* r_linfo = (const u32 GCRE_CONSTANT*)ap->rec_linfo;
+        const u32 GCRE_CONSTANT* r_lover = (const u32 GCRE_CONSTANT*)ap->rec_lover;
         const u32 ra = r_row0[row0], rzr = r_rowz[row0];
         const u32 ri0 = r_linfo[(u64)row0 * 2], ri1 = r_linfo[(u64)row0 * 2 + 1];
 #pragma unroll
         for (int h = 0; h < 2; h++)
-          load_groups(B[h], a.rec_planes_a, ((u64)kt * (u64)a.rec_rows_a + (u64)ra * 2 + h) * (u64)a.rec_ga, a.rec_ga);
+          load_groups(B[h], ap->rec_planes_a, ((u64)kt * (u64)ap->rec_rows_a + (u64)ra * 2 + h) * (u64)ap->rec_ga, ap->rec_ga);
 #pragma unroll
         for (int h = 0; h < 2; h++) {
           const u32 rinfo = h ? ri1 : ri0;
           const u32 rlen = linfo_len(rinfo);
           if (!linfo_overlap(rinfo) && rlen == linfo_pad(rinfo)) continue;
-          const u32x8 ro = *(const u32x8 GCRE_CONSTANT*)(a.rec_slot + ((u64)row0 * 2 + h) * 8u);
+          const u32x8 ro = *(const u32x8 GCRE_CONSTANT*)(ap->rec_slot + ((u64)row0 * 2 + h) * 8u);
           u32 yr[8];
 #pragma unroll
           for (int j = 0; j < 8; j++) yr[j] = __builtin_amdgcn_raw_buffer_load_b32(mt, lane4, ro[j], 0);
           u32 ZR[LP];
           if (linfo_overlap(rinfo)) {
             const u32 hz = (rzr >> 31) ? (u32)(1 - h) : (u32)h;
-            load_groups(ZR, a.rec_planes_z, ((u64)kt * (u64)a.rec_rows_z + (u64)(rzr & 0x7fffffffu) * 2 + hz) * (u64)a.rec_gz, a.rec_gz);
+            load_groups(ZR, ap->rec_planes_z, ((u64)kt * (u64)ap->rec_rows_z + (u64)(rzr & 0x7fffffffu) * 2 + hz) * (u64)ap->rec_gz, ap->rec_gz);
           }
           u32 S[L];
           {
@@ -436,7 +438,7 @@
 #pragma unroll
             for (int l = 0; l < L; l++) S[l] = (l < 4) ? S4[l < 4 ? l : 0] : 0u;
           }
-          if (rlen > 8u) sum_more(S, rlen, (const u32 GCRE_CONSTANT*)a.rec_over, r_lover + (u64)row0 * 2 + h);
+          if (rlen > 8u) sum_more(S, rlen, (const u32 GCRE_CONSTANT*)ap->rec_over, r_lover + (u64)row0 * 2 + h);
           if (linfo_overlap(rinfo)) {
             u32 cy = 0u, bw = 0u;
 #pragma unroll
@@ -459,11 +461,11 @@
       }
       auto write_out = [&](u32 h, u32 t, const auto& C) {
         if constexpr (OUT) {
-          const u64 rh = ((u64)a.out_first + first + t) * 2 + h;
-          u32x4* dst = (u32x4*)(a.planes_out + (((u64)kt * (u64)a.rows_out + rh) * (u64)a.go) * 256u) + lane;
+          const u64 rh = ((u64)ap->out_first + first + t) * 2 + h;
+          u32x4* dst = (u32x4*)(ap->planes_out + (((u64)kt * (u64)ap->rows_out + rh) * (u64)ap->go) * 256u) + lane;
 #pragma unroll
           for (int j = 0; j < 4; j++) {
-            if (j < a.go) {
+            if (j < ap->go) {
               u32x4 v = {0u, 0u, 0u, 0u};
               if (4 * j < L) v = u32x4{C[(4 * j) % L], (4 * j + 1 < L) ? C[(4 * j + 1) % L] : 0u,
                                        (4 * j + 2 < L) ? C[(4 * j + 2) % L] : 0u, (4 * j + 3 < L) ? C[(4 * j + 3) % L] : 0u};
@@ -480,12 +482,12 @@
         u32 info2[2], zunit2[2], lad2[NS][2];
 #pragma unroll
         for (int h = 0; h < 2; h++) {
-          info2[h] = a.linfo[(u64)qv * 2 + h];
+          info2[h] = ap->linfo[(u64)qv * 2 + h];
           const u32 hz = (rzv >> 31) ? (u32)(1 - h) : (u32)h;
-          zunit2[h] = ((u32)kt * (u32)a.rowsz + (rzv & 0x7fffffffu) * 2u + hz) * (u32)a.gz;
-          const u32 th = a.tot[(u64)qv * 2 + h];
-#pragma unroll
-          for (int s = 0; s < NS; s++) lad2[s][h] = a.ladder[(mine ? lad[s] : lad_keep) + th];
+          zunit2[h] = ((u32)kt * (u32)ap->rowsz + (rzv & 0x7fffffffu) * 2u + hz) * (u32)ap->gz;
+          const u32 th = ap->tot[(u64)qv * 2 + h];
+#pragma unroll
+          for (int s = 0; s < NS; s++) lad2[s][h] = ap->ladder[(mine ? lad[s] : lad_keep) + th];
         }
         u64 rem = pm2;
         u32 t = (u32)__builtin_ctzll(rem);
@@ -603,10 +605,10 @@
   }
   flush_tile();
 #ifdef GCRE_IE_TIMING
-  if (a.timing && lane == 0)
-    for (int i = 0; i < 7; i++) atomicAdd((unsigned long long*)a.timing + i, (unsigned long long)tm[i]);
-#endif
-  if (a.stats && lane == 0 && n_slow) atomicAdd(a.stats, n_slow);
+  if (ap->timing && lane == 0)
+    for (int i = 0; i < 7; i++) atomicAdd((unsigned long long*)ap->timing + i, (unsigned long long)tm[i]);
+#endif
+  if (ap->stats && lane == 0 && n_slow) atomicAdd(ap->stats, n_slow);
 }
 
 #define GCRE_IE_M2P(EXPR)                                                                  \
diff --git a/geneticscre_amd/csrc/gcre_ie_common.h b/geneticscre_amd/csrc/gcre_ie_common.h
--- a/geneticscre_amd/csrc/gcre_ie_common.h
+++ b/geneticscre_amd/csrc/gcre_ie_common.h
@@ -1,12 +1,22 @@
 #pragma once
 #include "gcre_bitslice.h"
 #include "gcre_kernels.h"
+
+#include <type_traits>
 
 namespace gcre {
 
 constexpr int kIeWaves = 4;
 constexpr int kIeQueueStride = 16;
 constexpr int kIeRefresh = 32;
+
+static_assert(std::is_trivially_copyable<IeArgs>::value && alignof(IeArgs) <= 16, "IeArgs sits in the kernarg segment byte for byte as the host fills it");
+__device__ __forceinline__ void ie_args_again(const IeArgs GCRE_CONSTANT*& ap) { asm volatile("" : "+s"(ap)); }
+__device__ __forceinline__ const IeArgs GCRE_CONSTANT* ie_args() {
+  const IeArgs GCRE_CONSTANT* ap = (const IeArgs GCRE_CONSTANT*)__builtin_amdgcn_kernarg_segment_ptr();
+  ie_args_again(ap);
+  return ap;
+}
 
 __device__ __forceinline__ u32 maj3(u32 a, u32 b, u32 c) { return (a & b) | ((a ^ b) & c); }
 
diff --git a/geneticscre_amd/csrc/gcre_ieq.hip b/geneticscre_amd/csrc/gcre_ieq.hip
--- a/geneticscre_amd/csrc/gcre_ieq.hip
+++ b/geneticscre_amd/csrc/gcre_ieq.hip
@@ -32,11 +32,12 @@
 }
 
 template <int L, int GZ, bool REC, bool WIDE>
-__global__ __launch_bounds__(64 * kIeWaves) __attribute__((amdgpu_waves_per_eu(GCRE_QWAVES))) void k_null_ie_q(const IeArgs a) {
+__global__ __launch_bounds__(64 * kIeWaves) __attribute__((amdgpu_waves_per_eu(GCRE_QWAVES))) void k_null_ie_q(const IeArgs ) {
   constexpr int LP = (L + 3) / 4 * 4;
   constexpr int LZ = 4 * GZ;
   static_assert(L >= 8 && L <= 16 && GZ >= 2 && LZ <= LP, "planes come in groups of 4");
   typedef u32 __attribute__((ext_vector_type(8))) u32x8;
+  const IeArgs GCRE_CONSTANT* ap = ie_args();
   __shared__ u32 nmax_lds[kIeWaves][32 * 64];
   __shared__ u32 wq_state[kIeWaves][8];
   constexpr u32 kLqCap = 128u;
@@ -57,42 +58,34 @@
     for (u32 base = 0u; base < lq_n; base += 64u) {
       const u32 i = base + (u32)lane;
       if (i < lq_n)
-        __hip_atomic_fetch_max(nmax_lds[wave] + lq[1][i], ((const u32*)a.t32)[lq[0][i]], __ATOMIC_RELAXED, __HIP_MEMORY_SCOPE_WAVEFRONT);
+        __hip_atomic_fetch_max(nmax_lds[wave] + lq[1][i], ((const u32*)ap->t32)[lq[0][i]], __ATOMIC_RELAXED, __HIP_MEMORY_SCOPE_WAVEFRONT);
     }
     lq_n = 0u;
   };
   auto uni = [](u32 v) -> u32 { return (u32)__builtin_amdgcn_readfirstlane((int)v); };
   auto uni_ptr = [&](const void* p) -> const char* { return (const char*)(((u64)uni((u32)((u64)p >> 32)) << 32) | (u64)uni((u32)(u64)p)); };
-  const u32 k_quad_begin = uni((u32)a.quad_begin), k_quad_end = uni((u32)a.quad_end), k_batch = uni((u32)a.batch);
-  const u32 k_nkt = uni((u32)a.nkt), k_K = uni((u32)a.K), k_mt_rows = uni(a.mt_rows), k_lstride = uni((u32)a.ladder_stride);
-  const u32 k_lad_mode = uni((u32)a.lad_mode), k_score_segs = uni(a.score_segs);
-  const char* k_mt = uni_ptr(a.mt);
-  const char* k_planesz = uni_ptr(a.planesz);
-  const u32 k_ztile = uni(a.z_tile_units);
-
-  const u32 k_road = (k_lad_mode == 0u) ? (uni(a.flagq) != 0u ? 2u : 1u) : 0u;
+  auto road = [&]() -> u32 { return (ap->lad_mode == 0) ? (ap->flagq != 0u ? 2u : 1u) : 0u; };
 
   int cur_kt = -1;
   u32 valid = 0u;
-  u32 lad_base = (k_lad_mode == 0u) ? 0u : ((u32)kLadderLevels - 1u + k_lad_mode) * k_lstride;
-  const u32 lad_keep = (u32)kLadderLevels * k_lstride;
+  u32 lad_base = (ap->lad_mode == 0) ? 0u : ((u32)kLadderLevels - 1u + (u32)ap->lad_mode) * (u32)ap->ladder_stride;
   u32 n_slow = 0u;
 #ifdef GCRE_IE_TIMING
   u64 tm[11] = {0, 0, 0, 0, 0, 0, 0, 0, 0, 0, 0};
   u32 n_flagged = 0u;
   const u64 tm_begin = __builtin_amdgcn_s_memtime();
 #endif
-  __amdgpu_buffer_rsrc_t mt = __builtin_amdgcn_make_buffer_rsrc((void*)k_mt, 0, 0x7fffffff, 0x00020000);
-  __amdgpu_buffer_rsrc_t zt = __builtin_amdgcn_make_buffer_rsrc((void*)k_planesz, 0, 0x7fffffff, 0x00020000);
+  __amdgpu_buffer_rsrc_t mt = __builtin_amdgcn_make_buffer_rsrc((void*)ap->mt, 0, 0x7fffffff, 0x00020000);
+  __amdgpu_buffer_rsrc_t zt = __builtin_amdgcn_make_buffer_rsrc((void*)ap->planesz, 0, 0x7fffffff, 0x00020000);
 
   auto fq_drain = [&]() {
     GCRE_QT(td0);
     if ((u32)lane < fq_n) {
       const u32 q = fq[0][lane], w = fq[1][lane];
       const u32 bb = (w >> 17) & 31u, at = (w >> 22) * 4u;
-      const u32x4* e = (const u32x4*)(a.dlist + (u64)q * 8u);
+      const u32x4* e = (const u32x4*)(ap->dlist + (u64)q * 8u);
       const u32x4 e0 = e[0], e1 = e[1];
-      const u32 tot = a.tot[q];
+      const u32 tot = ap->tot[q];
       u32 y[8];
 #pragma unroll
       for (int j = 0; j < 4; j++) {
@@ -103,7 +96,7 @@
 #pragma unroll
       for (int j = 0; j < 8; j++) S += (y[j] >> bb) & 1u;
       const u32 cell = sp_diag_offset(tot) + (w & 0x1ffffu) - S;
-      __hip_atomic_fetch_max(nmax_lds[wave] + bb * 64u + (w >> 22), ((const u32*)a.t32)[cell], __ATOMIC_RELAXED, __HIP_MEMORY_SCOPE_WAVEFRONT);
+      __hip_atomic_fetch_max(nmax_lds[wave] + bb * 64u + (w >> 22), ((const u32*)ap->t32)[cell], __ATOMIC_RELAXED, __HIP_MEMORY_SCOPE_WAVEFRONT);
     }
     fq_n = 0u;
     GCRE_QT(td1);
@@ -111,12 +104,14 @@
   };
 
   auto merge_global = [&](bool want_theta) {
-    u32* out = a.null_bits + (size_t)cur_kt * 2048 + lane * 32;
-    __amdgpu_buffer_rsrc_t nb = __builtin_amdgcn_make_buffer_rsrc((void*)(a.null_bits + (size_t)cur_kt * 2048), 0, 8192, 0x00020000);
+    u32* out = ap->null_bits + (size_t)cur_kt * 2048 + lane * 32;
+    __amdgpu_buffer_rsrc_t nb = __builtin_amdgcn_make_buffer_rsrc((void*)(ap->null_bits + (size_t)cur_kt * 2048), 0, 8192, 0x00020000);
     u32x4 g4[8];
 #pragma unroll
     for (int j = 0; j < 8; j++) g4[j] = __builtin_amdgcn_raw_buffer_load_b128(nb, (u32)lane * 128u + (u32)j * 16u, 0, 16 );
     u32 lo = 0xffffffffu;
+    u32 live = valid;
+    asm volatile("" : "+v"(live));
 #pragma unroll
     for (int q = 0; q < 32; q++) {
       const u32 g = g4[q >> 2][q & 3];
@@ -124,7 +119,7 @@
       if (own > g) atomicMax(out + q, own);
       const u32 v = own > g ? own : g;
       nm[q * 64] = want_theta ? v : 0u;
-      if ((valid >> q) & 1u) lo = v < lo ? v : lo;
+      if ((live >> q) & 1u) lo = v < lo ? v : lo;
     }
     return lo;
   };
@@ -135,7 +130,7 @@
     if (theta == 0xffffffffu) theta = 0u;
     int j = (int)(__uint_as_float(theta) * (float)kLadderPerUnit);
     j = j < 0 ? 0 : (j > kLadderLevels - 1 ? kLadderLevels - 1 : j);
-    lad_base = (u32)j * k_lstride;
+    lad_base = (u32)j * (u32)ap->ladder_stride;
   };
   auto flush_tile = [&]() {
     fq_drain();
@@ -145,11 +140,12 @@
 
   WorkQueue wq;
   wq.st = wq_state[wave];
-  wq.init(a.queue, (k_quad_end - k_quad_begin + k_batch - 1u) / k_batch, k_nkt);
+  wq.init(ap->queue, ((u32)ap->quad_end - (u32)ap->quad_begin + (u32)ap->batch - 1u) / (u32)ap->batch, (u32)ap->nkt);
   wq.select(blockIdx.x & 7u);
   u32 ticket = wq.take(lane);
   int since = 0, period = 1;
   for (;;) {
+    ie_args_again(ap);
     const u32 work = __builtin_amdgcn_readfirstlane(ticket);
     const u32 q_n = wq.get(2);
     if (work >= q_n) {
@@ -160,16 +156,16 @@
     ticket = wq.take(lane);
     const u32 item = wq.get(1) + work, nbt = wq.get(3);
     const int kt = __builtin_amdgcn_readfirstlane((int)(item / nbt));
-    const u32 q_lo = uni(k_quad_begin + (item - (u32)kt * nbt) * k_batch);
-    const u32 q_hi = uni(q_lo + k_batch < k_quad_end ? q_lo + k_batch : k_quad_end);
+    const u32 q_lo = uni((u32)ap->quad_begin + (item - (u32)kt * nbt) * (u32)ap->batch);
+    const u32 q_hi = uni(q_lo + (u32)ap->batch < (u32)ap->quad_end ? q_lo + (u32)ap->batch : (u32)ap->quad_end);
     if (kt != cur_kt) {
       flush_tile();
       cur_kt = kt;
-      mt = __builtin_amdgcn_make_buffer_rsrc((void*)(k_mt + (size_t)kt * k_mt_rows * 256u), 0, 0x7fffffff, 0x00020000);
-      if constexpr (!WIDE) zt = __builtin_amdgcn_make_buffer_rsrc((void*)(k_planesz + (u64)kt * (u64)k_ztile * 1024u), 0, 0x7fffffff, 0x00020000);
-      const int live = (int)k_K - kt * 2048 - lane * 32;
+      mt = __builtin_amdgcn_make_buffer_rsrc((void*)((const char*)ap->mt + (size_t)kt * ap->mt_rows * 256u), 0, 0x7fffffff, 0x00020000);
+      if constexpr (!WIDE) zt = __builtin_amdgcn_make_buffer_rsrc((void*)((const char*)ap->planesz + (u64)kt * (u64)ap->z_tile_units * 1024u), 0, 0x7fffffff, 0x00020000);
+      const int live = ap->K - kt * 2048 - lane * 32;
       valid = live >= 32 ? 0xffffffffu : (live <= 0 ? 0u : ((1u << live) - 1u));
-      if (k_lad_mode == 0u) lad_base = 0u;
+      if (ap->lad_mode == 0) lad_base = 0u;
       since = 0;
       period = 1;
     }
@@ -179,9 +175,9 @@
       for (int g = 0; g < kQSegs; g++) {
         h[g] = 0u;
         if ((u32)g < cnt_) {
-          const u32* src = (const u32*)a.segs + (u64)(s0_ + (u32)g) * 3u + (u32)(lane < 3 ? lane : 0);
+          const u32* src = (const u32*)ap->segs + (u64)(s0_ + (u32)g) * 3u + (u32)(lane < 3 ? lane : 0);
           if constexpr (REC) {
-            if (lane >= 4 && lane < 16) src = a.rec_segs + (u64)(s0_ + (u32)g) * kRecSegWords + (u32)(lane - 4);
+            if (lane >= 4 && lane < 16) src = ap->rec_segs + (u64)(s0_ + (u32)g) * kRecSegWords + (u32)(lane - 4);
           }
           h[g] = *src;
         }
@@ -191,6 +187,7 @@
     u32 qe_n = 0u;
     bool have_next = false;
     for (u32 qi = q_lo; qi < q_hi; qi++) {
+      ie_args_again(ap);
       GCRE_QT(t0);
       u32 hdr[kQSegs];
       u32 qe;
@@ -199,23 +196,24 @@
 #pragma unroll
         for (int g = 0; g < kQSegs; g++) hdr[g] = hdr_n[g];
       } else {
-        qe = uni(((const u32 GCRE_CONSTANT*)a.quads)[qi]);
+        qe = uni(((const u32 GCRE_CONSTANT*)ap->quads)[qi]);
         load_hdr(qe, hdr);
       }
       have_next = qi + 1u < q_hi;
-      if (have_next) qe_n = uni(((const u32 GCRE_CONSTANT*)a.quads)[qi + 1u]);
+      if (have_next) qe_n = uni(((const u32 GCRE_CONSTANT*)ap->quads)[qi + 1u]);
       const u32 qcnt = (qe >> 30) + 1u;
       const u32 s0 = qe & 0x3fffffffu;
       const u32 npaths = rdlane(hdr[0], 2);
       GCRE_QT(te0);
-      if (k_lad_mode == 0u && ++since >= period) {
+      if (ap->lad_mode == 0 && ++since >= period) {
         exchange();
         since = 0;
         period = period < kIeRefresh ? period * 2 : kIeRefresh;
       }
       GCRE_QT(te1);
       GCRE_QT_ADD(5, te1, te0);
-      const u32 lad_row = (s0 < k_score_segs) ? lad_base : lad_keep;
+      const u32 lad_keep = (u32)kLadderLevels * (u32)ap->ladder_stride;
+      const u32 lad_row = (s0 < ap->score_segs) ? lad_base : lad_keep;
 
       u32 infov[kQSegs], lhv[kQSegs], lfv[kQSegs], firstg[kQSegs];
       u32 B[kQSegs][L];
@@ -242,11 +240,11 @@
           const u32 first = rdlane(hdr[g], 1);
           firstg[g] = first;
           const u32 qv = first + (((u32)lane < npaths) ? (u32)lane : 0u);
-          infov[g] = a.linfo[qv];
-          totv[g] = a.tot[qv];
+          infov[g] = ap->linfo[qv];
+          totv[g] = ap->tot[qv];
           if (g == 0) {
-            if constexpr (WIDE) zunit = ((u32)kt * (u32)a.rowsz + (a.rowz[qv] & 0x7fffffffu)) * (u32)a.gz;
-            else zunit = ((a.rowz[qv] & 0x7fffffffu) * (u32)a.gz) << 10;
+            if constexpr (WIDE) zunit = ((u32)kt * (u32)ap->rowsz + (ap->rowz[qv] & 0x7fffffffu)) * (u32)ap->gz;
+            else zunit = ((ap->rowz[qv] & 0x7fffffffu) * (u32)ap->gz) << 10;
           }
         }
       }
@@ -255,7 +253,7 @@
         if ((u32)g < qcnt) {
           const u32 row0 = rdlane(hdr[g], 0);
           if constexpr (!REC) {
-            load_groups(B[g], a.planes0, ((u64)kt * (u64)a.rows0 + (u64)row0) * (u64)a.g0, a.g0);
+            load_groups(B[g], ap->planes0, ((u64)kt * (u64)ap->rows0 + (u64)row0) * (u64)ap->g0, ap->g0);
           } else {
             const u32 ra = rdlane(hdr[g], 4);
             rz_g[g] = rdlane(hdr[g], 5) & 0x7fffffffu;
@@ -271,7 +269,7 @@
               if ((u32)j < rtrue) yr[REC ? g : 0][j] = __builtin_amdgcn_raw_buffer_load_b32(mt, lane4, ro[j], 0);
             }
             const int ga_need = (int)linfo_groups(rinfo_g[g]) + 1;
-            load_groups(B[g], a.rec_planes_a, ((u64)kt * (u64)a.rec_rows_a + (u64)ra) * (u64)a.rec_ga, ga_need < a.rec_ga ? ga_need : a.rec_ga);
+            load_groups(B[g], ap->rec_planes_a, ((u64)kt * (u64)ap->rec_rows_a + (u64)ra) * (u64)ap->rec_ga, ga_need < ap->rec_ga ? ga_need : ap->rec_ga);
           }
         }
       }
@@ -280,11 +278,11 @@
       GCRE_QT_ADD(0, t1, t0);
       if constexpr (REC) {
         u32 ZR[LP];
-        load_groups(ZR, a.rec_planes_z, ((u64)kt * (u64)a.rec_rows_z + (u64)rz_g[0]) * (u64)a.rec_gz, a.rec_gz);
+        load_groups(ZR, ap->rec_planes_z, ((u64)kt * (u64)ap->rec_rows_z + (u64)rz_g[0]) * (u64)ap->rec_gz, ap->rec_gz);
 #pragma unroll
         for (int g = 0; g < kQSegs; g++) {
           if ((u32)g < qcnt) {
-            if (rz_g[g] != rz_g[0]) load_groups(ZR, a.rec_planes_z, ((u64)kt * (u64)a.rec_rows_z + (u64)rz_g[g]) * (u64)a.rec_gz, a.rec_gz);
+            if (rz_g[g] != rz_g[0]) load_groups(ZR, ap->rec_planes_z, ((u64)kt * (u64)ap->rec_rows_z + (u64)rz_g[g]) * (u64)ap->rec_gz, ap->rec_gz);
             const u32 rinfo = rinfo_g[g];
             const u32 rlen = linfo_len(rinfo);
             u32 S[L];
@@ -295,7 +293,7 @@
               for (int l = 0; l < L; l++) S[l] = (l < 4) ? S4[l < 4 ? l : 0] : 0u;
             }
             if (rlen > 8u) {
-              const u32 GCRE_CONSTANT* more = (const u32 GCRE_CONSTANT*)(a.rec_over + rlov_g[g]);
+              const u32 GCRE_CONSTANT* more = (const u32 GCRE_CONSTANT*)(ap->rec_over + rlov_g[g]);
               for (u32 p = 0u; p + 8u < rlen; p += 8u) {
                 const u32x8 o8 = *(const u32x8 GCRE_CONSTANT*)(more + p);
                 u32 yy[8], s4[4];
@@ -330,7 +328,7 @@
                 cy = majority(bl, S[l], cy);
               }
             }
-            if (rz_g[g] != rz_g[0]) load_groups(ZR, a.rec_planes_z, ((u64)kt * (u64)a.rec_rows_z + (u64)rz_g[0]) * (u64)a.rec_gz, a.rec_gz);
+            if (rz_g[g] != rz_g[0]) load_groups(ZR, ap->rec_planes_z, ((u64)kt * (u64)ap->rec_rows_z + (u64)rz_g[0]) * (u64)ap->rec_gz, ap->rec_gz);
           }
         }
       }
@@ -339,7 +337,7 @@
 #pragma unroll
       for (int g = 0; g < kQSegs; g++) {
         if ((u32)g < qcnt) {
-          const u32 lh = a.ladder[lad_row + totv[g]];
+          const u32 lh = ap->ladder[lad_row + totv[g]];
           const u32 r0 = infov[g];
           const u32 ov = linfo_true_len(r0);
           const u32 lo = lh & 0xffffu;
@@ -351,11 +349,11 @@
 
       GCRE_QT(t3);
       GCRE_QT_ADD(2, t3, t2);
-      const u32x8 GCRE_CONSTANT* slots = (const u32x8 GCRE_CONSTANT*)a.dlist;
+      const u32x8 GCRE_CONSTANT* slots = (const u32x8 GCRE_CONSTANT*)ap->dlist;
       auto issue_at = [&](u32 zu, u32 (&ZZ)[LZ]) {
         __amdgpu_buffer_rsrc_t rz = zt;
         u32 so = 0u;
-        if constexpr (WIDE) rz = __builtin_amdgcn_make_buffer_rsrc((void*)(k_planesz + (u64)zu * 1024u), 0, 0x7fffffff, 0x00020000);
+        if constexpr (WIDE) rz = __builtin_amdgcn_make_buffer_rsrc((void*)((const char*)ap->planesz + (u64)zu * 1024u), 0, 0x7fffffff, 0x00020000);
         else so = zu;
 #pragma unroll
         for (int j = 0; j < GZ; j++) {
@@ -387,7 +385,7 @@
         u32 fm = (blo | bhi | cy) & valid;
         if (__builtin_amdgcn_ballot_w64(fm != 0u) == 0ull) return;
         const u32 info = rdlane(infov[g], t);
-        if (k_road != 0u && (info & 1u) != 0u && __builtin_amdgcn_ballot_w64(__builtin_popcount(fm) > GCRE_REFINE_MAX) == 0ull) {
+        if ((info & 1u) != 0u && road() != 0u && __builtin_amdgcn_ballot_w64(__builtin_popcount(fm) > GCRE_REFINE_MAX) == 0ull) {
           GCRE_QT(ts0);
 #ifdef GCRE_IE_TIMING
           tm[10] += 1;
@@ -407,7 +405,7 @@
               }
             }
           };
-          if (k_road == 2u && linfo_len(info) <= 8u) {
+          if (road() == 2u && linfo_len(info) <= 8u) {
             u32 total = 0u;
             {
               u32 f = fm;
@@ -444,7 +442,7 @@
             }
           }
           const u32 ov = linfo_true_len(info);
-          const u32* lad_t = a.ladder + rdlane(totv[g], t);
+          const u32* lad_t = ap->ladder + rdlane(totv[g], t);
           sum_w();
           bool unsafe = false;
           while (__builtin_amdgcn_ballot_w64(fm != 0u) != 0ull) {
@@ -457,7 +455,7 @@
             if (has) {
               int j = (int)(__uint_as_float(nm[bb * 64]) * (float)kLadderPerUnit);
               j = j < 0 ? 0 : (j > kLadderLevels - 1 ? kLadderLevels - 1 : j);
-              const u32 lh = lad_t[(u32)j * k_lstride];
+              const u32 lh = lad_t[(u32)j * (u32)ap->ladder_stride];
               const u32 lo = lh & 0xffffu, hi = lh >> 16;
               if (cnt > hi || (lo != 0u && cnt < lo + ov)) unsafe = true;
             }
@@ -530,7 +528,7 @@
 #pragma unroll
         for (int l = 0; l < L; l++) S[l] = (l < 4) ? S4[l < 4 ? l : 0] : 0u;
         if (len > 8u) {
-          const u32 GCRE_CONSTANT* more = (const u32 GCRE_CONSTANT*)(a.dover + ((const u32 GCRE_CONSTANT*)a.lover)[it.lov]);
+          const u32 GCRE_CONSTANT* more = (const u32 GCRE_CONSTANT*)(ap->dover + ((const u32 GCRE_CONSTANT*)ap->lover)[it.lov]);
           for (u32 p = 0u; p + 8u < len; p += 8u) {
             const u32x8 o8 = *(const u32x8 GCRE_CONSTANT*)(more + p);
             u32 yy[8], s4[4];
@@ -641,11 +639,11 @@
   flush_tile();
 #ifdef GCRE_IE_TIMING
   tm[6] = __builtin_amdgcn_s_memtime() - tm_begin;
-  if (a.timing && lane == 0)
-    for (int i = 0; i < 11; i++) atomicAdd((unsigned long long*)a.timing + i, (unsigned long long)tm[i]);
-  if (a.timing && n_flagged) atomicAdd((unsigned long long*)a.timing + 11, (unsigned long long)n_flagged);
-#endif
-  if (a.stats && lane == 0 && n_slow) atomicAdd(a.stats, n_slow);
+  if (ap->timing && lane == 0)
+    for (int i = 0; i < 11; i++) atomicAdd((unsigned long long*)ap->timing + i, (unsigned long long)tm[i]);
+  if (ap->timing && n_flagged) atomicAdd((unsigned long long*)ap->timing + 11, (unsigned long long)n_flagged);
+#endif
+  if (ap->stats && lane == 0 && n_slow) atomicAdd(ap->stats, n_slow);
 }
 
 #define GCRE_IEQ_W(EXPR, LL, GG, RR) if (wide) { EXPR(LL, GG, RR, true); } else { EXPR(LL, GG, RR, false); }
```

New measurement: 10040 billion, median of 6. +2.5%, better.
